# microsoft/FIBER

Measured on AMD Instinct MI355X. Metric: train-step images/sec (384^2, seq40) FIBER-Base, higher is better.
Workload: dtype bf16; 1 GPU; FIBER-Base (Swin-B 384^2 + RoBERTa-base S=40) MLM+ITM pretrain step, fused backbone fwd+bwd x2 + heads + AdamW; per_gpu_batch=256, global_batch=256, parallelism=dp1, rccl_ranks=1, dropout=reference defaults (text 0.1, DropPath linspace 0..0.1), residual_dtype=bf16, mlm_head_rows=all, launch=eager (one launch per kernel)

## Files before the change

### fiber_amd/csrc/elementwise.hip

```cpp
#include "common.h"

namespace {

__global__ __launch_bounds__(256) void gelu_bwd_kernel(const bf16* __restrict__ dg, const bf16* __restrict__ h,
                                                       bf16* __restrict__ dh, size_t nvec) {
  for (size_t i = blockIdx.x * (size_t)256 + threadIdx.x; i < nvec; i += (size_t)gridDim.x * 256) {
    const bf16x8 a = reinterpret_cast<const bf16x8*>(dg)[i], b = reinterpret_cast<const bf16x8*>(h)[i];
    reinterpret_cast<bf16x8*>(dh)[i] = gelu_grad_mul8(a, b);
  }
}

__global__ __launch_bounds__(256) void scale_add_kernel(const bf16* __restrict__ a, const bf16* __restrict__ b,
                                                        const float* __restrict__ alpha, float mult,
                                                        bf16* __restrict__ out, size_t nvec) {
  const float s = (alpha ? alpha[0] : 1.f) * mult;
  for (size_t i = blockIdx.x * (size_t)256 + threadIdx.x; i < nvec; i += (size_t)gridDim.x * 256) {
    const bf16x8 y = reinterpret_cast<const bf16x8*>(b)[i];
    bf16x8 o;
    if (a) {
      const bf16x8 x = reinterpret_cast<const bf16x8*>(a)[i];
#pragma unroll
      for (int e = 0; e < 8; ++e) o[e] = f2bf(bf2f(x[e]) + s * bf2f(y[e]));
    } else {
#pragma unroll
// ... 10 lines not shown
  for (size_t i = blockIdx.x * (size_t)256 + threadIdx.x; i < nvec; i += (size_t)gridDim.x * 256) {
    const bf16x8 x = reinterpret_cast<const bf16x8*>(a)[i], y = reinterpret_cast<const bf16x8*>(b)[i];
#pragma unroll
    for (int e = 0; e < 8; ++e) s += bf2f(x[e]) * bf2f(y[e]);
  }
  s = wave_sum(s);
  if ((threadIdx.x & 63) == 0) red[threadIdx.x >> 6] = s;
  __syncthreads();
  if (threadIdx.x == 0) out[blockIdx.x] = (red[0] + red[1]) + (red[2] + red[3]);
}

__global__ __launch_bounds__(256) void colsum_kernel(const bf16* __restrict__ x, float* __restrict__ out, int M, int N,
                                                     int ld, int rows_per_block) {
  __shared__ float red[8][32 * 8 + 1];
  const int cv = threadIdx.x & 31, rl = threadIdx.x >> 5;
  const int col = (blockIdx.x * 32 + cv) * 8;
  const int r0 = blockIdx.y * rows_per_block, r1 = min(M, r0 + rows_per_block);
  float s[8] = {0, 0, 0, 0, 0, 0, 0, 0};
  if (col < N) {
    int r = r0 + rl;
    for (; r + 24 < r1; r += 32) {
      const bf16x8 v0 = *reinterpret_cast<const bf16x8*>(x + (size_t)r * ld + col);
      const bf16x8 v1 = *reinterpret_cast<const bf16x8*>(x + (size_t)(r + 8) * ld + col);
      const bf16x8 v2 = *reinterpret_cast<const bf16x8*>(x + (size_t)(r + 16) * ld + col);
      const bf16x8 v3 = *reinterpret_cast<const bf16x8*>(x + (size_t)(r + 24) * ld + col);
#pragma unroll
      for (int e = 0; e < 8; ++e) s[e] += (bf2f(v0[e]) + bf2f(v1[e])) + (bf2f(v2[e]) + bf2f(v3[e]));
    }
    for (; r < r1; r += 8) {
      const bf16x8 v = *reinterpret_cast<const bf16x8*>(x + (size_t)r * ld + col);
#pragma unroll
      for (int e = 0; e < 8; ++e) s[e] += bf2f(v[e]);
    }
  }
#pragma unroll
  for (int e = 0; e < 8; ++e) red[rl][cv * 8 + e] = s[e];
  __syncthreads();
  const int c = threadIdx.x;
  float t = 0.f;
#pragma unroll
  for (int r = 0; r < 8; ++r) t += red[r][c];
  const int gc = blockIdx.x * 256 + c;
  if (gc < N) out[(size_t)blockIdx.y * N + gc] = t;
}

__global__ __launch_bounds__(256) void gelu_bwd_colsum_kernel(const bf16* __restrict__ dg, const bf16* __restrict__ h,
                                                              bf16* __restrict__ dh, float* __restrict__ out, int M, int N,
                                                              int rows_per_block) {
  __shared__ float red[8][32 * 8 + 1];
  const int cv = threadIdx.x & 31, rl = threadIdx.x >> 5;
  const int col = (blockIdx.x * 32 + cv) * 8;
  const int r0 = blockIdx.y * rows_per_block, r1 = min(M, r0 + rows_per_block);
  float s[8] = {0, 0, 0, 0, 0, 0, 0, 0};
  if (col < N) {
    auto one = [&](int r, const bf16x8& a, const bf16x8& b) {
      const bf16x8 o = gelu_grad_mul8(a, b);
#pragma unroll
      for (int e = 0; e < 8; ++e) s[e] += bf2f(o[e]);
      *reinterpret_cast<bf16x8*>(dh + (size_t)r * N + col) = o;
    };
    int r = r0 + rl;
    for (; r + 8 < r1; r += 16) {
      const size_t o0 = (size_t)r * N + col, o1 = (size_t)(r + 8) * N + col;
      const bf16x8 a0 = *reinterpret_cast<const bf16x8*>(dg + o0), b0 = *reinterpret_cast<const bf16x8*>(h + o0);
      const bf16x8 a1 = *reinterpret_cast<const bf16x8*>(dg + o1), b1 = *reinterpret_cast<const bf16x8*>(h + o1);
      one(r, a0, b0); one(r + 8, a1, b1);
    }
    for (; r < r1; r += 8) {
      const size_t off = (size_t)r * N + col;
      one(r, *reinterpret_cast<const bf16x8*>(dg + off), *reinterpret_cast<const bf16x8*>(h + off));
    }
  }
#pragma unroll
  for (int e = 0; e < 8; ++e) red[rl][cv * 8 + e] = s[e];
  __syncthreads();
  const int c = threadIdx.x;
  float t = 0.f;
#pragma unroll
  for (int r = 0; r < 8; ++r) t += red[r][c];
  const int gc = blockIdx.x * 256 + c;
  if (gc < N) out[(size_t)blockIdx.y * N + gc] = t;
}

__global__ __launch_bounds__(256) void rowscale_colsum_kernel(const bf16* __restrict__ x, const float* __restrict__ scale,
                                                              bf16* __restrict__ y, float* __restrict__ out, int M, int N,
                                                              int rows_per_block, int rows_per_sample) {
  __shared__ float red[8][32 * 8 + 1];
  const int cv = threadIdx.x & 31, rl = threadIdx.x >> 5;
  const int col = (blockIdx.x * 32 + cv) * 8;
  const int r0 = blockIdx.y * rows_per_block, r1 = min(M, r0 + rows_per_block);
  float s[8] = {0, 0, 0, 0, 0, 0, 0, 0};
  if (col < N) {
    auto one = [&](int r, const bf16x8& a) {
      const float sc = scale[r / rows_per_sample];
      bf16x8 o;
#pragma unroll
      for (int e = 0; e < 8; ++e) { o[e] = f2bf(sc * bf2f(a[e])); s[e] += bf2f(o[e]); }
      *reinterpret_cast<bf16x8*>(y + (size_t)r * N + col) = o;
    };
    int r = r0 + rl;
    for (; r + 24 < r1; r += 32) {
      const bf16x8 a0 = *reinterpret_cast<const bf16x8*>(x + (size_t)r * N + col);
      const bf16x8 a1 = *reinterpret_cast<const bf16x8*>(x + (size_t)(r + 8) * N + col);
      const bf16x8 a2 = *reinterpret_cast<const bf16x8*>(x + (size_t)(r + 16) * N + col);
      const bf16x8 a3 = *reinterpret_cast<const bf16x8*>(x + (size_t)(r + 24) * N + col);
      one(r, a0); one(r + 8, a1); one(r + 16, a2); one(r + 24, a3);
    }
    for (; r < r1; r += 8) one(r, *reinterpret_cast<const bf16x8*>(x + (size_t)r * N + col));
  }
#pragma unroll
  for (int e = 0; e < 8; ++e) red[rl][cv * 8 + e] = s[e];
  __syncthreads();
  const int c = threadIdx.x;
  float t = 0.f;
#pragma unroll
  for (int r = 0; r < 8; ++r) t += red[r][c];
  const int gc = blockIdx.x * 256 + c;
  if (gc < N) out[(size_t)blockIdx.y * N + gc] = t;
}

__global__ __launch_bounds__(256) void colsum_fold_kernel(const float* __restrict__ part, float* __restrict__ out, int slabs, int N) {
  __shared__ float red[16][17];
  const int cl = threadIdx.x & 15, rl = threadIdx.x >> 4;
  const int c = blockIdx.x * 16 + cl;
  float s0 = 0.f, s1 = 0.f, s2 = 0.f, s3 = 0.f;
  if (c < N) {
    int y = rl;
    for (; y + 48 < slabs; y += 64) {
      s0 += part[(size_t)y * N + c];
      s1 += part[(size_t)(y + 16) * N + c];
      s2 += part[(size_t)(y + 32) * N + c];
      s3 += part[(size_t)(y + 48) * N + c];
    }
    for (; y < slabs; y += 16) s0 += part[(size_t)y * N + c];
  }
  red[rl][cl] = (s0 + s1) + (s2 + s3);
  __syncthreads();
  if (rl == 0 && c < N) {
    float t = 0.f;
#pragma unroll
    for (int r = 0; r < 16; ++r) t += red[r][cl];
    out[c] = t;
  }
}

__global__ __launch_bounds__(256) void dropout_kernel(const bf16* __restrict__ x, bf16* __restrict__ y, size_t nvec,
                                                      uint64_t seed, const uint64_t* __restrict__ seed_base, uint32_t thresh,
                                                      float inv_keep) {
  if (seed_base) seed += *seed_base;
  for (size_t i = blockIdx.x * (size_t)256 + threadIdx.x; i < nvec; i += (size_t)gridDim.x * 256) {
    const bf16x8 v = reinterpret_cast<const bf16x8*>(x)[i];
    bf16x8 o;
    const uint32_t h0 = drop_base(seed, i * 8);
#pragma unroll
    for (int e = 0; e < 8; ++e) o[e] = drop_keep_e(h0, e, thresh) ? f2bf(bf2f(v[e]) * inv_keep) : f2bf(0.f);
    reinterpret_cast<bf16x8*>(y)[i] = o;
  }
}

__global__ __launch_bounds__(256) void droppath_scale_kernel(float* __restrict__ out, int n, float keep, uint64_t seed,
                                                             const uint64_t* __restrict__ seed_base) {
  if (seed_base) seed += *seed_base;
  const int i = blockIdx.x * 256 + threadIdx.x;
  if (i < n) {
    const float u = (float)(hash_u32(seed, (uint64_t)i) >> 9) * (1.0f / 8388608.0f);
    out[i] = floorf(keep + u) / keep;
  }
}

__global__ __launch_bounds__(256) void rowscale_add_kernel(const bf16* __restrict__ r, const bf16* __restrict__ x,
                                                           const float* __restrict__ scale, bf16* __restrict__ out,
                                                           size_t nvec, size_t vec_per_sample) {
  for (size_t i = blockIdx.x * (size_t)256 + threadIdx.x; i < nvec; i += (size_t)gridDim.x * 256) {
    const float s = scale[i / vec_per_sample];
    const bf16x8 b = reinterpret_cast<const bf16x8*>(x)[i];
    bf16x8 o;
    if (r) {
      const bf16x8 a = reinterpret_cast<const bf16x8*>(r)[i];
#pragma unroll
      for (int e = 0; e < 8; ++e) o[e] = f2bf(bf2f(a[e]) + s * bf2f(b[e]));
    } else {
#pragma unroll
      for (int e = 0; e < 8; ++e) o[e] = f2bf(s * bf2f(b[e]));
    }
    reinterpret_cast<bf16x8*>(out)[i] = o;
  }
}


struct StreamAddArgs {
  const void* res; const bf16* a; const bf16* b; const float* alpha; const float* rowscale;
  float* out32; bf16* out16;
  size_t nvec, vec_per_sample;
  uint64_t seed_a, seed_b; const uint64_t* seed_base;
  uint32_t thresh_a, thresh_b; float inv_keep_a, inv_keep_b;
};

template <int RES>
__global__ __launch_bounds__(256) void stream_add_kernel(StreamAddArgs p) {
  const float al = p.alpha ? p.alpha[0] : 1.f;
  uint64_t sa = p.seed_a, sb = p.seed_b;
  if (p.seed_base) { sa += *p.seed_base; sb += *p.seed_base; }
  for (size_t i = blockIdx.x * (size_t)256 + threadIdx.x; i < p.nvec; i += (size_t)gridDim.x * 256) {
    const float rs = p.rowscale ? p.rowscale[i / p.vec_per_sample] : 1.f;
    const bf16x8 av = reinterpret_cast<const bf16x8*>(p.a)[i];
    float v[8];
#pragma unroll
    for (int e = 0; e < 8; ++e) v[e] = bf2f(av[e]);
    if (p.thresh_a) {
      const uint32_t ha = drop_base(sa, i * 8);
#pragma unroll
      for (int e = 0; e < 8; ++e) v[e] = drop_keep_e(ha, e, p.thresh_a) ? v[e] * p.inv_keep_a : 0.f;
    }
    if (p.b) {
      const bf16x8 bv = reinterpret_cast<const bf16x8*>(p.b)[i];
      const uint32_t hb = drop_base(sb, i * 8);
#pragma unroll
      for (int e = 0; e < 8; ++e) {
        float t = bf2f(bv[e]);
        if (p.thresh_b) t = drop_keep_e(hb, e, p.thresh_b) ? t * p.inv_keep_b : 0.f;
        v[e] += al * t;
      }
    }
#pragma unroll
    for (int e = 0; e < 8; ++e) v[e] *= rs;
    if constexpr (RES == 2) {
      const float* rp = reinterpret_cast<const float*>(p.res) + i * 8;
      const float4 r0 = *reinterpret_cast<const float4*>(rp), r1 = *reinterpret_cast<const float4*>(rp + 4);
      v[0] += r0.x; v[1] += r0.y; v[2] += r0.z; v[3] += r0.w; v[4] += r1.x; v[5] += r1.y; v[6] += r1.z; v[7] += r1.w;
    } else if constexpr (RES == 1) {
      const bf16x8 rv = reinterpret_cast<const bf16x8*>(p.res)[i];
#pragma unroll
      for (int e = 0; e < 8; ++e) v[e] += bf2f(rv[e]);
    }
    if (p.out32) {
      float* op = p.out32 + i * 8;
      *reinterpret_cast<float4*>(op) = float4{v[0], v[1], v[2], v[3]};
      *reinterpret_cast<float4*>(op + 4) = float4{v[4], v[5], v[6], v[7]};
    }
    if (p.out16) {
      bf16x8 o;
#pragma unroll
      for (int e = 0; e < 8; ++e) o[e] = f2bf(v[e]);
      reinterpret_cast<bf16x8*>(p.out16)[i] = o;
    }
  }
}

struct StreamAddBwdArgs {
  const bf16* dy; const bf16* b; const float* alpha; const float* rowscale;
  bf16* da; bf16* db; float* dpart;
  size_t nvec, vec_per_sample;
// ... 89 lines not shown
  hipLaunchKernelGGL(scale_add_kernel, dim3(ew_grid(n / 8)), dim3(256), 0, stream, (const bf16*)a, (const bf16*)b, alpha, mult, (bf16*)out, (size_t)n / 8);
  FIBER_CHECK_LAUNCH();
  return FIBER_OK;
}

static inline int dot_grid(size_t nvec) {
  const size_t g = (nvec + 255) / 256;
  return (int)(g > FIBER_DOT_PARTS ? FIBER_DOT_PARTS : g);
}

extern "C" int fiber_dot_bf16(const void* a, const void* b, float* out, float* workspace, long n, hipStream_t stream) {
  if (n <= 0) return FIBER_OK;
  if ((n & 7) || !out || fiber_misaligned(16, a, b)) return FIBER_EINVAL;
  const size_t nvec = n / 8;
  const int grid = dot_grid(nvec);
  if (grid > 1 && !workspace) return FIBER_EINVAL;
  hipLaunchKernelGGL(dot_kernel, dim3(grid), dim3(256), 0, stream, (const bf16*)a, (const bf16*)b, grid > 1 ? workspace : out, nvec);
  FIBER_CHECK_LAUNCH();
  if (grid > 1) {
    hipLaunchKernelGGL(colsum_fold_kernel, dim3(1), dim3(256), 0, stream, workspace, out, grid, 1);
    FIBER_CHECK_LAUNCH();
  }
  return FIBER_OK;
}

extern "C" int fiber_colsum_slabs(int M, int N) {
  const int gx = cdiv(N, 256);
  int gy = cdiv(M, 512);
  int cap = cdiv(1024, gx);
  cap = cap > 512 ? 512 : cap;
  gy = gy > cap ? cap : gy;
  return gy < 1 ? 1 : gy;
}

extern "C" int fiber_colsum_bf16(const void* x, float* out, float* workspace, int M, int N, int ld, hipStream_t stream) {
  if (M <= 0 || N <= 0) return FIBER_OK;
  if ((N & 7) || (ld & 7) || fiber_misaligned(16, x)) return FIBER_EINVAL;
  const int gx = cdiv(N, 256);
  const int gy0 = fiber_colsum_slabs(M, N);
  const int rpb = cdiv(M, gy0), gy = cdiv(M, rpb);
  if (gy > 1 && !workspace) return FIBER_EINVAL;
  hipLaunchKernelGGL(colsum_kernel, dim3(gx, gy), dim3(256), 0, stream, (const bf16*)x, gy > 1 ? workspace : out, M, N, ld, rpb);
  FIBER_CHECK_LAUNCH();
  if (gy > 1) {
    hipLaunchKernelGGL(colsum_fold_kernel, dim3(cdiv(N, 16)), dim3(256), 0, stream, workspace, out, gy, N);
    FIBER_CHECK_LAUNCH();
  }
  return FIBER_OK;
}

extern "C" int fiber_gelu_bwd_colsum_bf16(const void* dgelu, const void* h_pre, void* dh, float* db, float* workspace, int M,
                                          int N, hipStream_t stream) {
  if (M <= 0 || N <= 0) return FIBER_OK;
  if ((N & 7) || fiber_misaligned(16, dgelu, h_pre, dh)) return FIBER_EINVAL;
  const int gx = cdiv(N, 256);
  const int gy0 = fiber_colsum_slabs(M, N);
  const int rpb = cdiv(M, gy0), gy = cdiv(M, rpb);
  if (gy > 1 && !workspace) return FIBER_EINVAL;
  hipLaunchKernelGGL(gelu_bwd_colsum_kernel, dim3(gx, gy), dim3(256), 0, stream, (const bf16*)dgelu, (const bf16*)h_pre, (bf16*)dh,
                     gy > 1 ? workspace : db, M, N, rpb);
  FIBER_CHECK_LAUNCH();
  if (gy > 1) {
    hipLaunchKernelGGL(colsum_fold_kernel, dim3(cdiv(N, 16)), dim3(256), 0, stream, workspace, db, gy, N);
    FIBER_CHECK_LAUNCH();
  }
  return FIBER_OK;
}

extern "C" int fiber_rowscale_colsum_bf16(const void* x, const float* scale, void* y, float* db, float* workspace, int M, int N,
                                          int rows_per_sample, hipStream_t stream) {
  if (M <= 0 || N <= 0) return FIBER_OK;
  if ((N & 7) || rows_per_sample <= 0 || fiber_misaligned(16, x, y)) return FIBER_EINVAL;
  const int gx = cdiv(N, 256);
  const int gy0 = fiber_colsum_slabs(M, N);
  const int rpb = cdiv(M, gy0), gy = cdiv(M, rpb);
  if (gy > 1 && !workspace) return FIBER_EINVAL;
  hipLaunchKernelGGL(rowscale_colsum_kernel, dim3(gx, gy), dim3(256), 0, stream, (const bf16*)x, scale, (bf16*)y,
                     gy > 1 ? workspace : db, M, N, rpb, rows_per_sample);
  FIBER_CHECK_LAUNCH();
  if (gy > 1) {
    hipLaunchKernelGGL(colsum_fold_kernel, dim3(cdiv(N, 16)), dim3(256), 0, stream, workspace, db, gy, N);
    FIBER_CHECK_LAUNCH();
  }
  return FIBER_OK;
}

extern "C" int fiber_fold_rows_f32(const float* part, float* out, int rows, int N, hipStream_t stream) {
  if (rows <= 0 || N <= 0) return FIBER_OK;
  hipLaunchKernelGGL(colsum_fold_kernel, dim3(cdiv(N, 16)), dim3(256), 0, stream, part, out, rows, N);
  FIBER_CHECK_LAUNCH();
  return FIBER_OK;
}

extern "C" int fiber_dropout_bf16(const void* x, void* y, long n, float p, uint64_t seed, const uint64_t* seed_base,
                                  hipStream_t stream) {
  if (n <= 0) return FIBER_OK;
  if ((n & 7) || p < 0.f || p >= 1.f || fiber_misaligned(16, x, y)) return FIBER_EINVAL;
  const uint32_t thresh = (uint32_t)((double)p * 4294967296.0);
  hipLaunchKernelGGL(dropout_kernel, dim3(ew_grid(n / 8)), dim3(256), 0, stream, (const bf16*)x, (bf16*)y, (size_t)n / 8, seed, seed_base, thresh, 1.f / (1.f - p));
  FIBER_CHECK_LAUNCH();
  return FIBER_OK;
}

extern "C" int fiber_droppath_scale_f32(float* out, int n, float keep, uint64_t seed, const uint64_t* seed_base,
                                        hipStream_t stream) {
  if (n <= 0) return FIBER_OK;
  if (keep <= 0.f || keep > 1.f) return FIBER_EINVAL;
  hipLaunchKernelGGL(droppath_scale_kernel, dim3(cdiv(n, 256)), dim3(256), 0, stream, out, n, keep, seed, seed_base);
  FIBER_CHECK_LAUNCH();
  return FIBER_OK;
}

extern "C" int fiber_rowscale_add_bf16(const void* r, const void* x, const float* scale, void* out, long n,
                                       long per_sample, hipStream_t stream) {
  if (n <= 0) return FIBER_OK;
  if ((n & 7) || per_sample <= 0 || (per_sample & 7) || fiber_misaligned(16, r, x, out)) return FIBER_EINVAL;
  hipLaunchKernelGGL(rowscale_add_kernel, dim3(ew_grid(n / 8)), dim3(256), 0, stream, (const bf16*)r, (const bf16*)x, scale, (bf16*)out, (size_t)n / 8, (size_t)per_sample / 8);
  FIBER_CHECK_LAUNCH();
  return FIBER_OK;
}

extern "C" int fiber_stream_add(const void* res, int res_kind, const void* a, const void* b, const float* alpha,
                                const float* rowscale, long per_sample, float p_a, uint64_t seed_a, float p_b, uint64_t seed_b,
                                const uint64_t* seed_base, float* out32, void* out16, long n, hipStream_t stream) {
  if (n <= 0) return FIBER_OK;
  if ((n & 7) || !a || (!out32 && !out16) || (res_kind && !res) || res_kind < 0 || res_kind > 2) return FIBER_EINVAL;
  if (fiber_misaligned(16, res, a, b, out32, out16)) return FIBER_EINVAL;
  if (rowscale && (per_sample <= 0 || (per_sample & 7))) return FIBER_EINVAL;
  if (p_a < 0.f || p_a >= 1.f || p_b < 0.f || p_b >= 1.f || (p_b > 0.f && !b)) return FIBER_EINVAL;
  StreamAddArgs p{res, (const bf16*)a, (const bf16*)b, alpha, rowscale, out32, (bf16*)out16, (size_t)n / 8,
                  rowscale ? (size_t)per_sample / 8 : (size_t)1, seed_a, seed_b, seed_base,
                  (uint32_t)((double)p_a * 4294967296.0), (uint32_t)((double)p_b * 4294967296.0), 1.f / (1.f - p_a), 1.f / (1.f - p_b)};
  const int grid = ew_grid(p.nvec);
  if (res_kind == 2) hipLaunchKernelGGL(stream_add_kernel<2>, dim3(grid), dim3(256), 0, stream, p);
  else if (res_kind == 1) hipLaunchKernelGGL(stream_add_kernel<1>, dim3(grid), dim3(256), 0, stream, p);
  else hipLaunchKernelGGL(stream_add_kernel<0>, dim3(grid), dim3(256), 0, stream, p);
  FIBER_CHECK_LAUNCH();
  return FIBER_OK;
}

extern "C" int fiber_stream_add_bwd(const void* dy, const void* b, const float* alpha, const float* rowscale, long per_sample,
                                    float p_a, uint64_t seed_a, float p_b, uint64_t seed_b, const uint64_t* seed_base, void* da,
                                    void* db, float* dalpha, float* workspace, long n, hipStream_t stream) {
  if (n <= 0) return FIBER_OK;
  if ((n & 7) || !dy || (dalpha && (!b || !db))) return FIBER_EINVAL;
  if (fiber_misaligned(16, dy, b, da, db)) return FIBER_EINVAL;
  if (rowscale && (per_sample <= 0 || (per_sample & 7))) return FIBER_EINVAL;
  if (p_a < 0.f || p_a >= 1.f || p_b < 0.f || p_b >= 1.f) return FIBER_EINVAL;
  StreamAddBwdArgs p{(const bf16*)dy, (const bf16*)b, alpha, rowscale, (bf16*)da, (bf16*)db, nullptr, (size_t)n / 8,
                     rowscale ? (size_t)per_sample / 8 : (size_t)1, seed_a, seed_b, seed_base,
                     (uint32_t)((double)p_a * 4294967296.0), (uint32_t)((double)p_b * 4294967296.0), 1.f / (1.f - p_a), 1.f / (1.f - p_b)};
  int grid = ew_grid(p.nvec);
  if (dalpha) {
    grid = dot_grid(p.nvec);
    if (grid > 1 && !workspace) return FIBER_EINVAL;
    p.dpart = grid > 1 ? workspace : dalpha;
  }
  hipLaunchKernelGGL(stream_add_bwd_kernel, dim3(grid), dim3(256), 0, stream, p);
  FIBER_CHECK_LAUNCH();
  if (dalpha && grid > 1) {
    hipLaunchKernelGGL(colsum_fold_kernel, dim3(1), dim3(256), 0, stream, workspace, dalpha, grid, 1);
    FIBER_CHECK_LAUNCH();
  }
  return FIBER_OK;
}

// ... 8 lines not shown
```

### fiber_amd/csrc/gemm.hip

```cpp
#include <stdlib.h>

#include "gemm_epilogue.h"

namespace {

template <int BM, int BN>
__global__ __launch_bounds__(256) void gemm_nt_kernel(GemmArgs a) {
  constexpr int WTM = BM / 2, WTN = BN / 2;
  constexpr int TM = WTM / 32, TN = WTN / 32;
  constexpr int PA = BM / 32, PB = BN / 32;
  __shared__ __attribute__((aligned(16))) bf16 As[2][BM * BK];
  __shared__ __attribute__((aligned(16))) bf16 Bs[2][BN * BK];

  const int tid = threadIdx.x, lane = tid & 63, wave = tid >> 6;
  const int wm = wave >> 1, wn = wave & 1;
  const int tilesN = (a.N + BN - 1) / BN, tilesM = (a.M + BM - 1) / BM;
  const int nblk = tilesM * tilesN;
  int bid = blockIdx.x;
  {
    const int q = nblk >> 3, r = nblk & 7, xcd = bid & 7, idx = bid >> 3;
    bid = (xcd < r ? xcd * (q + 1) : r * (q + 1) + (xcd - r) * q) + idx;
  }
  const int tm0 = (bid / tilesN) * BM, tn0 = (bid % tilesN) * BN;

// ... 45 lines not shown
  const int frow = lane & 31, fk = lane >> 5;
  for (int kt = 0; kt < nk; ++kt) {
    const int cur = kt & 1;
    if (kt + 1 < nk) gload(kt + 1);
#pragma unroll
    for (int ks = 0; ks < BK / 16; ++ks) {
      bf16x8 fa[TM], fb[TN];
#pragma unroll
      for (int i = 0; i < TM; ++i)
        fa[i] = *reinterpret_cast<const bf16x8*>(&As[cur][swz(wm * WTM + i * 32 + frow, ks * 2 + fk)]);
#pragma unroll
      for (int j = 0; j < TN; ++j)
        fb[j] = *reinterpret_cast<const bf16x8*>(&Bs[cur][swz(wn * WTN + j * 32 + frow, ks * 2 + fk)]);
#pragma unroll
      for (int i = 0; i < TM; ++i)
#pragma unroll
        for (int j = 0; j < TN; ++j)
          acc[i][j] = __builtin_amdgcn_mfma_f32_32x32x16_bf16(fb[j], fa[i], acc[i][j], 0, 0, 0);
    }
    if (kt + 1 < nk) lstore(cur ^ 1);
    __syncthreads();
  }

#pragma unroll
  for (int i = 0; i < TM; ++i) {
    const int m = tm0 + wm * WTM + i * 32 + (lane & 31);
    if (m >= a.M) continue;
    const float rsc = a.rowscale ? a.rowscale[m / a.rows_per_sample] : 1.f;
#pragma unroll
    for (int j = 0; j < TN; ++j) {
#pragma unroll
      for (int q = 0; q < 4; ++q) {
        const int n = tn0 + wn * WTN + j * 32 + q * 8 + (lane >> 5) * 4;
        if (n >= a.N) continue;
        float v[4];
#pragma unroll
        for (int e = 0; e < 4; ++e) v[e] = acc[i][j][q * 4 + e];
        if (a.bias) {
          const float4 b = *reinterpret_cast<const float4*>(a.bias + n);
          v[0] += b.x; v[1] += b.y; v[2] += b.z; v[3] += b.w;
        }
        if ((a.act & 0xff) == 1) {
          if (a.Ypre) {
            bf16x4 o;
#pragma unroll
            for (int e = 0; e < 4; ++e) o[e] = f2bf(v[e]);
            *reinterpret_cast<bf16x4*>(a.Ypre + (size_t)m * a.ldy + n) = o;
          }
#pragma unroll
          for (int e = 0; e < 4; ++e) v[e] = gelu_erf(v[e]);
        }
        if (a.rowscale) {
#pragma unroll
          for (int e = 0; e < 4; ++e) v[e] *= rsc;
        }
        if (a.act & 0x800) {
          const float4 r = *reinterpret_cast<const float4*>(reinterpret_cast<const float*>(a.R) + (size_t)m * a.ldr + n);
          const float4 o = {bf2f(f2bf(v[0])) + r.x, bf2f(f2bf(v[1])) + r.y, bf2f(f2bf(v[2])) + r.z, bf2f(f2bf(v[3])) + r.w};
          *reinterpret_cast<float4*>(reinterpret_cast<float*>(a.Ypre) + (size_t)m * a.ldy + n) = o;
          if (a.Y) {
            bf16x4 ob = {f2bf(o.x), f2bf(o.y), f2bf(o.z), f2bf(o.w)};
            *reinterpret_cast<bf16x4*>(a.Y + (size_t)m * a.ldy + n) = ob;
          }
          continue;
        }
        if (a.R) {
          const bf16x4 r = *reinterpret_cast<const bf16x4*>(a.R + (size_t)m * a.ldr + n);
#pragma unroll
          for (int e = 0; e < 4; ++e) v[e] += bf2f(r[e]);
        }
        if (a.act & 0x100) {
          *reinterpret_cast<float4*>(reinterpret_cast<float*>(a.Y) + (size_t)m * a.ldy + n) = float4{v[0], v[1], v[2], v[3]};
          continue;
        }
        bf16x4 o;
#pragma unroll
        for (int e = 0; e < 4; ++e) o[e] = f2bf(v[e]);
        *reinterpret_cast<bf16x4*>(a.Y + (size_t)m * a.ldy + n) = o;
      }
    }
  }
}

template <int BM, int BN, int WM, int WN, int NS, int EPI, bool HAS_R, bool HAS_RS>
__global__ __launch_bounds__(64 * WM * WN) void gemm_nt_glds_kernel(GemmArgs a) {
  constexpr int NT = 64 * WM * WN;
  constexpr int WTM = BM / WM, WTN = BN / WN;
  constexpr int TM = WTM / 32, TN = WTN / 32;
  constexpr int RPD = NT / 8;
  constexpr int PA = BM / RPD, PB = BN / RPD;
  constexpr int CLD = BN + 8;
  static_assert(BM * CLD <= NS * (BM + BN) * BK, "epilogue tile must fit in the operand buffers");
  __shared__ __attribute__((aligned(16))) bf16 smem[NS * (BM + BN) * BK + 512];
  bf16* As = smem;
  bf16* Bs = smem + NS * BM * BK;
  float* bias_s = reinterpret_cast<float*>(smem + NS * (BM + BN) * BK);

  const int tid = threadIdx.x, lane = tid & 63, wave = tid >> 6;
  const int wm = wave / WN, wn = wave % WN;
  const int tilesN = (a.N + BN - 1) / BN, tilesM = (a.M + BM - 1) / BM;
  const int nblk = tilesM * tilesN;
  int bid = blockIdx.x;
  {
    const int q = nblk >> 3, r = nblk & 7, xcd = bid & 7, idx = bid >> 3;
    bid = (xcd < r ? xcd * (q + 1) : r * (q + 1) + (xcd - r) * q) + idx;
  }
  const int tm0 = (bid / tilesN) * BM, tn0 = (bid % tilesN) * BN;

  const int srow = wave * 8 + (lane >> 3), spc = lane & 7;
  const bf16* xsrc[PA];
  const bf16* wsrc[PB];
#pragma unroll
  for (int p = 0; p < PA; ++p) {
    const int row = srow + p * RPD;
    int r = tm0 + row;
    r = r < a.M ? r : a.M - 1;
    xsrc[p] = a.X + (size_t)r * a.ldx + ((spc ^ ((row >> 1) & 7)) << 3);
  }
#pragma unroll
  for (int p = 0; p < PB; ++p) {
    const int row = srow + p * RPD;
    int r = tn0 + row;
    r = r < a.N ? r : a.N - 1;
    wsrc[p] = a.W + (size_t)r * a.ldw + ((spc ^ ((row >> 1) & 7)) << 3);
  }
  auto dma1 = [&](int d, int kt, int buf) {
    if (d < PA)
      __builtin_amdgcn_global_load_lds((const __attribute__((address_space(1))) void*)(xsrc[d < PA ? d : 0] + kt * BK),
                                       (__attribute__((address_space(3))) void*)(As + buf * BM * BK + (d * RPD + wave * 8) * BK), 16, 0, 0);
    else
      __builtin_amdgcn_global_load_lds((const __attribute__((address_space(1))) void*)(wsrc[d >= PA ? d - PA : 0] + kt * BK),
                                       (__attribute__((address_space(3))) void*)(Bs + buf * BN * BK + ((d - PA) * RPD + wave * 8) * BK), 16, 0, 0);
  };
  auto dma = [&](int kt, int buf) {
#pragma unroll
    for (int d = 0; d < PA + PB; ++d) dma1(d, kt, buf);
  };

  f32x16 acc[TM][TN];
#pragma unroll
  for (int i = 0; i < TM; ++i)
#pragma unroll
    for (int j = 0; j < TN; ++j)
#pragma unroll
      for (int r = 0; r < 16; ++r) acc[i][j][r] = 0.f;

  stage_bias<BN>(a, bias_s, tn0);
  const int nk = a.K / BK;
  const int frow = lane & 31, fk = lane >> 5;
  const bool dbg_nodma = a.act & 0x100;
  constexpr int KS = BK / 16;
  constexpr int DPK = (PA + PB + KS - 2) / (KS - 1);
  auto compute = [&](int buf, bool prefetch, int kt_next, int nbuf) {
    const bf16* Ac = As + buf * BM * BK;
    const bf16* Bc = Bs + buf * BN * BK;
    bf16x8 fa[2][TM], fb[2][TN];
#pragma unroll
    for (int i = 0; i < TM; ++i) fa[0][i] = *reinterpret_cast<const bf16x8*>(Ac + swz(wm * WTM + i * 32 + frow, fk));
#pragma unroll
    for (int j = 0; j < TN; ++j) fb[0][j] = *reinterpret_cast<const bf16x8*>(Bc + swz(wn * WTN + j * 32 + frow, fk));
#pragma unroll
    for (int ks = 0; ks < KS; ++ks) {
      const int c = ks & 1, n = c ^ 1;
      if (ks + 1 < KS) {
#pragma unroll
        for (int i = 0; i < TM; ++i) fa[n][i] = *reinterpret_cast<const bf16x8*>(Ac + swz(wm * WTM + i * 32 + frow, (ks + 1) * 2 + fk));
#pragma unroll
        for (int j = 0; j < TN; ++j) fb[n][j] = *reinterpret_cast<const bf16x8*>(Bc + swz(wn * WTN + j * 32 + frow, (ks + 1) * 2 + fk));
        if (prefetch) {
#pragma unroll
          for (int d = ks * DPK; d < (ks + 1) * DPK && d < PA + PB; ++d) dma1(d, kt_next, nbuf);
        }
      }
      __builtin_amdgcn_sched_barrier(0);
#pragma unroll
      for (int i = 0; i < TM; ++i)
#pragma unroll
        for (int j = 0; j < TN; ++j)
          acc[i][j] = __builtin_amdgcn_mfma_f32_32x32x16_bf16(fb[c][j], fa[c][i], acc[i][j], 0, 0, 0);
      __builtin_amdgcn_sched_barrier(0);
    }
  };
  if constexpr (NS == 2) {
    dma(0, 0);
    asm volatile("s_waitcnt vmcnt(0)" ::: "memory");
    __syncthreads();
    for (int kt = 0; kt < nk; ++kt) {
      const int cur = kt & 1;
      compute(cur, kt + 1 < nk && !dbg_nodma, kt + 1, cur ^ 1);
      asm volatile("s_waitcnt vmcnt(0)" ::: "memory");
      __syncthreads();
    }
  } else {
    static_assert(NS == 3 && PA + PB == 6, "counted vmcnt below is written for 3 stages x 6 DMA instructions");
    dma(0, 0);
    if (nk > 1) dma(1, 1);
    int buf = 0;
    for (int kt = 0; kt < nk; ++kt) {
      if (kt + 1 < nk) asm volatile("s_waitcnt vmcnt(6)" ::: "memory");
      else asm volatile("s_waitcnt vmcnt(0)" ::: "memory");
      __builtin_amdgcn_s_barrier();
      asm volatile("" ::: "memory");
      const int nb = buf == 0 ? 2 : buf - 1;
      compute(buf, kt + 2 < nk && !dbg_nodma, kt + 2, nb);
      buf = buf == 2 ? 0 : buf + 1;
    }
    asm volatile("s_waitcnt lgkmcnt(0)" ::: "memory");
    __syncthreads();
  }

  if (tm0 + BM <= a.M && tn0 + BN <= a.N)
    tile_epilogue<BM, BN, WM, WN, 1, EPI, HAS_R, HAS_RS, true>(a, acc, smem, bias_s, tm0, tn0);
  else
    tile_epilogue<BM, BN, WM, WN, 1, EPI, HAS_R, HAS_RS, false>(a, acc, smem, bias_s, tm0, tn0);
}

template <int WM, int WN, int EPI, bool HAS_R, bool HAS_RS>
__global__ __launch_bounds__(64 * WM * WN) void gemm_nt_wide_persist_kernel(GemmArgs a) {
  constexpr int BM = 256, BN = 256, NS = 2;
  constexpr int NT = 64 * WM * WN;
  static_assert(NT == 512 && WM == 2, "two wave groups of four; DMA pass geometry for 8 waves");
  constexpr int WTM = BM / WM, WTN = BN / WN;
  constexpr int TM = WTM / 32, TN = WTN / 32;
  constexpr int RPD = NT / 8;
  constexpr int PA = BM / RPD, PB = BN / RPD;
  constexpr int STAGE = (BM + BN) * BK;
  constexpr int CLD = BN + 8;
  constexpr int ROUNDS = 4;
  static_assert((size_t)(BM / ROUNDS) * CLD * 2 <= (size_t)STAGE * 2, "an epilogue round must fit one ring stage");
  __shared__ __attribute__((aligned(16))) bf16 smem[NS * STAGE + 1024];
  float* bias_s = reinterpret_cast<float*>(smem + NS * STAGE);

  const int tid = threadIdx.x, lane = tid & 63, wave = tid >> 6;
  const int wm = wave / WN, wn = wave % WN;
  const int tilesN = (a.N + BN - 1) / BN, tilesM = (a.M + BM - 1) / BM;
  const int nblk = tilesM * tilesN;
  const int P = gridDim.x >> 3, xcd = blockIdx.x & 7, widx = blockIdx.x >> 3;
  const int q8 = nblk >> 3, r8 = nblk & 7;
  const int first = (xcd < r8 ? xcd * (q8 + 1) : r8 * (q8 + 1) + (xcd - r8) * q8) + widx;
  const int count = q8 + (xcd < r8 ? 1 : 0);
  const int T = widx < count ? (count - widx + P - 1) / P : 0;
  if (T == 0) return;

  const int srow = wave * 8 + (lane >> 3), spc = lane & 7;
  const bf16* xbase; const bf16* wbase;
  unsigned xo[PA], wo[PB];
  auto aim = [&](int seq) {
    const int id = first + seq * P;
    const int m0 = (id / tilesN) * BM, n0 = (id % tilesN) * BN;
    xbase = a.X + (size_t)m0 * a.ldx;
    wbase = a.W + (size_t)n0 * a.ldw;
#pragma unroll
    for (int p = 0; p < PA; ++p) {
      const int row = srow + p * RPD;
      xo[p] = (unsigned)(min(row, a.M - 1 - m0) * a.ldx + ((spc ^ ((row >> 1) & 7)) << 3)) * 2u;
    }
#pragma unroll
    for (int p = 0; p < PB; ++p) {
      const int row = srow + p * RPD;
      wo[p] = (unsigned)(min(row, a.N - 1 - n0) * a.ldw + ((spc ^ ((row >> 1) & 7)) << 3)) * 2u;
    }
    if (a.bias)
      lds_dma16(a.bias, (unsigned)min(n0 + lane * 4, a.N - 4) * 4u, bias_s + (seq & 1) * 256);
  };
  auto dma = [&](int g, int kt) {
    bf16* st = smem + (g & 1) * STAGE;
#pragma unroll
    for (int p = 0; p < PA; ++p)
      lds_dma16(xbase + kt * BK, xo[p], st + (p * RPD + wave * 8) * BK);
#pragma unroll
    for (int p = 0; p < PB; ++p)
      lds_dma16(wbase + kt * BK, wo[p], st + BM * BK + (p * RPD + wave * 8) * BK);
  };

  f32x16 acc[TM][TN];
  auto zero_acc = [&]() {
#pragma unroll
    for (int i = 0; i < TM; ++i)
#pragma unroll
      for (int j = 0; j < TN; ++j)
#pragma unroll
        for (int r = 0; r < 16; ++r) acc[i][j][r] = 0.f;
  };
  zero_acc();

  const int nk = a.K / BK;
  const int frow = lane & 31, fk = lane >> 5;
  bf16x8 fa[2][TM], fb[2][TN];
  auto load_phase = [&](int g, int sub) {
    const bf16* Ac = smem + (g & 1) * STAGE;
    const bf16* Bc = Ac + BM * BK;
#pragma unroll
    for (int ks = 0; ks < 2; ++ks) {
#pragma unroll
      for (int i = 0; i < TM; ++i) fa[ks][i] = *reinterpret_cast<const bf16x8*>(Ac + swz(wm * WTM + i * 32 + frow, sub * 4 + ks * 2 + fk));
#pragma unroll
      for (int j = 0; j < TN; ++j) fb[ks][j] = *reinterpret_cast<const bf16x8*>(Bc + swz(wn * WTN + j * 32 + frow, sub * 4 + ks * 2 + fk));
    }
  };
  auto math_phase = [&]() {
    __builtin_amdgcn_s_setprio(1);
#pragma unroll
    for (int ks = 0; ks < 2; ++ks)
#pragma unroll
      for (int i = 0; i < TM; ++i)
#pragma unroll
        for (int j = 0; j < TN; ++j)
          acc[i][j] = __builtin_amdgcn_mfma_f32_32x32x16_bf16(fb[ks][j], fa[ks][i], acc[i][j], 0, 0, 0);
    __builtin_amdgcn_s_setprio(0);
  };
  auto phase_barrier = [&](bool landed) {
    if (landed) asm volatile("s_waitcnt vmcnt(0) lgkmcnt(0)" ::: "memory");
    else asm volatile("s_waitcnt lgkmcnt(0)" ::: "memory");
    __builtin_amdgcn_sched_barrier(0);
    __builtin_amdgcn_s_barrier();
    asm volatile("" ::: "memory");
    __builtin_amdgcn_sched_barrier(0);
  };

  aim(0);
  dma(0, 0);
  phase_barrier(true);
  int g = 0;
  for (int seq = 0; seq < T; ++seq) {
    const int id = first + seq * P;
    const int tm0 = (id / tilesN) * BM, tn0 = (id % tilesN) * BN;
    if (wm == 1) phase_barrier(false);
    for (int kt = 0; kt < nk; ++kt, ++g) {
      load_phase(g, 0);
      if (kt + 1 < nk) dma(g + 1, kt + 1);
      else if (seq + 1 < T) { aim(seq + 1); dma(g + 1, 0); }
      phase_barrier(false);
      math_phase();
      phase_barrier(false);
      load_phase(g, 1);
      phase_barrier(wm == 1);
      math_phase();
      phase_barrier(wm == 0);
    }
    if (wm == 0) phase_barrier(false);
    bf16* Cs = smem + ((g - 1) & 1) * STAGE;
    const float* bias_c = bias_s + (seq & 1) * 256;
    if (tm0 + BM <= a.M && tn0 + BN <= a.N)
      tile_epilogue<BM, BN, WM, WN, ROUNDS, EPI, HAS_R, HAS_RS, true, true>(a, acc, Cs, bias_c, tm0, tn0);
    else
      tile_epilogue<BM, BN, WM, WN, ROUNDS, EPI, HAS_R, HAS_RS, false, true>(a, acc, Cs, bias_c, tm0, tn0);
    zero_acc();
  }
}

template <int EPI, bool HAS_R, bool HAS_RS, bool TRACE = false>
__global__ __launch_bounds__(512) void gemm_nt_q8_kernel(GemmArgs a) {
  constexpr int BM = 256, BN = 256, WN = 4;
  constexpr int WTM = 128, WTN = 64, TM = 4, TN = 2;
  constexpr int STAGE = (BM + BN) * BK;
  constexpr int SLAB = 32 * 64;
  __shared__ __attribute__((aligned(16))) bf16 smem[2 * STAGE + 8 * SLAB];

  const int tid = threadIdx.x, lane = tid & 63;
  const int wave = __builtin_amdgcn_readfirstlane(tid >> 6);
  const int wm = wave / WN, wn = wave % WN;
  bf16* cw = smem + 2 * STAGE + wave * SLAB;
  const int tilesN = (a.N + BN - 1) / BN, tilesM = (a.M + BM - 1) / BM;
  const int nblk = tilesM * tilesN;
  const int P = gridDim.x >> 3, xcd = blockIdx.x & 7, widx = blockIdx.x >> 3;
  const int q8 = nblk >> 3, r8 = nblk & 7;
  const int first = (xcd < r8 ? xcd * (q8 + 1) : r8 * (q8 + 1) + (xcd - r8) * q8) + widx;
  const int count = q8 + (xcd < r8 ? 1 : 0);
  const int T = widx < count ? (count - widx + P - 1) / P : 0;
  if (T == 0) return;
  const int nk = a.K / BK;

  const int lr = lane >> 3;
  const unsigned csw = (unsigned)(((lane & 7) ^ (((wave & 1) << 2) + (lr >> 1))) << 4);
  const int ra0 = wave * 8, rb0 = (wave >> 2) * 64 + (wave & 3) * 8;
  const bf16* xbase; const bf16* wbase;
  unsigned xo[2][2], wo[2][2];
  int c_seq = 0, c_kt = 0, c_g = 0;
  auto aim = [&]() {
    const int id = first + c_seq * P;
    const int m0 = (id / tilesN) * BM, n0 = (id % tilesN) * BN;
    xbase = a.X + (size_t)m0 * a.ldx;
    wbase = a.W + (size_t)n0 * a.ldw;
    const int xlim = a.M - 1 - m0, wlim = a.N - 1 - n0;
#pragma unroll
    for (int h = 0; h < 2; ++h)
#pragma unroll
      for (int u = 0; u < 2; ++u) {
        xo[h][u] = (unsigned)(min(u * 128 + h * 64 + ra0 + lr, xlim) * a.ldx) * 2u + csw;
        wo[h][u] = (unsigned)(min(u * 128 + h * 32 + rb0 + lr, wlim) * a.ldw) * 2u + csw;
      }
  };
  auto advance = [&]() {
    ++c_g;
    if (++c_kt == nk) {
      if (c_seq + 1 < T) { c_kt = 0; ++c_seq; aim(); }
      else c_kt = nk - 1;
    }
  };
  auto stageA = [&](int h) {
    bf16* st = smem + (c_g & 1) * STAGE;
    lds_dma16(xbase + c_kt * BK, xo[h][0], st + (h * 64 + ra0) * BK);
    lds_dma16(xbase + c_kt * BK, xo[h][1], st + (128 + h * 64 + ra0) * BK);
  };
  auto stageW = [&](int j) {
    bf16* st = smem + (c_g & 1) * STAGE + BM * BK;
    lds_dma16(wbase + c_kt * BK, wo[j][0], st + (j * 32 + rb0) * BK);
    lds_dma16(wbase + c_kt * BK, wo[j][1], st + (128 + j * 32 + rb0) * BK);
  };

  f32x16 acc[TM][TN];
  const int frow = lane & 31, fk = lane >> 5;
  bf16x8 fa[4][2], fb[2][4];
  auto readA = [&](const bf16* sb, int h) {
#pragma unroll
    for (int ks = 0; ks < 4; ++ks)
#pragma unroll
      for (int ii = 0; ii < 2; ++ii)
        fa[ks][ii] = *reinterpret_cast<const bf16x8*>(sb + swz(wm * WTM + (2 * h + ii) * 32 + frow, ks * 2 + fk));
  };
  auto readW = [&](const bf16* sb, int j) {
#pragma unroll
    for (int ks = 0; ks < 4; ++ks)
      fb[j][ks] = *reinterpret_cast<const bf16x8*>(sb + BM * BK + swz(wn * WTN + j * 32 + frow, ks * 2 + fk));
  };
  struct SeedRaw { float v[32]; bool on; };
  auto seed_raw = [&](int n0w, int j) {
    SeedRaw r;
    r.on = EPI != 2 && a.bias && n0w < a.N;
    if (r.on) {
      typedef __attribute__((address_space(4))) const float cfloat;
      cfloat* bp = (cfloat*)(uintptr_t)(a.bias + n0w + j * 32);
#pragma unroll
      for (int i = 0; i < 32; ++i) r.v[i] = bp[i];
    } else {
// ... 63 lines not shown
      const unsigned long long t = __builtin_amdgcn_s_memtime();
      tr[i] += t - t0;
      t0 = t;
    }
  };
  for (int seq = 0; seq < T; ++seq) {
    const int id = first + seq * P;
    const int tm0 = (id / tilesN) * BM, tn0 = (id % tilesN) * BN;
    const int n0w = tn0 + wn * WTN;
    if (!keep_stagger && wm == 1) { __builtin_amdgcn_s_barrier(); asm volatile("" ::: "memory"); }
    for (int kt = 0; kt < nk; ++kt, ++g) {
      const bf16* sb = smem + (g & 1) * STAGE;
      readW(sb, 0);
      __builtin_amdgcn_sched_barrier(0);
      readA(sb, 0);
      stageW(1);
      mark(0);
      if (kt == 0) {
        const SeedRaw raw = seed_raw(n0w, 0);
        bar_load(false);
        mark(1);
        mma_seeded(0, 0, seed_sel(raw));
      } else {
        bar_load(false);
        mark(1);
        mma(0, 0);
      }
      mark(2);
      bar_math();
      mark(3);
      readW(sb, 1);
      stageA(1);
      advance();
      mark(4);
      if (kt == 0) {
        const SeedRaw raw = seed_raw(n0w, 1);
        bar_load(true);
        mark(5);
        mma_seeded(0, 1, seed_sel(raw));
      } else {
        bar_load(true);
        mark(5);
        mma(0, 1);
      }
      mark(6);
      bar_math();
      mark(7);
      readA(sb, 1);
      stageA(0);
      mark(8);
      if (kt == 0) {
        const SeedRaw raw = seed_raw(n0w, 1);
        bar_load(false);
        mark(9);
        mma_seeded(1, 1, seed_sel(raw));
      } else {
        bar_load(false);
        mark(9);
        mma(1, 1);
      }
      mark(10);
      bar_math();
      mark(11);
      stageW(0);
      mark(12);
      if (kt == 0) {
        const SeedRaw raw = seed_raw(n0w, 0);
        bar_load(true);
        mark(13);
        mma_seeded(1, 0, seed_sel(raw));
      } else {
        bar_load(true);
        mark(13);
        mma(1, 0);
      }
      mark(14);
      bar_math();
      mark(15);
    }
    if (!keep_stagger && wm == 0) { __builtin_amdgcn_s_barrier(); asm volatile("" ::: "memory"); }
    if constexpr (TRACE) t0 = __builtin_amdgcn_s_memtime();
    if (n0w >= a.N) {
    } else if (tm0 + BM <= a.M)
      wave_epilogue<TM, EPI, HAS_R, HAS_RS, true>(a, acc, cw, tm0 + wm * WTM, tn0 + wn * WTN);
    else
      wave_epilogue<TM, EPI, HAS_R, HAS_RS, false>(a, acc, cw, tm0 + wm * WTM, tn0 + wn * WTN);
    mark(16);
  }
  if (keep_stagger && wm == 0) { __builtin_amdgcn_s_barrier(); asm volatile("" ::: "memory"); }
  asm volatile("s_waitcnt vmcnt(0)" ::: "memory");
  if constexpr (TRACE) {
    if (lane == 0 && blockIdx.x < 8) {
      float* o = a.colpart + (blockIdx.x * 8 + wave) * 24;
      for (int i = 0; i < 17; ++i) o[i] = (float)tr[i];
      o[17] = (float)(__builtin_amdgcn_s_memtime() - tstart);
      o[18] = (float)nk;
      o[19] = (float)T;
    }
  }
}

constexpr bool q8_ok(int epi, bool r, bool rs) { return (epi == 0 && (!r || rs)) || (epi == 1 && !r) || epi == 2 || (epi == 3 && rs); }
__device__ float g_gemm_one = 1.0f;
constexpr bool wide_persist_ok(int epi, bool r, bool rs) { return epi != 0 && !q8_ok(epi, r, rs); }

}

#ifdef FIBER_P2_PROBE
#ifndef FIBER_P2_PROBE_EPI
#define FIBER_P2_PROBE_EPI 0
#endif
extern "C" void fiber_p2_probe(GemmArgs a, hipStream_t st) {
  hipLaunchKernelGGL((gemm_nt_q8_kernel<FIBER_P2_PROBE_EPI, false, false>), dim3(256), dim3(512), 0, st, a);
}
#else
enum GemmFamily { kRejected, kQ8, kWidePersist, kRing256x128, kRing128, kRing64, kReg128, kReg64 };
struct GemmPlan { GemmFamily family; int rows; unsigned grid; };

constexpr long kWideMinTiles = 200;

static GemmPlan gemm_plan(int M, int N, int K, int ldy, int ldr, bool has_r, bool has_rs, bool colpart, int act) {
  static const int force = getenv("FIBER_GEMM_TILE") ? atoi(getenv("FIBER_GEMM_TILE")) : 0;
  static const int nowide = getenv("FIBER_GEMM_NOWIDE") ? atoi(getenv("FIBER_GEMM_NOWIDE")) : 0;
  static const int tile[8][2] = {{0, 0}, {256, 256}, {256, 256}, {256, 128}, {128, 128}, {64, 64}, {128, 128}, {64, 64}};
  const long big = (long)cdiv(M, 128) * cdiv(N, 128);
  const long huge = (long)cdiv(M, 256) * cdiv(N, 128);
  const long wide = (long)cdiv(M, 256) * cdiv(N, 256);
  const int mode = act & 0xff;
  const int epi = (act & 0x800) ? 3 : (mode == 1 || mode == 2) ? mode : 0;
  const bool trace = (act & 0x1000) != 0;
  const bool v2 = (K % 64 == 0) && (N % 8 == 0) && (ldy % 8 == 0) && (!has_r || ldr % 8 == 0) && !getenv("FIBER_GEMM_V1");
  const bool wide_ok = v2 && !nowide && force == 0 && wide >= kWideMinTiles && K >= 128;
  const bool q8 = q8_ok(epi, has_r, has_rs) && !(epi == 2 && colpart) && !trace;
  GemmFamily f;
  if (act & 0x100) {
    if (mode != 0 || has_r || colpart) return GemmPlan{kRejected, 0, 0};
    f = big >= 192 ? kReg128 : kReg64;
  } else if (wide_ok && q8 && (N % 256 == 0 || (N % 64 == 0 && N > 256))) f = kQ8;
  else if (wide_ok && epi != 2 && N % 256 == 0) f = (epi == 0 || trace) ? kQ8 : kWidePersist;
  else if (v2 && ((huge >= 400 && K >= 256 && force == 0) || force == 256)) f = kRing256x128;
  else if (big >= 192 || force == 128) f = v2 ? kRing128 : kReg128;
  else f = v2 ? kRing64 : kReg64;
  const bool persistent = f == kQ8 || f == kWidePersist;
  return GemmPlan{f, tile[f][0], persistent ? 256u : (unsigned)(cdiv(M, tile[f][0]) * cdiv(N, tile[f][1]))};
}

extern "C" int fiber_gemm_row_tile(int M, int N, int K) {
  return gemm_plan(M, N, K, N, 0, false, false, true, 2).rows;
}

template <int EPI, bool R, bool RS>
static int launch_nt(const GemmPlan& p, const GemmArgs& a, hipStream_t stream) {
  const dim3 grid(p.grid);
  if (p.family == kQ8) {
    if constexpr (q8_ok(EPI, R, RS)) hipLaunchKernelGGL((gemm_nt_q8_kernel<EPI, R, RS>), grid, dim3(512), 0, stream, a);
    else return FIBER_EINVAL;
  } else if (p.family == kWidePersist) {
    if constexpr (wide_persist_ok(EPI, R, RS)) hipLaunchKernelGGL((gemm_nt_wide_persist_kernel<2, 4, EPI, R, RS>), grid, dim3(512), 0, stream, a);
    else return FIBER_EINVAL;
  } else if (p.family == kRing256x128) hipLaunchKernelGGL((gemm_nt_glds_kernel<256, 128, 4, 2, 3, EPI, R, RS>), grid, dim3(512), 0, stream, a);
  else if (p.family == kRing128) hipLaunchKernelGGL((gemm_nt_glds_kernel<128, 128, 2, 2, 2, EPI, R, RS>), grid, dim3(256), 0, stream, a);
  else hipLaunchKernelGGL((gemm_nt_glds_kernel<64, 64, 2, 2, 2, EPI, R, RS>), grid, dim3(256), 0, stream, a);
  return FIBER_OK;
}

extern "C" int fiber_gemm_nt_bf16(const void* X, const void* W, const float* bias, const void* residual, void* Y,
                                  void* Ypre, const float* rowscale, int rows_per_sample, const void* aux, int ldaux,
                                  float* colpart, int M, int N, int K, int ldx, int ldw, int ldy, int ldr, int act,
                                  hipStream_t stream) {
  if (M <= 0 || N <= 0 || K <= 0) return FIBER_OK;
  if ((K & 7) || (N & 3) || (ldx & 7) || (ldw & 7) || (ldy & 3) || (residual && (ldr & 3))) return FIBER_EINVAL;
  if (rowscale && rows_per_sample <= 0) return FIBER_EINVAL;
  if ((act & 0xff) == 2 && (!aux || (ldaux & 7))) return FIBER_EINVAL;
  GemmArgs a{(const bf16*)X, (const bf16*)W, bias, (const bf16*)residual, (bf16*)Y, (bf16*)Ypre, rowscale,
             (const bf16*)aux, colpart, M, N, K, ldx, ldw, ldy, ldr, act, rows_per_sample, ldaux};
  static const int stagger_env = getenv("FIBER_GEMM_STAGGER") ? atoi(getenv("FIBER_GEMM_STAGGER")) : 0;
  if (stagger_env) a.act |= 0x4000;
  if ((size_t)M * N * 2 > ((size_t)256 << 20)) a.act |= 0x2000;
  const int mode = act & 0xff;
  if ((mode == 2 || colpart) && !((K % 64 == 0) && (N % 8 == 0) && (ldy % 8 == 0))) return FIBER_EINVAL;
  if (mode == 2 && residual) return FIBER_EINVAL;
  if ((act & 0x800) && (mode != 0 || !residual || !Ypre || colpart || (act & 0x100))) return FIBER_EINVAL;
  if (colpart && mode != 2 && !(act & 0x1000)) return FIBER_EINVAL;
  const GemmPlan plan = gemm_plan(M, N, K, ldy, ldr, residual != nullptr, rowscale != nullptr, colpart != nullptr, act);
  if (plan.family == kRejected) return FIBER_EINVAL;
  const dim3 grid(plan.grid);
  int rc = FIBER_OK;
  if (plan.family == kQ8 && (act & 0x1000)) {
    a.act &= 0x40ff;
    if (mode == 1) hipLaunchKernelGGL((gemm_nt_q8_kernel<1, false, false, true>), grid, dim3(512), 0, stream, a);
    else hipLaunchKernelGGL((gemm_nt_q8_kernel<0, false, false, true>), grid, dim3(512), 0, stream, a);
  }
  else if (plan.family == kReg128) hipLaunchKernelGGL((gemm_nt_kernel<128, 128>), grid, dim3(256), 0, stream, a);
  else if (plan.family == kReg64) hipLaunchKernelGGL((gemm_nt_kernel<64, 64>), grid, dim3(256), 0, stream, a);
  else if (act & 0x800) rc = rowscale ? launch_nt<3, true, true>(plan, a, stream) : launch_nt<3, true, false>(plan, a, stream);
  else if (mode == 2) rc = rowscale ? launch_nt<2, false, true>(plan, a, stream) : launch_nt<2, false, false>(plan, a, stream);
  else if (mode == 1 && residual) rc = rowscale ? launch_nt<1, true, true>(plan, a, stream) : launch_nt<1, true, false>(plan, a, stream);
  else if (mode == 1) rc = rowscale ? launch_nt<1, false, true>(plan, a, stream) : launch_nt<1, false, false>(plan, a, stream);
  else if (residual && rowscale) rc = launch_nt<0, true, true>(plan, a, stream);
  else if (residual && plan.family == kQ8) {
    static const float* one_of[16] = {};
    int dev = 0;
    if (hipGetDevice(&dev) != hipSuccess || dev < 0 || dev >= 16) return FIBER_ELAUNCH;
    if (one_of[dev] == nullptr) { float* p = nullptr; if (hipGetSymbolAddress((void**)&p, HIP_SYMBOL(g_gemm_one)) != hipSuccess) return FIBER_ELAUNCH; one_of[dev] = p; }
    const float* one = one_of[dev];
    if (one == nullptr) return FIBER_ELAUNCH;
    a.rowscale = one; a.rows_per_sample = a.M;
    rc = launch_nt<0, true, true>(plan, a, stream);
  }
  else if (residual) rc = launch_nt<0, true, false>(plan, a, stream);
  else if (rowscale) rc = launch_nt<0, false, true>(plan, a, stream);
  else rc = launch_nt<0, false, false>(plan, a, stream);
  if (rc != FIBER_OK) return rc;
  FIBER_CHECK_LAUNCH();
  return FIBER_OK;
}
#endif
```

### fiber_amd/csrc/gemm_epilogue.h

```cpp
#pragma once
#include "common.h"

namespace {

constexpr int BK = 64;

struct GemmArgs {
  const bf16* X; const bf16* W; const float* bias; const bf16* R; bf16* Y; bf16* Ypre;
  const float* rowscale;
  const bf16* aux;
  float* colpart;
  int M, N, K, ldx, ldw, ldy, ldr, act, rows_per_sample, ldaux;
};

__device__ __forceinline__ int swz(int row, int chunk) { return (row * 8 + (chunk ^ ((row >> 1) & 7))) * 8; }

__device__ __forceinline__ void st_out(bf16x8* p, bf16x8 v, bool stream) {
  if (stream) __builtin_nontemporal_store(v, p); else *p = v;
}
__device__ __forceinline__ void st_stream(bf16x8* p, bf16x8 v) { __builtin_nontemporal_store(v, p); }

template <bool RAWBAR>
__device__ __forceinline__ void epi_barrier() {
  if constexpr (RAWBAR) {
    asm volatile("s_waitcnt lgkmcnt(0)" ::: "memory");
    __builtin_amdgcn_s_barrier();
    asm volatile("" ::: "memory");
  } else {
    __syncthreads();
  }
}

template <int BM, int BN, int WM, int WN, int ROUNDS, int EPI, bool HAS_R, bool HAS_RS, bool FULL, bool RAWBAR = false>
__device__ __forceinline__ void tile_epilogue(const GemmArgs& a, f32x16 (&acc)[BM / WM / 32][BN / WN / 32], bf16* Cs,
                                              const float* bias_s, int tm0, int tn0) {
  constexpr int NT = 64 * WM * WN;
  constexpr int WTM = BM / WM, WTN = BN / WN;
  constexpr int TM = WTM / 32, TN = WTN / 32;
  constexpr int CLD = BN + 8;
  constexpr int HM = BM / ROUNDS;
  constexpr int CPR = BN / 8;
  constexpr int RPP = NT / CPR;
  constexpr int NPH = HM / RPP;
  static_assert(HM % 32 == 0 && HM % RPP == 0, "epilogue geometry");
  const int tid = threadIdx.x, lane = tid & 63, wave = tid >> 6;
  const int wm = wave / WN, wn = wave % WN;
  const int erow = tid / CPR, echunk = tid % CPR;
  const int n_out = tn0 + echunk * 8;
  const bool col_ok = FULL || n_out < a.N;
  constexpr bool E0 = EPI == 0 || EPI == 3;
  constexpr bool SIDE = (HAS_R && EPI != 3) || EPI == 2;
  const bf16* sidep = EPI == 2 ? a.aux : a.R;
  const size_t sideld = EPI == 2 ? a.ldaux : a.ldr;
  const bool has_bias = a.bias != nullptr;
  float csum[8] = {0.f, 0.f, 0.f, 0.f, 0.f, 0.f, 0.f, 0.f};

#pragma unroll
  for (int h = 0; h < ROUNDS; ++h) {
    const int mbase = tm0 + h * HM + erow;
    bf16x8 side[SIDE ? NPH : 1];
    float prs[((EPI == 1 || EPI == 2) && HAS_RS) ? NPH : 1];
    if constexpr (SIDE) {
      const bf16* sp = sidep + (size_t)mbase * sideld + n_out;
#pragma unroll
      for (int pp = 0; pp < NPH; ++pp)
        if (FULL || (mbase + pp * RPP < a.M && col_ok)) side[pp] = *reinterpret_cast<const bf16x8*>(sp + (size_t)pp * RPP * sideld);
    }
    if constexpr ((EPI == 1 || EPI == 2) && HAS_RS) {
#pragma unroll
      for (int pp = 0; pp < NPH; ++pp) prs[pp] = a.rowscale[min(mbase + pp * RPP, a.M - 1) / a.rows_per_sample];
    }
#pragma unroll
    for (int i = 0; i < TM; ++i) {
      if (ROUNDS == 1 || (wm * WTM + i * 32) / HM == h) {
        const int ml = wm * WTM + i * 32 + (lane & 31);
        float rsc = 1.f;
        if constexpr (E0 && HAS_RS) rsc = a.rowscale[min(tm0 + ml, a.M - 1) / a.rows_per_sample];
        bf16* crow = Cs + (ml - h * HM) * CLD + wn * WTN + (lane >> 5) * 4;
#pragma unroll
        for (int j = 0; j < TN; ++j)
#pragma unroll
          for (int q = 0; q < 4; ++q) {
            const int nl = wn * WTN + j * 32 + q * 8 + (lane >> 5) * 4;
            float v[4];
#pragma unroll
            for (int e = 0; e < 4; ++e) v[e] = acc[i][j][q * 4 + e];
            if (EPI != 2 && has_bias) {
              const float4 bb = *reinterpret_cast<const float4*>(bias_s + nl);
              v[0] += bb.x; v[1] += bb.y; v[2] += bb.z; v[3] += bb.w;
            }
            if constexpr (E0 && HAS_RS) {
#pragma unroll
              for (int e = 0; e < 4; ++e) v[e] *= rsc;
            }
            bf16x4 o;
#pragma unroll
            for (int e = 0; e < 4; ++e) o[e] = f2bf(v[e]);
            *reinterpret_cast<bf16x4*>(crow + j * 32 + q * 8) = o;
          }
      }
    }
    epi_barrier<RAWBAR>();
    {
      bf16* yp = a.Y + (size_t)mbase * a.ldy + n_out;
      bf16* prep = (EPI == 1 && a.Ypre) ? a.Ypre + (size_t)mbase * a.ldy + n_out : nullptr;
      const size_t ystep = (size_t)RPP * a.ldy;
      const bf16* cp = Cs + erow * CLD + echunk * 8;
#pragma unroll
      for (int pp = 0; pp < NPH; ++pp) {
        if (FULL || (mbase + pp * RPP < a.M && col_ok)) {
          bf16x8 v = *reinterpret_cast<const bf16x8*>(cp + pp * RPP * CLD);
          if constexpr (EPI == 1) {
            if (prep) st_stream(reinterpret_cast<bf16x8*>(prep + pp * ystep), v);
            v = gelu8(v, HAS_RS ? prs[pp] : 1.f);
          } else if constexpr (EPI == 2) {
            v = gelu_grad_mul8(v, side[pp], HAS_RS ? prs[pp] : 1.f);
          }
          if constexpr (EPI == 3) {
            const size_t row = (size_t)(mbase + pp * RPP);
            const float* rp = reinterpret_cast<const float*>(a.R) + row * a.ldr + n_out;
            float* op = reinterpret_cast<float*>(a.Ypre) + row * a.ldy + n_out;
            const float4 r0 = *reinterpret_cast<const float4*>(rp), r1 = *reinterpret_cast<const float4*>(rp + 4);
            const float4 o0 = {bf2f(v[0]) + r0.x, bf2f(v[1]) + r0.y, bf2f(v[2]) + r0.z, bf2f(v[3]) + r0.w};
            const float4 o1 = {bf2f(v[4]) + r1.x, bf2f(v[5]) + r1.y, bf2f(v[6]) + r1.z, bf2f(v[7]) + r1.w};
            *reinterpret_cast<float4*>(op) = o0;
            *reinterpret_cast<float4*>(op + 4) = o1;
            if (a.Y) {
              v[0] = f2bf(o0.x); v[1] = f2bf(o0.y); v[2] = f2bf(o0.z); v[3] = f2bf(o0.w);
              v[4] = f2bf(o1.x); v[5] = f2bf(o1.y); v[6] = f2bf(o1.z); v[7] = f2bf(o1.w);
              st_out(reinterpret_cast<bf16x8*>(yp + pp * ystep), v, (a.act & 0x2000) != 0);
            }
            continue;
          }
          if constexpr (HAS_R) {
#pragma unroll
            for (int e = 0; e < 8; ++e) v[e] = f2bf(bf2f(v[e]) + bf2f(side[pp][e]));
          }
          st_out(reinterpret_cast<bf16x8*>(yp + pp * ystep), v, (a.act & 0x2000) != 0);
          if constexpr (EPI == 2) {
#pragma unroll
            for (int e = 0; e < 8; ++e) csum[e] += bf2f(v[e]);
          }
        }
      }
    }
    if (h + 1 < ROUNDS || EPI == 2 || RAWBAR) epi_barrier<RAWBAR>();
  }
  if constexpr (EPI == 2) {
    if (a.colpart) {
      float* red = reinterpret_cast<float*>(Cs);
      constexpr int LPC = 64 / (CPR < 64 ? CPR : 64);
#pragma unroll
      for (int e = 0; e < 8; ++e) {
        float t = csum[e];
        if constexpr (LPC >= 2 && CPR <= 32) t += __shfl_xor(t, 32);
        if constexpr (LPC >= 4 && CPR <= 16) t += __shfl_xor(t, 16);
        if constexpr (LPC >= 8 && CPR <= 8) t += __shfl_xor(t, 8);
        csum[e] = t;
      }
      static_assert(CPR == 8 || CPR == 16 || CPR == 32, "column-sum shuffle tree");
      if (lane < CPR) {
#pragma unroll
        for (int e = 0; e < 8; ++e) red[wave * BN + lane * 8 + e] = csum[e];
      }
      epi_barrier<RAWBAR>();
      for (int c = tid; c < BN; c += NT) {
        float t = 0.f;
#pragma unroll
        for (int w = 0; w < WM * WN; ++w) t += red[w * BN + c];
        if (tn0 + c < a.N) a.colpart[(size_t)(tm0 / BM) * a.N + tn0 + c] = t;
      }
      if constexpr (RAWBAR) epi_barrier<RAWBAR>();
    }
  }
}

template <int TM, int EPI, bool HAS_R, bool HAS_RS, bool FULL>
__device__ __forceinline__ void wave_epilogue(const GemmArgs& a, f32x16 (&acc)[TM][2], bf16* cw, int m0w, int n0w) {
  int lane = __builtin_amdgcn_mbcnt_hi(~0u, __builtin_amdgcn_mbcnt_lo(~0u, 0u));
  asm volatile("" : "+v"(lane));
  const int wr = lane & 31, wh = lane >> 5;
  const int rr = lane >> 3, rc = lane & 7;
  constexpr bool E0 = EPI == 0 || EPI == 3;
  constexpr bool SIDE = (HAS_R && EPI != 3) || EPI == 2;
  const bf16* sidep = EPI == 2 ? a.aux : a.R;
  const size_t sideld = EPI == 2 ? a.ldaux : a.ldr;
  const int n_out = n0w + rc * 8;
  bf16* wbase = cw + wr * 64 + wh * 4;
  const int wsw = (wr >> 1) & 7;
  const bf16* rbase = cw + rr * 64;
  auto stage = [&](int i) {
    float rsc = 1.f;
    if constexpr (E0 && HAS_RS) rsc = a.rowscale[min(m0w + i * 32 + wr, a.M - 1) / a.rows_per_sample];
#pragma unroll
    for (int j = 0; j < 2; ++j)
#pragma unroll
      for (int q = 0; q < 4; ++q) {
        bf16x4 o;
#pragma unroll
        for (int e = 0; e < 4; ++e) o[e] = f2bf((E0 && HAS_RS) ? acc[i][j][q * 4 + e] * rsc : acc[i][j][q * 4 + e]);
        *reinterpret_cast<bf16x4*>(wbase + (((j * 4 + q) ^ wsw) << 3)) = o;
      }
  };
  auto read_pass = [&](int pp) {
    const int row = pp * 8 + rr;
    return *reinterpret_cast<const bf16x8*>(rbase + pp * 8 * 64 + ((rc ^ ((row >> 1) & 7)) << 3));
  };
  auto load_side = [&](int i, bf16x8 (&sd)[4], float (&prs)[4]) {
    const int mrow = m0w + i * 32 + rr;
    if constexpr (SIDE) {
      const bf16* sp = sidep + (size_t)mrow * sideld + n_out;
#pragma unroll
      for (int pp = 0; pp < 4; ++pp)
        if (FULL || mrow + pp * 8 < a.M) sd[pp] = *reinterpret_cast<const bf16x8*>(sp + (size_t)pp * 8 * sideld);
    }
    if constexpr ((EPI == 1 || EPI == 2) && HAS_RS) {
#pragma unroll
      for (int pp = 0; pp < 4; ++pp) prs[pp] = a.rowscale[min(mrow + pp * 8, a.M - 1) / a.rows_per_sample];
    }
  };
  auto load_side_pass = [&](int i, int pp, bf16x8& sdp, float& prp) {
    const int mrow = m0w + i * 32 + rr + pp * 8;
    if (FULL || mrow < a.M) sdp = *reinterpret_cast<const bf16x8*>(sidep + (size_t)mrow * sideld + n_out);
    if constexpr (HAS_RS) prp = a.rowscale[min(mrow, a.M - 1) / a.rows_per_sample];
  };
  const float* r32 = reinterpret_cast<const float*>(a.R);
  float* y32 = reinterpret_cast<float*>(a.Ypre);
  float4 rf[EPI == 3 ? 4 : 1][2];
  auto load_r32 = [&](int i, int pp) {
    const int mrow = m0w + i * 32 + rr + pp * 8;
    if (FULL || mrow < a.M) {
      const float* rp = r32 + (size_t)mrow * a.ldr + n_out;
      rf[pp][0] = *reinterpret_cast<const float4*>(rp);
      rf[pp][1] = *reinterpret_cast<const float4*>(rp + 4);
    }
  };
  constexpr bool PREF = EPI != 2 && EPI != 3;
  bf16x8 cur[4], sd[4], sdn[PREF ? 4 : 1];
  float prs[4] = {1.f, 1.f, 1.f, 1.f}, prsn[4] = {1.f, 1.f, 1.f, 1.f};
  load_side(0, sd, prs);
  if constexpr (EPI == 3) {
#pragma unroll
    for (int pp = 0; pp < 4; ++pp) load_r32(0, pp);
  }
  stage(0);
  asm volatile("" ::: "memory");
#pragma unroll
  for (int pp = 0; pp < 4; ++pp) cur[pp] = read_pass(pp);
#pragma unroll
  for (int i = 0; i < TM; ++i) {
    if (i + 1 < TM) {
      if constexpr (PREF) load_side(i + 1, sdn, prsn);
      asm volatile("" ::: "memory");
      stage(i + 1);
      asm volatile("" ::: "memory");
    }
    const int mrow = m0w + i * 32 + rr;
    bf16* yp = a.Y + (size_t)mrow * a.ldy + n_out;
    bf16* prep = (EPI == 1 && a.Ypre) ? a.Ypre + (size_t)mrow * a.ldy + n_out : nullptr;
#pragma unroll
    for (int pp = 0; pp < 4; ++pp) {
      if (FULL || mrow + pp * 8 < a.M) {
        bf16x8 v = cur[pp];
        if constexpr (EPI == 1) {
          if (prep) st_stream(reinterpret_cast<bf16x8*>(prep + (size_t)pp * 8 * a.ldy), v);
          v = gelu8(v, HAS_RS ? prs[pp] : 1.f);
        } else if constexpr (EPI == 2) {
          v = gelu_grad_mul8(v, sd[pp], HAS_RS ? prs[pp] : 1.f);
        }
        if constexpr (EPI == 3) {
          const float4 o0 = {bf2f(v[0]) + rf[pp][0].x, bf2f(v[1]) + rf[pp][0].y, bf2f(v[2]) + rf[pp][0].z, bf2f(v[3]) + rf[pp][0].w};
          const float4 o1 = {bf2f(v[4]) + rf[pp][1].x, bf2f(v[5]) + rf[pp][1].y, bf2f(v[6]) + rf[pp][1].z, bf2f(v[7]) + rf[pp][1].w};
          float* op = y32 + (size_t)(mrow + pp * 8) * a.ldy + n_out;
          *reinterpret_cast<float4*>(op) = o0;
          *reinterpret_cast<float4*>(op + 4) = o1;
          if (a.Y) {
            v[0] = f2bf(o0.x); v[1] = f2bf(o0.y); v[2] = f2bf(o0.z); v[3] = f2bf(o0.w);
            v[4] = f2bf(o1.x); v[5] = f2bf(o1.y); v[6] = f2bf(o1.z); v[7] = f2bf(o1.w);
            st_out(reinterpret_cast<bf16x8*>(yp + (size_t)pp * 8 * a.ldy), v, (a.act & 0x2000) != 0);
          }
        } else {
          if constexpr (HAS_R) {
#pragma unroll
            for (int e = 0; e < 8; ++e) v[e] = f2bf(bf2f(v[e]) + bf2f(sd[pp][e]));
          }
          st_out(reinterpret_cast<bf16x8*>(yp + (size_t)pp * 8 * a.ldy), v, (a.act & 0x2000) != 0);
        }
      }
      if constexpr (HAS_R || EPI == 2) __builtin_amdgcn_sched_barrier(0);
      if (i + 1 < TM) {
        asm volatile("" ::: "memory");
        cur[pp] = read_pass(pp);
        if constexpr (EPI == 3) load_r32(i + 1, pp);
        else if constexpr (PREF) { sd[pp] = sdn[pp]; prs[pp] = prsn[pp]; }
        else load_side_pass(i + 1, pp, sd[pp], prs[pp]);
      }
    }
  }
}

template <int BN>
__device__ __forceinline__ void stage_bias(const GemmArgs& a, float* bias_s, int tn0) {
  if (a.bias && threadIdx.x < BN / 4) {
    const int n = min(tn0 + (int)threadIdx.x * 4, a.N - 4);
    *reinterpret_cast<float4*>(bias_s + threadIdx.x * 4) = *reinterpret_cast<const float4*>(a.bias + n);
  }
  asm volatile("s_waitcnt vmcnt(0)" ::: "memory");
}

}
```

### fiber_amd/csrc/norm.hip

```cpp
#include "common.h"

namespace {

struct MergeMap {
  int H, W, C;
  __device__ __forceinline__ size_t src(int row, int col) const {
    const int Wh = W >> 1, per = (H >> 1) * Wh;
    const int b = row / per, ij = row - b * per, i = ij / Wh, j = ij - i * Wh;
    const int s = col / C, c = col - s * C;
    return ((size_t)(b * H + 2 * i + (s & 1)) * W + 2 * j + (s >> 1)) * C + c;
  }
};

template <int LPR>
__device__ __forceinline__ float group_sum(float v) {
#pragma unroll
  for (int o = LPR / 2; o > 0; o >>= 1) v += __shfl_xor(v, o);
  return v;
}

template <int LPR, int NV, bool MERGE, bool X32, int U>
__global__ __launch_bounds__(256) void ln_fwd_kernel(const void* __restrict__ xv, const float* __restrict__ gamma,
                                                     const float* __restrict__ beta, bf16* __restrict__ y,
                                                     float* __restrict__ y32, float* __restrict__ mean,
                                                     float* __restrict__ rstd, int rows, int C, float eps, MergeMap mm) {
  const bf16* x = reinterpret_cast<const bf16*>(xv);
  const float* xf = reinterpret_cast<const float*>(xv);
  constexpr int RPW = 64 / LPR;
  const int lane = threadIdx.x & 63, wave = threadIdx.x >> 6;
  const int sub = lane / LPR, gl = lane % LPR;
  const int nvec = C >> 3;
  float g[NV][8], b[NV][8];
#pragma unroll
  for (int i = 0; i < NV; ++i) {
    const int vi = gl + i * LPR;
#pragma unroll
    for (int e = 0; e < 8; ++e) { g[i][e] = vi < nvec ? gamma[vi * 8 + e] : 0.f; b[i][e] = vi < nvec ? beta[vi * 8 + e] : 0.f; }
  }
  for (int base = (blockIdx.x * 4 + wave) * (U * RPW); base < rows; base += gridDim.x * 4 * (U * RPW)) {
    float v[U][NV][8];
    bf16x8 raw[U][NV];
#pragma unroll
    for (int u = 0; u < U; ++u) {
      const int row = base + u * RPW + sub;
#pragma unroll
      for (int i = 0; i < NV; ++i) {
        const int vi = gl + i * LPR;
        if (row < rows && vi < nvec) {
          const size_t off = MERGE ? mm.src(row, vi * 8) : (size_t)row * C + vi * 8;
          if constexpr (X32) {
            const float4 t0 = *reinterpret_cast<const float4*>(xf + off), t1 = *reinterpret_cast<const float4*>(xf + off + 4);
            v[u][i][0] = t0.x; v[u][i][1] = t0.y; v[u][i][2] = t0.z; v[u][i][3] = t0.w;
            v[u][i][4] = t1.x; v[u][i][5] = t1.y; v[u][i][6] = t1.z; v[u][i][7] = t1.w;
          } else {
            raw[u][i] = *reinterpret_cast<const bf16x8*>(x + off);
          }
        } else {
          if constexpr (X32) {
#pragma unroll
            for (int e = 0; e < 8; ++e) v[u][i][e] = 0.f;
          } else {
#pragma unroll
            for (int e = 0; e < 8; ++e) raw[u][i][e] = (bf16)0.f;
          }
        }
      }
    }
    float mu[U], rs[U];
#pragma unroll
    for (int u = 0; u < U; ++u) {
      float s = 0.f;
#pragma unroll
      for (int i = 0; i < NV; ++i)
#pragma unroll
        for (int e = 0; e < 8; ++e) {
          if constexpr (!X32) v[u][i][e] = bf2f(raw[u][i][e]);
          s += v[u][i][e];
        }
      mu[u] = s;
    }
#pragma unroll
    for (int u = 0; u < U; ++u) mu[u] = group_sum<LPR>(mu[u]) / C;
#pragma unroll
    for (int u = 0; u < U; ++u) {
      float q = 0.f;
#pragma unroll
      for (int i = 0; i < NV; ++i)
        if (gl + i * LPR < nvec)
#pragma unroll
          for (int e = 0; e < 8; ++e) { const float d = v[u][i][e] - mu[u]; q += d * d; }
      rs[u] = q;
    }
#pragma unroll
    for (int u = 0; u < U; ++u) rs[u] = rsqrtf(group_sum<LPR>(rs[u]) / C + eps);
#pragma unroll
    for (int u = 0; u < U; ++u) {
      const int row = base + u * RPW + sub;
      const bool rok = row < rows;
      if (rok && gl == 0) { mean[row] = mu[u]; rstd[row] = rs[u]; }
#pragma unroll
      for (int i = 0; i < NV; ++i) {
        const int vi = gl + i * LPR;
        if (rok && vi < nvec) {
          bf16x8 o;
          float of[8];
#pragma unroll
          for (int e = 0; e < 8; ++e) { of[e] = (v[u][i][e] - mu[u]) * rs[u] * g[i][e] + b[i][e]; o[e] = f2bf(of[e]); }
          *reinterpret_cast<bf16x8*>(y + (size_t)row * C + vi * 8) = o;
          if (y32) {
            float* yp = y32 + (size_t)row * C + vi * 8;
            *reinterpret_cast<float4*>(yp) = float4{of[0], of[1], of[2], of[3]};
            *reinterpret_cast<float4*>(yp + 4) = float4{of[4], of[5], of[6], of[7]};
          }
        }
      }
    }
  }
}

template <int LPR, int NV, bool MERGE, bool X32, int U>
__global__ __launch_bounds__(256) void ln_bwd_kernel(const bf16* __restrict__ dy, const void* __restrict__ xv,
                                                     const float* __restrict__ gamma, const float* __restrict__ mean,
                                                     const float* __restrict__ rstd, const bf16* __restrict__ dres,
                                                     bf16* __restrict__ dx,
                                                     float* __restrict__ part , int rows, int C,
                                                     MergeMap mm) {
  constexpr int RPW = 64 / LPR;
  const bf16* x = reinterpret_cast<const bf16*>(xv);
  const float* xf = reinterpret_cast<const float*>(xv);
  const int lane = threadIdx.x & 63, wave = threadIdx.x >> 6;
  const int sub = lane / LPR, gl = lane % LPR;
  const int nvec = C >> 3;
  float ag[NV][8], ab[NV][8], g[NV][8];
#pragma unroll
  for (int i = 0; i < NV; ++i) {
    const int vi = gl + i * LPR;
#pragma unroll
    for (int e = 0; e < 8; ++e) { ag[i][e] = 0.f; ab[i][e] = 0.f; g[i][e] = vi < nvec ? gamma[vi * 8 + e] : 0.f; }
  }
  for (int base = (blockIdx.x * 4 + wave) * (U * RPW); base < rows; base += gridDim.x * 4 * (U * RPW)) {
    float xh[U][NV][8], dg[U][NV][8];
    bf16x8 rx[U][NV], rd[U][NV], rr[U][NV];
    float mu[U], rs[U];
#pragma unroll
    for (int u = 0; u < U; ++u) {
      const int row = base + u * RPW + sub;
      const bool rok = row < rows;
      mu[u] = rok ? mean[row] : 0.f;
      rs[u] = rok ? rstd[row] : 0.f;
#pragma unroll
      for (int i = 0; i < NV; ++i) {
        const int vi = gl + i * LPR;
        if (rok && vi < nvec) {
          const size_t off = MERGE ? mm.src(row, vi * 8) : (size_t)row * C + vi * 8;
          if constexpr (X32) {
            const float4 t0 = *reinterpret_cast<const float4*>(xf + off), t1 = *reinterpret_cast<const float4*>(xf + off + 4);
            xh[u][i][0] = t0.x; xh[u][i][1] = t0.y; xh[u][i][2] = t0.z; xh[u][i][3] = t0.w;
            xh[u][i][4] = t1.x; xh[u][i][5] = t1.y; xh[u][i][6] = t1.z; xh[u][i][7] = t1.w;
          } else {
            rx[u][i] = *reinterpret_cast<const bf16x8*>(x + off);
          }
          rd[u][i] = *reinterpret_cast<const bf16x8*>(dy + (size_t)row * C + vi * 8);
          if (dres) rr[u][i] = *reinterpret_cast<const bf16x8*>(dres + off);
        } else {
#pragma unroll
          for (int e = 0; e < 8; ++e) {
            rd[u][i][e] = (bf16)0.f;
            if constexpr (X32) xh[u][i][e] = mu[u]; else rx[u][i][e] = (bf16)0.f;
          }
        }
      }
    }
    float s1[U], s2[U];
#pragma unroll
    for (int u = 0; u < U; ++u) {
      s1[u] = 0.f; s2[u] = 0.f;
#pragma unroll
      for (int i = 0; i < NV; ++i)
#pragma unroll
        for (int e = 0; e < 8; ++e) {
          const float d = bf2f(rd[u][i][e]);
          const float xv1 = X32 ? xh[u][i][e] : bf2f(rx[u][i][e]);
          xh[u][i][e] = (xv1 - mu[u]) * rs[u];
          dg[u][i][e] = d * g[i][e];
          s1[u] += dg[u][i][e];
          s2[u] += dg[u][i][e] * xh[u][i][e];
          ag[i][e] += d * xh[u][i][e];
          ab[i][e] += d;
        }
    }
#pragma unroll
    for (int u = 0; u < U; ++u) { s1[u] = group_sum<LPR>(s1[u]) / C; s2[u] = group_sum<LPR>(s2[u]) / C; }
#pragma unroll
    for (int u = 0; u < U; ++u) {
      const int row = base + u * RPW + sub;
#pragma unroll
      for (int i = 0; i < NV; ++i) {
        const int vi = gl + i * LPR;
        if (row < rows && vi < nvec) {
          const size_t off = MERGE ? mm.src(row, vi * 8) : (size_t)row * C + vi * 8;
          bf16x8 o;
          if (dres) {
#pragma unroll
            for (int e = 0; e < 8; ++e) o[e] = f2bf(rs[u] * (dg[u][i][e] - s1[u] - xh[u][i][e] * s2[u]) + bf2f(rr[u][i][e]));
          } else {
#pragma unroll
            for (int e = 0; e < 8; ++e) o[e] = f2bf(rs[u] * (dg[u][i][e] - s1[u] - xh[u][i][e] * s2[u]));
          }
          *reinterpret_cast<bf16x8*>(dx + off) = o;
        }
      }
    }
  }
#pragma unroll
  for (int i = 0; i < NV; ++i)
#pragma unroll
    for (int e = 0; e < 8; ++e)
#pragma unroll
      for (int o = 32; o >= LPR; o >>= 1) { ag[i][e] += __shfl_xor(ag[i][e], o); ab[i][e] += __shfl_xor(ab[i][e], o); }
  __shared__ float red[2 * LPR * NV * 8];
  constexpr int CP = LPR * NV * 8;
#pragma unroll 1
  for (int w = 0; w < 4; ++w) {
    if (wave == w && sub == 0) {
#pragma unroll
      for (int i = 0; i < NV; ++i) {
        const int vi = gl + i * LPR;
#pragma unroll
        for (int e = 0; e < 8; ++e) {
          if (w == 0) { red[vi * 8 + e] = ag[i][e]; red[CP + vi * 8 + e] = ab[i][e]; }
          else { red[vi * 8 + e] += ag[i][e]; red[CP + vi * 8 + e] += ab[i][e]; }
        }
      }
    }
    __syncthreads();
  }
  float* my = part + (size_t)blockIdx.x * 2 * C;
  for (int c = threadIdx.x; c < C; c += 256) { my[c] = red[c]; my[C + c] = red[CP + c]; }
}

__global__ __launch_bounds__(1024) void ln_bwd_reduce_kernel(const float* __restrict__ part, float* __restrict__ dgamma,
                                                             float* __restrict__ dbeta, int nrows, int C) {
  __shared__ float red[64][17];
  const int cl = threadIdx.x & 15, rl = threadIdx.x >> 4;
  const int col = blockIdx.x * 16 + cl;
  float s = 0.f;
  if (col < 2 * C)
    for (int r = rl; r < nrows; r += 64) s += part[(size_t)r * 2 * C + col];
  red[rl][cl] = s;
  __syncthreads();
#pragma unroll
  for (int o = 32; o > 0; o >>= 1) {
    if (rl < o) red[rl][cl] += red[rl + o][cl];
    __syncthreads();
  }
  if (rl == 0 && col < 2 * C) (col < C ? dgamma[col] : dbeta[col - C]) = red[0][cl];
}

#ifndef LN_UF
#define LN_UF 4
#endif
#ifndef LN_UB
#define LN_UB 4
#endif
#define LN_DISPATCH(KERNEL, LN_U, LN_U2, ...)                                                             \
  do {                                                                                      \
    const int nvec = C >> 3;                                                                \
    if (nvec <= 8) KERNEL(8, 1, LN_U, __VA_ARGS__);                                         \
    else if (nvec <= 16) KERNEL(16, 1, LN_U, __VA_ARGS__);                                  \
    else if (nvec <= 32) KERNEL(32, 1, LN_U, __VA_ARGS__);                                  \
    else if (nvec <= 64) KERNEL(64, 1, LN_U, __VA_ARGS__);                                  \
    else if (nvec <= 128) KERNEL(64, 2, LN_U2, __VA_ARGS__);                                \
    else if (nvec <= 256) KERNEL(64, 4, 1, __VA_ARGS__);                                    \
    else if (nvec <= 384) KERNEL(64, 6, 1, __VA_ARGS__);    \
    else if (nvec <= 512) {                                                                 \
       \
      if constexpr (MERGE) return FIBER_EINVAL; else KERNEL(64, 8, 1, __VA_ARGS__);         \
    } else return FIBER_EINVAL;                                                             \
  } while (0)

inline int rows_per_wave(int C) {
  const int nvec = C >> 3;
  const int u = nvec <= 64 ? LN_UF : nvec <= 128 ? (LN_UF > 1 ? 2 : 1) : 1;
  return u * (nvec <= 8 ? 8 : nvec <= 16 ? 4 : nvec <= 32 ? 2 : 1);
}

template <bool MERGE, bool X32>
int launch_fwd(const void* x, const float* g, const float* b, bf16* y, float* y32, float* mean, float* rstd, int rows, int C,
               float eps, MergeMap mm, hipStream_t st) {
  const int need = cdiv(rows, 4 * rows_per_wave(C));
  static const int div = getenv("FIBER_LN_FWD_DIV") ? atoi(getenv("FIBER_LN_FWD_DIV")) : 4;
  const int want = cdiv(need, div < 1 ? 1 : div);
  const int grid = want < 4096 ? want : 4096;
#define FWD(LPR, NV, UU, ...) hipLaunchKernelGGL((ln_fwd_kernel<LPR, NV, MERGE, X32, UU>), dim3(grid), dim3(256), 0, st, __VA_ARGS__)
  LN_DISPATCH(FWD, LN_UF, (LN_UF > 1 ? 2 : 1), x, g, b, y, y32, mean, rstd, rows, C, eps, mm);
#undef FWD
  FIBER_CHECK_LAUNCH();
  return FIBER_OK;
}

template <bool MERGE, bool X32>
int launch_bwd(const bf16* dy, const void* x, const float* g, const float* mean, const float* rstd, const bf16* dres,
               bf16* dx, float* dgamma, float* dbeta, float* ws, int grid, int rows, int C, MergeMap mm, hipStream_t st) {
#define BWD(LPR, NV, UU, ...) hipLaunchKernelGGL((ln_bwd_kernel<LPR, NV, MERGE, X32, UU>), dim3(grid), dim3(256), 0, st, __VA_ARGS__)
  LN_DISPATCH(BWD, LN_UB, 1, dy, x, g, mean, rstd, dres, dx, ws, rows, C, mm);
#undef BWD
  FIBER_CHECK_LAUNCH();
  hipLaunchKernelGGL(ln_bwd_reduce_kernel, dim3(cdiv(2 * C, 16)), dim3(1024), 0, st, ws, dgamma, dbeta, grid, C);
  FIBER_CHECK_LAUNCH();
  return FIBER_OK;
}

}

extern "C" int fiber_layernorm_bwd_grid(int rows) {
  int g = cdiv(rows, 4 * 16);
  return g < 1 ? 1 : (g > 1024 ? 1024 : g);
}

extern "C" int fiber_layernorm_fwd_bf16(const void* x, const float* gamma, const float* beta, void* y, float* mean,
                                        float* rstd, int rows, int C, float eps, hipStream_t stream) {
  if (rows <= 0) return FIBER_OK;
  if (C & 7) return FIBER_EINVAL;
  return launch_fwd<false, false>(x, gamma, beta, (bf16*)y, nullptr, mean, rstd, rows, C, eps, MergeMap{0, 0, 0}, stream);
}

extern "C" int fiber_layernorm_fwd_stream(const void* x, const float* gamma, const float* beta, void* y, float* y32, float* mean,
                                          float* rstd, int rows, int C, float eps, int flags, hipStream_t stream) {
  if (rows <= 0) return FIBER_OK;
  if (C & 7) return FIBER_EINVAL;
  if (flags & 1) return launch_fwd<false, true>(x, gamma, beta, (bf16*)y, y32, mean, rstd, rows, C, eps, MergeMap{0, 0, 0}, stream);
  return launch_fwd<false, false>(x, gamma, beta, (bf16*)y, y32, mean, rstd, rows, C, eps, MergeMap{0, 0, 0}, stream);
}

extern "C" int fiber_layernorm_bwd_bf16(const void* dy, const void* x, const float* gamma, const float* mean,
                                        const float* rstd, const void* dres, void* dx, float* dgamma, float* dbeta,
                                        float* workspace, int rows, int C, hipStream_t stream) {
  if (rows <= 0) return FIBER_OK;
  if (C & 7) return FIBER_EINVAL;
  return launch_bwd<false, false>((const bf16*)dy, x, gamma, mean, rstd, (const bf16*)dres, (bf16*)dx, dgamma, dbeta, workspace,
                                  fiber_layernorm_bwd_grid(rows), rows, C, MergeMap{0, 0, 0}, stream);
}

extern "C" int fiber_layernorm_bwd_stream(const void* dy, const void* x, const float* gamma, const float* mean,
                                          const float* rstd, const void* dres, void* dx, float* dgamma, float* dbeta,
                                          float* workspace, int rows, int C, int flags, hipStream_t stream) {
  if (rows <= 0) return FIBER_OK;
  if (C & 7) return FIBER_EINVAL;
  if (flags & 1)
    return launch_bwd<false, true>((const bf16*)dy, x, gamma, mean, rstd, (const bf16*)dres, (bf16*)dx, dgamma, dbeta, workspace,
                                   fiber_layernorm_bwd_grid(rows), rows, C, MergeMap{0, 0, 0}, stream);
  return launch_bwd<false, false>((const bf16*)dy, x, gamma, mean, rstd, (const bf16*)dres, (bf16*)dx, dgamma, dbeta, workspace,
                                  fiber_layernorm_bwd_grid(rows), rows, C, MergeMap{0, 0, 0}, stream);
}

extern "C" int fiber_patch_merge_ln_fwd_bf16(const void* x, const float* gamma, const float* beta, void* y, float* mean,
                                             float* rstd, int B, int H, int W, int C, float eps, hipStream_t stream) {
  if ((C & 7) || (H & 1) || (W & 1)) return FIBER_EINVAL;
  if (B <= 0) return FIBER_OK;
  return launch_fwd<true, false>(x, gamma, beta, (bf16*)y, nullptr, mean, rstd, B * (H / 2) * (W / 2), 4 * C, eps,
                                 MergeMap{H, W, C}, stream);
}

extern "C" int fiber_patch_merge_ln_fwd_stream(const void* x, const float* gamma, const float* beta, void* y, float* mean,
                                               float* rstd, int B, int H, int W, int C, float eps, int flags, hipStream_t stream) {
  if ((C & 7) || (H & 1) || (W & 1)) return FIBER_EINVAL;
  if (B <= 0) return FIBER_OK;
  const int rows = B * (H / 2) * (W / 2);
  if (flags & 1) return launch_fwd<true, true>(x, gamma, beta, (bf16*)y, nullptr, mean, rstd, rows, 4 * C, eps, MergeMap{H, W, C}, stream);
  return launch_fwd<true, false>(x, gamma, beta, (bf16*)y, nullptr, mean, rstd, rows, 4 * C, eps, MergeMap{H, W, C}, stream);
}

extern "C" int fiber_patch_merge_ln_bwd_bf16(const void* dy, const void* x, const float* gamma, const float* mean,
                                             const float* rstd, void* dx, float* dgamma, float* dbeta, float* workspace,
                                             int B, int H, int W, int C, hipStream_t stream) {
  if ((C & 7) || (H & 1) || (W & 1)) return FIBER_EINVAL;
  if (B <= 0) return FIBER_OK;
  const int rows = B * (H / 2) * (W / 2);
  return launch_bwd<true, false>((const bf16*)dy, x, gamma, mean, rstd, nullptr, (bf16*)dx, dgamma, dbeta, workspace,
                                 fiber_layernorm_bwd_grid(rows), rows, 4 * C, MergeMap{H, W, C}, stream);
}

extern "C" int fiber_patch_merge_ln_bwd_stream(const void* dy, const void* x, const float* gamma, const float* mean,
                                               const float* rstd, void* dx, float* dgamma, float* dbeta, float* workspace,
                                               int B, int H, int W, int C, int flags, hipStream_t stream) {
  if ((C & 7) || (H & 1) || (W & 1)) return FIBER_EINVAL;
  if (B <= 0) return FIBER_OK;
  const int rows = B * (H / 2) * (W / 2);
  if (flags & 1)
    return launch_bwd<true, true>((const bf16*)dy, x, gamma, mean, rstd, nullptr, (bf16*)dx, dgamma, dbeta, workspace,
                                  fiber_layernorm_bwd_grid(rows), rows, 4 * C, MergeMap{H, W, C}, stream);
  return launch_bwd<true, false>((const bf16*)dy, x, gamma, mean, rstd, nullptr, (bf16*)dx, dgamma, dbeta, workspace,
                                 fiber_layernorm_bwd_grid(rows), rows, 4 * C, MergeMap{H, W, C}, stream);
}
```

### fiber_amd/lib.py

```python
import ctypes as C
import os

import torch

_HERE = os.path.dirname(os.path.abspath(__file__))
LIB_PATH = os.environ.get("FIBER_HIP_LIB") or os.path.join(_HERE, "libfiber_hip.so")

P, I, F, L, U64 = C.c_void_p, C.c_int, C.c_float, C.c_long, C.c_uint64

SIGNATURES = {
    "fiber_gemm_nt_bf16": [P, P, P, P, P, P, P, I, P, I, P, I, I, I, I, I, I, I, I],
    "fiber_gemm_tn_bf16": [P, P, P, P, P, I, I, I, I, I, P, I, F],
    "fiber_gemm_tn_slabs_bf16": [P, P, P, P, P, I, I, I, I, I, P, I, F],
    "fiber_gemm_tn_rowmap_bf16": [P, P, P, P, P, I, I, I, I, I, P, I, F, P],
    "fiber_tn_fold_multi": [P, I, I],
    "fiber_ln_mlp_fwd_bf16": [P, P, P, P, P, P, P, P, I, I, I, F],
    "fiber_ln_mlp_bwd_bf16": [P, P, P, P, P, P, P, P, P, P, I, I, I, F],
    "fiber_layernorm_fwd_bf16": [P, P, P, P, P, P, I, I, F],
    "fiber_layernorm_bwd_bf16": [P, P, P, P, P, P, P, P, P, P, I, I],
    "fiber_layernorm_fwd_stream": [P, P, P, P, P, P, P, I, I, F, I],
    "fiber_layernorm_bwd_stream": [P, P, P, P, P, P, P, P, P, P, I, I, I],
    "fiber_patch_merge_ln_fwd_stream": [P, P, P, P, P, P, I, I, I, I, F, I],
    "fiber_patch_merge_ln_bwd_stream": [P, P, P, P, P, P, P, P, P, I, I, I, I, I],
    "fiber_stream_add": [P, I, P, P, P, P, L, F, U64, F, U64, P, P, P, L],
    "fiber_stream_add_bwd": [P, P, P, P, L, F, U64, F, U64, P, P, P, P, P, L],
    "fiber_cast_f32_bf16": [P, P, L],
    "fiber_patch_merge_ln_fwd_bf16": [P, P, P, P, P, P, I, I, I, I, F],
    "fiber_patch_merge_ln_bwd_bf16": [P, P, P, P, P, P, P, P, P, I, I, I, I],
    "fiber_window_attn_fwd_bf16": [P, P, P, P, I, I, I, I, I, I, I, I],
    "fiber_window_attn_bwd_bf16": [P, P, P, P, P, P, P, P, P, P, P, I, I, I, I, I, I, I, I],
    "fiber_mha_fwd_bf16": [P, P, P, P, P, P, I, I, I, I, I, I, I, I, I, F, F, U64, P],
    "fiber_mha_causal_fwd_bf16": [P, P, P, P, P, P, I, I, I, I, I, I, I, I, I, F, F, U64, P],
    "fiber_mha_bwd_bf16": [P, P, P, P, P, P, P, P, P, P, P, I, I, I, I, I, I, I, I, I, I, I, I, I, F, F, U64, P],
    "fiber_mha_causal_bwd_bf16": [P, P, P, P, P, P, P, P, P, P, P, I, I, I, I, I, I, I, I, I, I, I, I, I, F, F, U64, P],
    "fiber_roberta_embed_fwd": [P, P, P, P, P, P, P, P, P, P, I, I, I, I, F, F, U64, P],
    "fiber_roberta_embed_bwd": [P, P, P, P, P, P, P, P, P, P, P, P, P, P, P, I, I, I, I, F, U64, P],
    "fiber_im2col_patch4": [P, P, I, I, I],
    "fiber_im2col_patch4_pair": [P, P, P, P, I, I, I],
    "fiber_gelu_bwd_bf16": [P, P, P, L],
    "fiber_gelu_bwd_colsum_bf16": [P, P, P, P, P, I, I],
    "fiber_scale_add_bf16": [P, P, P, F, P, L],
    "fiber_dot_bf16": [P, P, P, P, L],
    "fiber_colsum_bf16": [P, P, P, I, I, I],
    "fiber_fold_rows_f32": [P, P, I, I],
    "fiber_dropout_bf16": [P, P, L, F, U64, P],
    "fiber_droppath_scale_f32": [P, I, F, U64, P],
    "fiber_rowscale_add_bf16": [P, P, P, P, L, L],
    "fiber_rowscale_colsum_bf16": [P, P, P, P, P, I, I, I],
    "fiber_ce_fwd_bf16": [P, P, P, P, P, I, I, L],
    "fiber_colsum_labelled_bf16": [P, P, P, P, I, I, L],
    "fiber_ce_bwd_bf16": [P, P, P, P, P, I, I, L],
    "fiber_adamw_multi_f32": [P, P, P, I, F, F, F, F, F, I, P],
    "fiber_resize_bicubic_norm_u8": [P, I, P, P, P, I, I, P, P],
    "fiber_mlm_mask_i64": [P, P, P, L, U64, C.c_uint, I, I, I, I],
    "fiber_transpose_multi_bf16": [P, I, I],
    "fiber_rowperm_cast_multi_bf16": [P, I, I],
    "fiber_dcn_gather_bf16": [P, P, P, P, I, I, I, I, I, I, I, I, I, I],
    "fiber_dcn_scatter_bf16": [P, P, P, P, P, P, P, I, I, I, I, I, I, I, I, I, I],
    "fiber_dcn_dx_bf16": [P, P, P, P, P, I, I, I, I, I, I, I, I, I, I],
    "fiber_ground_fwd_bf16": [P, P, P, P, P, P, P, P, P, I, I, I, I, F, F],
    "fiber_ground_bwd_bf16": [P, P, P, P, P, P, P, P, P, P, P, I, I, I, I, F, F],
    "fiber_det_scores_f32": [P, P, P, P, P, I, I, I, I, F, I],
    "fiber_det_decode_f32": [P, P, P, P, P, P, P, P, P, I, I, I, I, I, I, I, F],
    "fiber_det_nms_mask": [P, P, P, P, I, I, F],
    "fiber_det_nms_select": [P, P, P, P, P, P, P, P, P, P, I, I, I],
    "fiber_atss_candidates_f32": [P, P, I, P, P, P, P, I, I, I, I],
    "fiber_atss_resolve_f32": [P, P, P, P, P, P, I, I, I, I],
    "fiber_atss_finalize_f32": [P, P, P, P, P, P, P, P, P, P, I, I, I, I],
    "fiber_atss_loss_fwd_f32": [P, P, P, P, P, P, P, I, I, I, I, I],
    "fiber_atss_loss_bwd_f32": [P, P, P, P, P, P, P, P, I, I, I, I],
    "fiber_dropblock_mask_u8": [P, I, U64, P, F, I, P, P, I, I, I],
    "fiber_fpn_merge_fwd_bf16": [P, P, P, P, P, P, I, I, I, I, I, I],
    "fiber_fpn_merge_bwd_bf16": [P, P, P, P, P, P, I, I, I, I, I, I],
}
PLAIN = {"fiber_layernorm_bwd_grid": [I], "fiber_window_attn_bwd_slices": [I, I], "fiber_window_attn_colsum_rows": [I, I, I], "fiber_colsum_slabs": [I, I], "fiber_tn_fold_blocks": [I, I, I, I], "fiber_colsum_labelled_slabs": [I], "fiber_gemm_row_tile": [I, I, I], "fiber_gemm_tn_splits": [I, I, I],
         "fiber_adamw_chunk": [], "fiber_resample_ksize": [I, I], "fiber_dcn_dx_workspace": [I, I, I, I, I, I, I],
         "fiber_roberta_embed_bwd_workspace": [I, I, I], "fiber_ground_workspace": [I, I, I], "fiber_det_max_candidates": [],
         "fiber_atss_num_candidates": [P, I, I], "fiber_atss_loss_rows": [I, I]}

PLAIN_LONG = {"fiber_dcn_dx_workspace", "fiber_roberta_embed_bwd_workspace", "fiber_ground_workspace"}
_lib = None


class FiberHipError(RuntimeError):
    pass


def load():
    global _lib
    if _lib is not None:
        return _lib
    if not os.path.isfile(LIB_PATH):
        raise FiberHipError(f"{LIB_PATH} not built: run `python -c 'import __graft_entry__ as g; g.build()'` "
                            "or `make -C fiber_amd/csrc` (there is no fallback path)")
    lib = C.CDLL(LIB_PATH)
    for name, args in SIGNATURES.items():
        fn = getattr(lib, name)
        fn.argtypes = args + [P]
        fn.restype = I
    for name, args in PLAIN.items():
        fn = getattr(lib, name)
        fn.argtypes = args
        fn.restype = L if name in PLAIN_LONG else I
    _lib = lib
    return lib


def exported_symbols():
    return list(SIGNATURES) + list(PLAIN)


def ptr(t):
    if t is None:
        return None
    if not t.is_cuda:
        raise FiberHipError("fiber_amd ops need HIP device tensors (no CPU fallback)")
    return t.data_ptr()


_TRACE = [] if os.environ.get("FIBER_TRACE_LAUNCHES") else None


def call(name, *args):
    lib = load()
    cur = torch.cuda.current_stream()
    stream = cur.cuda_stream
    rc = getattr(lib, name)(*args, stream)
    if _TRACE is not None:
        ev = torch.cuda.Event()
        ev.record(cur)
        _TRACE.append((stream, name, [a for a in args if isinstance(a, (int, float))], ev))
# ... 8 lines not shown
```

### fiber_amd/modules/swin_transformer.py

```python
import torch
import torch.nn as nn

from .. import ops

DIM_TEXT = 768
NUM_FUSE_BLOCK = 6


def _rel_pos_index(ws):
    r = torch.arange(ws)
    rr, cc = torch.meshgrid(r, r, indexing="ij")
    rr, cc = rr.reshape(-1), cc.reshape(-1)
    return (rr[:, None] - rr[None, :] + ws - 1) * (2 * ws - 1) + (cc[:, None] - cc[None, :] + ws - 1)


def _shift_mask(H, W, ws, shift):
    def region(n):
        lab = torch.zeros(n, dtype=torch.long)
        lab[n - ws:n - shift] = 1
        lab[n - shift:] = 2
        return lab
    lab = region(H)[:, None] * 3 + region(W)[None, :]
    lab = lab.view(H // ws, ws, W // ws, ws).permute(0, 2, 1, 3).reshape(-1, ws * ws)
    diff = lab[:, None, :] - lab[:, :, None]
# ... 12 lines not shown
    def __init__(self, img_size=224, patch_size=4, in_chans=3, embed_dim=96):
        super().__init__()
        assert patch_size == 4 and in_chans == 3, "the HIP im2col kernel covers the 4x4 / RGB patch embed FIBER uses"
        self.img_size = (img_size, img_size)
        self.grid_size = (img_size // patch_size, img_size // patch_size)
        self.num_patches = self.grid_size[0] * self.grid_size[1]
        self.proj = nn.Conv2d(in_chans, embed_dim, kernel_size=patch_size, stride=patch_size)
        self.norm = nn.LayerNorm(embed_dim)

    def forward(self, img):
        x = ops.patch_embed_proj(img, self.proj.weight, self.proj.bias)
        return ops.layernorm(x, self.norm.weight, self.norm.bias, self.norm.eps, want_f32=ops.residual_fp32())


class WindowAttention(nn.Module):
    def __init__(self, dim, window_size, num_heads, dim_text=None):
        super().__init__()
        ws = window_size[0] if isinstance(window_size, (tuple, list)) else window_size
        self.dim, self.window_size, self.num_heads = dim, (ws, ws), num_heads
        assert dim // num_heads == 32, "Swin head_dim is 32 for every FIBER variant (kernel contract)"
        self.scale = (dim // num_heads) ** -0.5
        self.relative_position_bias_table = nn.Parameter(torch.zeros((2 * ws - 1) ** 2, num_heads))
        self.register_buffer("relative_position_index", _rel_pos_index(ws))
        self.qkv = nn.Linear(dim, dim * 3)
        self.proj = nn.Linear(dim, dim)
        nn.init.trunc_normal_(self.relative_position_bias_table, std=0.02)
        if dim_text is not None:
            self.qkv_text_i2t = nn.Linear(dim_text, dim * 2)
            self.qkv_i2t = nn.Linear(dim, dim)
            self.proj_i2t = nn.Linear(dim, dim)
            self.alpha_i2t = nn.Parameter(torch.Tensor([0]))
            self.norm_i2t_i = nn.LayerNorm(dim)

    def forward(self, u, res, shift, shortcut=None, y=None, y_mask=None, rowscale=None, rowscale_value=None):
        B, L, C = u.shape
        H, W = res
        ws = self.window_size[0]
        if ops.head_major_supported(ws):
            qkv = ops.linear_qkv_head_major(u, self.qkv.weight, self.qkv.bias, self.num_heads)
            o = ops.window_attention(qkv, self.relative_position_bias_table, B, H, W, self.num_heads, ws, shift, head_major=True)
        else:
            qkv = ops.linear(u, self.qkv.weight, self.qkv.bias)
            o = ops.window_attention(qkv, self.relative_position_bias_table, B, H, W, self.num_heads, ws, shift)
        if y is None:
            return ops.linear(o, self.proj.weight, self.proj.bias, residual=shortcut, rowscale=rowscale, rowscale_value=rowscale_value)
        a = ops.linear(o, self.proj.weight, self.proj.bias)
        S = y.shape[1]
        assert y.shape[0] == B, "text batch must match image batch"
        kv = ops.linear(y, self.qkv_text_i2t.weight, self.qkv_text_i2t.bias).view(B * S, 2 * C)
        an, a = ops.layernorm_res(a, self.norm_i2t_i.weight, self.norm_i2t_i.bias, self.norm_i2t_i.eps)
        qi = ops.linear(an, self.qkv_i2t.weight, self.qkv_i2t.bias).view(B * L, C)
        km = y_mask.reshape(B, S) if y_mask is not None else None
        yi = ops.mha(qi, kv[:, :C], kv[:, C:], km, B, self.num_heads, self.scale)
        yi = ops.linear(yi.view(B, L, C), self.proj_i2t.weight, self.proj_i2t.bias)
        if shortcut is None:
            return ops.scale_add(a, yi, self.alpha_i2t)
        return ops.stream_add(shortcut, a, b=yi, alpha=self.alpha_i2t, rowscale=rowscale)


class SwinTransformerBlock(nn.Module):
    def __init__(self, dim, input_resolution, num_heads, window_size=7, shift_size=0, mlp_ratio=4.0, drop_path=0.0,
                 dim_text=None):
        super().__init__()
        self.dim, self.input_resolution, self.num_heads = dim, input_resolution, num_heads
        self.window_size, self.shift_size = window_size, shift_size
        if min(input_resolution) <= window_size:
            self.shift_size, self.window_size = 0, min(input_resolution)
        assert 0 <= self.shift_size < self.window_size
        self.norm1 = nn.LayerNorm(dim)
        self.attn = WindowAttention(dim, self.window_size, num_heads, dim_text)
        self.drop_path_rate = float(drop_path)
        self.norm2 = nn.LayerNorm(dim)
        self.mlp = Mlp(dim, int(dim * mlp_ratio))
        H, W = input_resolution
        self.register_buffer("attn_mask", _shift_mask(H, W, self.window_size, self.shift_size) if self.shift_size > 0 else None)

    def forward(self, x, y=None, y_mask=None):
        H, W = self.input_resolution
        B, L, C = x.shape
        assert L == H * W, "input feature has wrong size"
        dp = self.drop_path_rate if self.training else 0.0
        s1 = ops.drop_path_scale(B, dp, x.device) if dp > 0.0 else None
        s2 = ops.drop_path_scale(B, dp, x.device) if dp > 0.0 else None
        u, x = ops.layernorm_res(x, self.norm1.weight, self.norm1.bias, self.norm1.eps)
        rv = 1.0 / (1.0 - dp) if dp > 0.0 else None
        x = self.attn(u, (H, W), self.shift_size, shortcut=x, y=y, y_mask=y_mask, rowscale=s1, rowscale_value=rv)
        return ops.ln_mlp(x, self.norm2.weight, self.norm2.bias, self.norm2.eps, self.mlp.fc1.weight, self.mlp.fc1.bias,
                          self.mlp.fc2.weight, self.mlp.fc2.bias, rowscale=s2, rowscale_value=rv)


class PatchMerging(nn.Module):
    def __init__(self, input_resolution, dim):
        super().__init__()
        self.input_resolution, self.dim = input_resolution, dim
        self.reduction = nn.Linear(4 * dim, 2 * dim, bias=False)
        self.norm = nn.LayerNorm(4 * dim)

    def forward(self, x):
        H, W = self.input_resolution
        B, L, C = x.shape
        assert L == H * W and H % 2 == 0 and W % 2 == 0
        z = ops.patch_merge_ln(x, self.norm.weight, self.norm.bias, H, W, self.norm.eps)
        return ops.start_stream(ops.linear(z, self.reduction.weight))


class BasicLayer(nn.Module):
    def __init__(self, dim, input_resolution, depth, num_heads, window_size, mlp_ratio=4.0, drop_path=0.0,
                 downsample=None, dim_text=None, layer_index=0):
        super().__init__()
        self.dim, self.input_resolution, self.depth = dim, input_resolution, depth
        self.blocks = nn.ModuleList([
            SwinTransformerBlock(
                dim=dim, input_resolution=input_resolution, num_heads=num_heads, window_size=window_size,
                shift_size=0 if (i % 2 == 0) else window_size // 2, mlp_ratio=mlp_ratio,
                drop_path=drop_path[i] if isinstance(drop_path, list) else drop_path,
                dim_text=None if layer_index == 2 and i < 20 - NUM_FUSE_BLOCK else dim_text)
            for i in range(depth)])
        self.downsample = downsample(input_resolution, dim=dim) if downsample is not None else None

    def forward(self, x, y=None, y_mask=None):
        for blk in self.blocks:
            x = blk(x, y, y_mask)
        return self.downsample(x) if self.downsample is not None else x


class SwinTransformer(nn.Module):
    def __init__(self, img_size=224, patch_size=4, in_chans=3, embed_dim=96, depths=(2, 2, 6, 2), num_heads=(3, 6, 12, 24),
                 window_size=7, mlp_ratio=4.0, drop_path_rate=0.1, **kwargs):
        super().__init__()
        window_size = int(img_size / 32)
        self.num_layers = len(depths)
        self.embed_dim = embed_dim
        self.num_features = int(embed_dim * 2 ** (self.num_layers - 1))
        self.patch_embed = PatchEmbed(img_size, patch_size, in_chans, embed_dim)
        self.patch_grid = self.patch_embed.grid_size
        self.absolute_pos_embed = None
        self.pos_drop = nn.Identity()
        dpr = [v.item() for v in torch.linspace(0, drop_path_rate, sum(depths))]
        self.layers = nn.Sequential(*[
            BasicLayer(dim=int(embed_dim * 2 ** i),
                       input_resolution=(self.patch_grid[0] // 2 ** i, self.patch_grid[1] // 2 ** i),
                       depth=depths[i], num_heads=num_heads[i], window_size=window_size, mlp_ratio=mlp_ratio,
                       drop_path=dpr[sum(depths[:i]):sum(depths[:i + 1])],
                       downsample=PatchMerging if i < self.num_layers - 1 else None,
                       dim_text=DIM_TEXT if i >= 2 else None, layer_index=i)
            for i in range(self.num_layers)])
        self.norm = nn.LayerNorm(self.num_features)
        self.avgpool = nn.AdaptiveAvgPool1d(1)
        self.apply(_init_vit_weights)

    def forward_features(self, x, y=None, y_mask=None):
        x = self.patch_embed(x)
        for layer in self.layers:
            x = layer(x, y, y_mask)
        return ops.layernorm(x, self.norm.weight, self.norm.bias, self.norm.eps)

    def forward(self, x, y=None, y_mask=None):
        return self.forward_features(x, y, y_mask)


def _init_vit_weights(m):
    if isinstance(m, nn.Linear):
        nn.init.trunc_normal_(m.weight, std=0.02)
        if m.bias is not None:
            nn.init.zeros_(m.bias)
    elif isinstance(m, nn.LayerNorm):
        nn.init.zeros_(m.bias)
        nn.init.ones_(m.weight)


_ARCH = {
# ... 24 lines not shown
```

### fiber_amd/ops.py

```python
import math
import threading
import weakref

import torch

from . import lib

import os

BF16 = torch.bfloat16
_wcache = {}


def _cache_get(key, w):
    hit = _wcache.get(key)
    if hit is not None and hit[2]() is w:
        return hit
    return None


def _cache_put(key, stamp, value, w):
    _wcache[key] = (stamp, value, weakref.ref(w, lambda _r, k=key: _wcache.pop(k, None)))
_FUSED_MLP_BWD = os.environ.get("FIBER_FUSED_MLP_BWD", "auto")
_WIN_COLSUM = os.environ.get("FIBER_WIN_COLSUM", "0") == "1"
# ... 548 lines not shown
        shp = x.shape
        x2 = _c(x).view(-1, shp[-1])
        wb = bf16_weight(weight)
        need_pre = bool(act) and any(ctx.needs_input_grad[:3])
        rps = (x2.shape[0] // rowscale.numel()) if rowscale is not None else 0
        oshp = (*shp[:-1], weight.shape[0])
        if res32 is not None:
            assert residual is not None and not act
            y, y32 = gemm_nt(x2, wb, bias, None, 0, False, rowscale, rps, res32=_c(res32).view(-1, weight.shape[0]))
            pre, y32 = None, y32.view(oshp)
            ctx.mark_non_differentiable(y32)
        else:
            r2 = _c(residual).view(-1, weight.shape[0]) if residual is not None else None
            y, pre = gemm_nt(x2, wb, bias, r2, act, need_pre, rowscale, rps)
            y32 = None
        ctx.save_for_backward(x2, weight, pre, rowscale)
        ctx.act, ctx.has_bias, ctx.has_res, ctx.shp, ctx.rs_value = act, bias is not None, residual is not None, shp, rs_value
        return y.view(oshp), y32

    @staticmethod
    def backward(ctx, dy, _dy32=None):
        x2, weight, pre, rowscale = ctx.saved_tensors
        dy2 = _c(dy).view(-1, weight.shape[0])
        dres = dy if ctx.has_res else None
        db = None
        hint = _take_colsum(dy2)
        fold = not ctx.act and dy2.shape[1] % 8 == 0 and droppath_foldable(dy2.shape[0], rowscale, ctx.rs_value)
        if rowscale is not None and not fold:
            if ctx.has_bias and ctx.needs_input_grad[2] and not ctx.act and dy2.shape[1] % 8 == 0:
                dy2, db = rowscale_colsum(dy2, rowscale)
            else:
                ds = torch.empty_like(dy2)
                lib.call("fiber_rowscale_add_bf16", None, lib.ptr(dy2), lib.ptr(rowscale), lib.ptr(ds), dy2.numel(),
                         dy2.numel() // rowscale.numel())
                dy2 = ds
        if ctx.act:
            dh, db = gelu_bwd_colsum(dy2, pre)
        else:
            dh = dy2
        need_db = ctx.has_bias and ctx.needs_input_grad[2]
        if fold:
            rps = dh.shape[0] // rowscale.numel()
            dx = gemm_nt(dh, bf16_weight_t(weight), None, None, 0, False, rowscale, rps)[0].view(ctx.shp) if ctx.needs_input_grad[0] else None
            dw = db = None
            if ctx.needs_input_grad[1]:
                dw = wgrad(dh, x2, want_bias=need_db, row_mask=rowscale, scale=ctx.rs_value)
                if need_db:
                    dw, db = dw
            elif need_db:
                db = rowscale_colsum(dh, rowscale)[1]
            return dx, dw, db, dres, None, None, None, None
        dx = _dgrad(dh, weight).view(ctx.shp) if ctx.needs_input_grad[0] else None
        if need_db and db is None and hint is not None and dh is dy2:
            db = hint
        want = need_db and db is None
        dw = None
        if ctx.needs_input_grad[1]:
            dw = wgrad(dh, x2, want_bias=want)
            if want:
                dw, db = dw
        elif want:
            db = colsum(dh)
        if not need_db:
            db = None
        return dx, dw, db, dres, None, None, None, None


def linear(x, weight, bias=None, residual=None, act=None, rowscale=None, rowscale_value=None):
    N, K = weight.shape
    if (N % 8) or (K % 8):
        _note_lib_site()
        y = _LibLinear.apply(x, weight.to(BF16), bias.to(BF16) if bias is not None else None)
        if act:
            y = torch.nn.functional.gelu(y)
        assert rowscale is None
        return y + residual if residual is not None else y
    y, y32 = _Linear.apply(x, weight, bias, residual, 1 if act else 0, rowscale, rowscale_value, f32_of(residual))
    return with_f32(y, y32)


class _MLP(torch.autograd.Function):

    @staticmethod
    def forward(ctx, x, w1, b1, w2, b2, residual, rowscale, rs_value=None, res32=None):
        shp = x.shape
        x2 = _c(x).view(-1, shp[-1])
        need_bwd = any(ctx.needs_input_grad[:5])
        g, h = gemm_nt(x2, bf16_weight(w1), b1, None, 1, need_bwd)
        rps = (x2.shape[0] // rowscale.numel()) if rowscale is not None else 0
        oshp = (*shp[:-1], w2.shape[0])
        if res32 is not None:
            y, y32 = gemm_nt(g, bf16_weight(w2), b2, None, 0, False, rowscale, rps, res32=_c(res32).view(-1, w2.shape[0]))
            y32 = y32.view(oshp)
            ctx.mark_non_differentiable(y32)
        else:
            r2 = _c(residual).view(-1, w2.shape[0]) if residual is not None else None
            y, _ = gemm_nt(g, bf16_weight(w2), b2, r2, 0, False, rowscale, rps)
            y32 = None
        if need_bwd:
            ctx.save_for_backward(x2, w1, w2, h, g, rowscale)
        ctx.has_res, ctx.shp, ctx.rs_value = residual is not None, shp, rs_value
        return y.view(oshp), y32

    @staticmethod
    def backward(ctx, dy, _dy32=None):
        dres = dy if ctx.has_res else None
        if not ctx.saved_tensors:
            return (None,) * 5 + (dres, None, None, None)
        x2, w1, w2, h, g, rowscale = ctx.saved_tensors
        dy2 = _c(dy).view(-1, w2.shape[0])
        db2 = None
        C, C4 = dy2.shape[1], h.shape[1]
        fused = C % 64 == 0 and C4 % 8 == 0 and _FUSED_MLP_BWD != "0"
        fold = fused and dy2.shape[1] % 8 == 0 and droppath_foldable(dy2.shape[0], rowscale, ctx.rs_value)
        rs_arg, rps, mask, scale = None, 0, None, 1.0
        if fold:
            rs_arg, rps, mask, scale = rowscale, dy2.shape[0] // rowscale.numel(), rowscale, ctx.rs_value
        elif rowscale is not None:
            if dy2.shape[1] % 8 == 0:
                dy2, db2 = rowscale_colsum(dy2, rowscale)
            else:
                ds = torch.empty_like(dy2)
                lib.call("fiber_rowscale_add_bf16", None, lib.ptr(dy2), lib.ptr(rowscale), lib.ptr(ds), dy2.numel(),
                         dy2.numel() // rowscale.numel())
                dy2 = ds
        if fused:
            dh, _ = gemm_nt(dy2, bf16_weight_t(w2), None, None, 2, False, rs_arg, rps, aux=h)
            db1 = None
        else:
            dh, db1 = gelu_bwd_colsum(_dgrad(dy2, w2), h)
        if db2 is None:
            dw2, db2 = wgrad(dy2, g, want_bias=True, row_mask=mask, scale=scale)
        else:
            dw2 = wgrad(dy2, g)
        dx = _dgrad(dh, w1).view(ctx.shp)
        if db1 is None:
            dw1, db1 = wgrad(dh, x2, want_bias=True)
        else:
            dw1 = wgrad(dh, x2)
        return dx, dw1, db1, dw2, db2, dres, None, None, None


def mlp(x, w1, b1, w2, b2, residual=None, rowscale=None, rowscale_value=None):
    y, y32 = _MLP.apply(x, w1, b1, w2, b2, residual, rowscale, rowscale_value, f32_of(residual))
    return with_f32(y, y32)


_LN_MLP = os.environ.get("FIBER_LN_MLP", "1") != "0"
_fa_perms = {}


def _fa_perm(K, device):
    key = (K, device)
    if key not in _fa_perms:
        i = torch.arange(K, device=device)
        _fa_perms[key] = (i & ~12) | ((i & 4) << 1) | ((i & 8) >> 1)
    return _fa_perms[key]


def _fa(m16):
    return m16[:, _fa_perm(m16.shape[1], m16.device)].contiguous()


def _ln_mlp_weights(gamma, beta, w1, b1, w2):
    key = ("LNMLP", id(w1))
    stamp = tuple(_stamp(t) for t in (gamma, beta, w1, b1, w2))
    hit = _cache_get(key, w1)
    if hit is not None and hit[0] == stamp:
        return hit[1]
    with torch.no_grad():
        w1f = w1.detach().float()
        w1p16 = (w1f * gamma.detach().float()[None, :]).to(BF16)
        b1p = torch.addmv(b1.detach().float(), w1f, beta.detach().float()).contiguous()
        w2_16 = w2.detach().to(BF16)
        val = (w1p16.contiguous(), b1p, _fa(w2_16), w2_16.t().contiguous(), _fa(w1p16.t()))
    _cache_put(key, stamp, val, w1)
    return val


_LN_MLP_WIDTHS = tuple(int(v) for v in os.environ.get("FIBER_LN_MLP_WIDTHS", "128").split(",") if v)


def ln_mlp_eligible(x, C):
    return _LN_MLP and C in _LN_MLP_WIDTHS and C in (128, 256) and x.is_cuda and x.dtype == BF16 and f32_of(x) is None


class _LnMlp(torch.autograd.Function):

    @staticmethod
    def forward(ctx, x, gamma, beta, eps, w1, b1, w2, b2, rowscale, rs_value):
        shp = x.shape
        C = shp[-1]
        x2 = _c(x).view(-1, C)
        M = x2.shape[0]
        w1p, b1p, w2p, _, _ = _ln_mlp_weights(gamma, beta, w1, b1, w2)
        y = torch.empty_like(x2)
        need_bwd = any(ctx.needs_input_grad[:8])
        g = torch.empty((M, 4 * C), dtype=BF16, device=x2.device) if need_bwd else None
        rps = M // rowscale.numel() if rowscale is not None else 0
        lib.call("fiber_ln_mlp_fwd_bf16", lib.ptr(x2), lib.ptr(w1p), lib.ptr(b1p), lib.ptr(w2p), lib.ptr(b2.detach()), lib.ptr(rowscale),
                 lib.ptr(y), lib.ptr(g), M, C, rps, float(eps))
        if need_bwd:
            ctx.save_for_backward(x2, gamma, beta, w1, b1, w2, rowscale, g)
        ctx.eps, ctx.shp, ctx.rs_value = float(eps), shp, rs_value
        return y.view(shp)

    @staticmethod
    def backward(ctx, dy):
        x2, gamma, beta, w1, b1, w2, rowscale, g = ctx.saved_tensors
        M, C = x2.shape
        H = 4 * C
        dy2 = _c(dy).view(M, C)
        w1p, b1p, _, w2tp, w1tp = _ln_mlp_weights(gamma, beta, w1, b1, w2)
        dx = torch.empty_like(x2)
        dh = torch.empty((M, H), dtype=BF16, device=x2.device)
        xhat = torch.empty_like(x2)
        rps = M // rowscale.numel() if rowscale is not None else 0
        lib.call("fiber_ln_mlp_bwd_bf16", lib.ptr(x2), lib.ptr(dy2), lib.ptr(w1p), lib.ptr(b1p), lib.ptr(w2tp), lib.ptr(w1tp),
                 lib.ptr(rowscale), lib.ptr(dx), lib.ptr(dh), lib.ptr(xhat), M, C, rps, ctx.eps)
        w1f, gf, bf_ = w1.detach().float(), gamma.detach().float(), beta.detach().float()

        def unfold(dw1p, db1):
            return (dw1p * w1f).sum(0), torch.mv(w1f.t(), db1), torch.addcmul(torch.outer(db1, bf_), dw1p, gf[None, :]), db1
        dgamma, dbeta, dw1, db1 = wgrad(dh, xhat, want_bias=True, post=unfold)
        del dh, xhat
        if rowscale is None:
            dw2, db2 = wgrad(dy2, g, want_bias=True)
        elif droppath_foldable(M, rowscale, ctx.rs_value):
            dw2, db2 = wgrad(dy2, g, want_bias=True, row_mask=rowscale, scale=ctx.rs_value)
        else:
            dys, db2 = rowscale_colsum(dy2, rowscale)
            dw2 = wgrad(dys, g)
        return dx.view(ctx.shp), dgamma, dbeta, None, dw1, db1, dw2, db2, None, None


def ln_mlp(x, gamma, beta, eps, w1, b1, w2, b2, rowscale=None, rowscale_value=None):
    if ln_mlp_eligible(x, x.shape[-1]) and w1.shape[0] == 4 * x.shape[-1]:
        return _LnMlp.apply(x, gamma, beta, eps, w1, b1, w2, b2, rowscale, rowscale_value)
    v, r = layernorm_res(x, gamma, beta, eps)
    return mlp(v, w1, b1, w2, b2, residual=r, rowscale=rowscale, rowscale_value=rowscale_value)


def _ln_fwd(x2, x32, gamma, beta, eps, want_f32):
    rows, C = x2.shape
    y = torch.empty((rows, C), dtype=BF16, device=x2.device)
    y32 = torch.empty((rows, C), dtype=torch.float32, device=x2.device) if want_f32 else None
    mean = torch.empty(rows, dtype=torch.float32, device=x2.device)
    rstd = torch.empty_like(mean)
    if x32 is None and not want_f32:
        lib.call("fiber_layernorm_fwd_bf16", lib.ptr(x2), lib.ptr(gamma), lib.ptr(beta), lib.ptr(y), lib.ptr(mean), lib.ptr(rstd), rows, C, eps)
    else:
        src = x32 if x32 is not None else x2
        lib.call("fiber_layernorm_fwd_stream", lib.ptr(src), lib.ptr(gamma), lib.ptr(beta), lib.ptr(y), lib.ptr(y32), lib.ptr(mean),
                 lib.ptr(rstd), rows, C, eps, 1 if x32 is not None else 0)
    return y, y32, mean, rstd


def _ln_bwd(dy2, xs, is32, gamma, mean, rstd, dr2):
    rows, C = dy2.shape
    dx = torch.empty((rows, C), dtype=BF16, device=dy2.device)
    dg = torch.empty(C, dtype=torch.float32, device=dy2.device)
    db = torch.empty_like(dg)
    ws = torch.empty(lib.plain("fiber_layernorm_bwd_grid", rows) * 8 * C, dtype=torch.float32, device=dy2.device)
    if is32:
        lib.call("fiber_layernorm_bwd_stream", lib.ptr(dy2), lib.ptr(xs), lib.ptr(gamma), lib.ptr(mean), lib.ptr(rstd), lib.ptr(dr2),
                 lib.ptr(dx), lib.ptr(dg), lib.ptr(db), lib.ptr(ws), rows, C, 1)
    else:
        lib.call("fiber_layernorm_bwd_bf16", lib.ptr(dy2), lib.ptr(xs), lib.ptr(gamma), lib.ptr(mean), lib.ptr(rstd), lib.ptr(dr2),
                 lib.ptr(dx), lib.ptr(dg), lib.ptr(db), lib.ptr(ws), rows, C)
    return dx, dg, db


class _LayerNorm(torch.autograd.Function):

    @staticmethod
    def forward(ctx, x, gamma, beta, eps, x32=None, want_f32=False):
        C = x.shape[-1]
        x2 = _c(x).view(-1, C)
        xs = _c(x32).view(-1, C) if x32 is not None else None
        y, y32, mean, rstd = _ln_fwd(x2, xs, gamma, beta, eps, want_f32)
        ctx.save_for_backward(xs if xs is not None else x2, gamma, mean, rstd)
        ctx.is32 = xs is not None
        if y32 is not None:
            y32 = y32.view(x.shape)
            ctx.mark_non_differentiable(y32)
        return y.view(x.shape), y32

    @staticmethod
    def backward(ctx, dy, _dy32=None):
        xs, gamma, mean, rstd = ctx.saved_tensors
        dx, dg, db = _ln_bwd(_c(dy).view(xs.shape), xs, ctx.is32, gamma, mean, rstd, None)
        return dx.view(dy.shape), dg, db, None, None, None


def layernorm(x, gamma, beta, eps=1e-5, want_f32=False):
    x32 = f32_of(x)
    y, y32 = _LayerNorm.apply(x, gamma, beta, eps, x32, bool(want_f32))
    return with_f32(y, y32)


class _LayerNormRes(torch.autograd.Function):

    @staticmethod
    def forward(ctx, x, gamma, beta, eps, x32=None):
        C = x.shape[-1]
        x2 = _c(x).view(-1, C)
        xs = _c(x32).view(-1, C) if x32 is not None else None
        y, _, mean, rstd = _ln_fwd(x2, xs, gamma, beta, eps, False)
        ctx.save_for_backward(xs if xs is not None else x2, gamma, mean, rstd)
        ctx.is32 = xs is not None
        return y.view(x.shape), x2.view(x.shape)

    @staticmethod
    def backward(ctx, dy, dres):
        xs, gamma, mean, rstd = ctx.saved_tensors
        rows, C = xs.shape
        if dy is None:
            return dres, None, None, None, None
        dr2 = _c(dres).view(rows, C) if dres is not None else None
        dx, dg, db = _ln_bwd(_c(dy).view(rows, C), xs, ctx.is32, gamma, mean, rstd, dr2)
        return dx.view(dy.shape), dg, db, None, None


def layernorm_res(x, gamma, beta, eps=1e-5):
    x32 = f32_of(x)
    y, r = _LayerNormRes.apply(x, gamma, beta, eps, x32)
    return y, with_f32(r, x32)


class _PatchMergeLN(torch.autograd.Function):
    @staticmethod
    def forward(ctx, x, gamma, beta, H, W, eps, x32=None):
        B, L, C = x.shape
        xs = _c(x32) if x32 is not None else _c(x)
        rows = B * (H // 2) * (W // 2)
        y = torch.empty((B, rows // B, 4 * C), dtype=BF16, device=x.device)
        mean = torch.empty(rows, dtype=torch.float32, device=x.device)
        rstd = torch.empty_like(mean)
        if x32 is not None:
            lib.call("fiber_patch_merge_ln_fwd_stream", lib.ptr(xs), lib.ptr(gamma), lib.ptr(beta), lib.ptr(y), lib.ptr(mean), lib.ptr(rstd),
                     B, H, W, C, eps, 1)
        else:
            lib.call("fiber_patch_merge_ln_fwd_bf16", lib.ptr(xs), lib.ptr(gamma), lib.ptr(beta), lib.ptr(y), lib.ptr(mean), lib.ptr(rstd), B, H, W, C, eps)
        ctx.save_for_backward(xs, gamma, mean, rstd)
        ctx.dims, ctx.is32 = (B, H, W, C), x32 is not None
        return y

    @staticmethod
    def backward(ctx, dy):
        xs, gamma, mean, rstd = ctx.saved_tensors
        B, H, W, C = ctx.dims
        rows = B * (H // 2) * (W // 2)
        dy = _c(dy)
        dx = torch.empty(xs.shape, dtype=BF16, device=dy.device)
        dg = torch.empty(4 * C, dtype=torch.float32, device=dy.device)
        db = torch.empty_like(dg)
        ws = torch.empty(lib.plain("fiber_layernorm_bwd_grid", rows) * 8 * 4 * C, dtype=torch.float32, device=dy.device)
        if ctx.is32:
            lib.call("fiber_patch_merge_ln_bwd_stream", lib.ptr(dy), lib.ptr(xs), lib.ptr(gamma), lib.ptr(mean), lib.ptr(rstd), lib.ptr(dx),
                     lib.ptr(dg), lib.ptr(db), lib.ptr(ws), B, H, W, C, 1)
        else:
            lib.call("fiber_patch_merge_ln_bwd_bf16", lib.ptr(dy), lib.ptr(xs), lib.ptr(gamma), lib.ptr(mean), lib.ptr(rstd), lib.ptr(dx),
                     lib.ptr(dg), lib.ptr(db), lib.ptr(ws), B, H, W, C)
        return dx, dg, db, None, None, None, None


def patch_merge_ln(x, gamma, beta, H, W, eps=1e-5):
    return _PatchMergeLN.apply(x, gamma, beta, H, W, eps, f32_of(x))


class _WindowAttn(torch.autograd.Function):
    @staticmethod
    def forward(ctx, qkv, bias_table, B, H, W, heads, ws, shift, head_major):
        C = qkv.shape[-1] // 3
        qkv = _c(qkv)
        rows = B * H * W
        o = torch.empty((rows, C), dtype=BF16, device=qkv.device)
        lse = torch.empty((rows, heads), dtype=torch.float32, device=qkv.device)
        lib.call("fiber_window_attn_fwd_bf16", lib.ptr(qkv), lib.ptr(bias_table), lib.ptr(o), lib.ptr(lse), B, H, W, C, heads, ws, shift, head_major)
        ctx.save_for_backward(qkv, bias_table, o, lse)
        ctx.dims = (B, H, W, C, heads, ws, shift, head_major)
        return o.view(B, H * W, C)

    @staticmethod
    def backward(ctx, do):
        qkv, bias_table, o, lse = ctx.saved_tensors
        B, H, W, C, heads, ws, shift, head_major = ctx.dims
        do = _c(do)
        rows, N = B * H * W, ws * ws
        dqkv = torch.empty_like(qkv)
        dtab = torch.empty_like(bias_table)
        delta = torch.empty((rows, heads), dtype=torch.float32, device=do.device)
        nz = lib.plain("fiber_window_attn_bwd_slices", rows // N, heads)
        part = torch.empty(nz * heads * N * N, dtype=torch.float32, device=do.device)
        cs_rows = lib.plain("fiber_window_attn_colsum_rows", rows // N, heads, ws) if _WIN_COLSUM else 0
        csum = torch.empty(3 * C, dtype=torch.float32, device=do.device) if cs_rows else None
        cs_ws = torch.empty(cs_rows * 3 * C, dtype=torch.float32, device=do.device) if cs_rows else None
        lib.call("fiber_window_attn_bwd_bf16", lib.ptr(qkv), lib.ptr(bias_table), lib.ptr(o), lib.ptr(do), lib.ptr(lse), lib.ptr(dqkv),
                 lib.ptr(dtab), lib.ptr(delta), lib.ptr(part), lib.ptr(csum), lib.ptr(cs_ws), B, H, W, C, heads, ws, shift, head_major)
        if csum is not None:
            _offer_colsum(dqkv.view(-1, 3 * C), csum)
        return dqkv, dtab, None, None, None, None, None, None, None


def window_attention(qkv, bias_table, B, H, W, heads, ws, shift, head_major=False):
    return _WindowAttn.apply(qkv, bias_table, B, H, W, heads, ws, shift, int(head_major))


def head_major_supported(ws):
# ... 426 lines not shown
        t.fill_(v - (1 << 64) if v >= (1 << 63) else v)


def manual_seed(seed):
    _seed_state["seed"], _seed_state["ctr"], _seed_state["step"] = int(seed) & 0xFFFFFFFF, 0, None
    _seed_state["collate_ctr"] = 0
    _write_base_dev()


def set_rng_step(step):
    if _seed_state["step"] != step:
        _seed_state["step"] = step
        _seed_state["ctr"] = 0
        if _seed_state["base_dev"] is not None and not torch.cuda.is_current_stream_capturing():
            _write_base_dev()


def enable_graph_rng(device):
    if _seed_state["base_dev"] is None or _seed_state["base_dev"].device != torch.device(device):
        _seed_state["base_dev"] = torch.zeros((), dtype=torch.int64, device=device)
    _write_base_dev()
    return _seed_state["base_dev"]


def disable_graph_rng():
    _seed_state["base_dev"] = None


def seed_base_ptr():
    t = _seed_state["base_dev"]
    return None if t is None else t.data_ptr()


def next_seed():
    _seed_state["ctr"] += 1
    if _seed_state["base_dev"] is not None:
        return _seed_state["ctr"]
    return (_base_value() + _seed_state["ctr"]) & _M64


def collate_seed():
    _seed_state["collate_ctr"] = _seed_state.get("collate_ctr", 0) + 1
    hi = (_seed_state["seed"] ^ 0xC011A7E5) & 0xFFFFFFFF
    return ((hi << 32) | (_seed_state["collate_ctr"] & 0xFFFFFFFF)) & _M64


def collate_counter():
    return int(_seed_state.get("collate_ctr", 0))


def set_collate_counter(n):
    _seed_state["collate_ctr"] = int(n)


def dropout(x, p, training):
    if not training or p <= 0.0:
        return x
    return _Dropout.apply(x, float(p), next_seed())


class _RowScaleAdd(torch.autograd.Function):

    @staticmethod
    def forward(ctx, resid, x, scale):
        resid, x = _c(resid), _c(x)
        out = torch.empty_like(x)
        per = x.numel() // x.shape[0]
        lib.call("fiber_rowscale_add_bf16", lib.ptr(resid), lib.ptr(x), lib.ptr(scale), lib.ptr(out), x.numel(), per)
        ctx.save_for_backward(scale)
        return out

    @staticmethod
    def backward(ctx, dout):
        (scale,) = ctx.saved_tensors
        dout = _c(dout)
        dx = torch.empty_like(dout)
        per = dout.numel() // dout.shape[0]
        lib.call("fiber_rowscale_add_bf16", None, lib.ptr(dout), lib.ptr(scale), lib.ptr(dx), dout.numel(), per)
        return dout, dx, None


def drop_path_scale(batch, p, device):
    out = torch.empty(batch, dtype=torch.float32, device=device)
    lib.call("fiber_droppath_scale_f32", lib.ptr(out), batch, 1.0 - p, next_seed(), seed_base_ptr())
    return out


def rowscale_add(resid, x, scale):
    return _RowScaleAdd.apply(resid, x, scale)


def drop_path_add(resid, x, p, training):
    if not training or p <= 0.0:
        return add(resid, x)
    return _RowScaleAdd.apply(resid, x, drop_path_scale(x.shape[0], p, x.device))


class _RobertaEmbed(torch.autograd.Function):
    @staticmethod
    def forward(ctx, ids, word, pos_tab, type_tab, gamma, beta, pad, eps, p_drop, seed):
        B, S = ids.shape
        C = word.shape[1]
        ids = _c(ids)
        word, pos_tab, type_tab, gamma, beta = (_c(t) for t in (word, pos_tab, type_tab, gamma, beta))
        y = torch.empty((B, S, C), dtype=BF16, device=ids.device)
        pos = torch.empty((B, S), dtype=torch.int32, device=ids.device)
        mean = torch.empty(B * S, dtype=torch.float32, device=ids.device)
        rstd = torch.empty_like(mean)
        lib.call("fiber_roberta_embed_fwd", lib.ptr(ids), lib.ptr(word), lib.ptr(pos_tab), lib.ptr(type_tab), lib.ptr(gamma), lib.ptr(beta),
                 lib.ptr(y), lib.ptr(pos), lib.ptr(mean), lib.ptr(rstd), B, S, C, pad, eps, p_drop, seed, seed_base_ptr())
        ctx.save_for_backward(ids, pos, word, pos_tab, type_tab, gamma, mean, rstd)
        ctx.cfg = (B, S, C, pad, p_drop, seed, seed_base_ptr())
        return y

    @staticmethod
    def backward(ctx, dy):
        ids, pos, word, pos_tab, type_tab, gamma, mean, rstd = ctx.saved_tensors
        B, S, C, pad, p_drop, seed, base = ctx.cfg
        dy = _c(dy)
        dword, dpos, dtype = torch.zeros_like(word), torch.zeros_like(pos_tab), torch.zeros_like(type_tab)
        dg = torch.empty(C, dtype=torch.float32, device=dy.device)
        db = torch.empty_like(dg)
        ws = torch.empty(lib.plain("fiber_roberta_embed_bwd_workspace", B, S, C), dtype=torch.float32, device=dy.device)
        lib.call("fiber_roberta_embed_bwd", lib.ptr(dy), lib.ptr(ids), lib.ptr(pos), lib.ptr(word), lib.ptr(pos_tab), lib.ptr(type_tab),
                 lib.ptr(gamma), lib.ptr(mean), lib.ptr(rstd), lib.ptr(dword), lib.ptr(dpos), lib.ptr(dtype), lib.ptr(dg), lib.ptr(db),
                 lib.ptr(ws), B, S, C, pad, p_drop, seed, base)
        return None, dword, dpos, dtype, dg, db, None, None, None, None


def roberta_embed(ids, word, pos_tab, type_tab, gamma, beta, pad=1, eps=1e-5, p_drop=0.0, training=False):
    p = float(p_drop) if training else 0.0
    return _RobertaEmbed.apply(ids, word, pos_tab, type_tab, gamma, beta, pad, eps, p, next_seed() if p > 0 else 0)


class ImagePair:

    def __init__(self, img, alt, sel):
        assert img.shape == alt.shape and sel.numel() == img.shape[0]
        self.img, self.alt, self.sel = img, alt, sel.reshape(-1).to(torch.bool)
        self.shape = torch.Size((2 * img.shape[0],) + tuple(img.shape[1:]))
        self.device, self.dtype, self.is_cuda = img.device, img.dtype, img.is_cuda

    def size(self, d=None):
        return self.shape if d is None else self.shape[d]

    def tensor(self):
        return torch.cat([self.img, torch.where(self.sel.view(-1, 1, 1, 1), self.img, self.alt)], 0)


class _PatchEmbedProj(torch.autograd.Function):

    @staticmethod
    def forward(ctx, img, weight, bias, pair=None):
        Cout = weight.shape[0]
        if pair is not None:
            B, _, H, W = pair.shape
            rows = B * (H // 4) * (W // 4)
            a, b, sel = _c(pair.img.float()), _c(pair.alt.float()), pair.sel.to(torch.uint8)
            cols = torch.empty((rows, 64), dtype=BF16, device=a.device)
            lib.call("fiber_im2col_patch4_pair", lib.ptr(a), lib.ptr(b), lib.ptr(sel), lib.ptr(cols), B // 2, H, W)
            img = a
        else:
            B, _, H, W = img.shape
            img = _c(img.float())
            rows = B * (H // 4) * (W // 4)
            cols = torch.empty((rows, 64), dtype=BF16, device=img.device)
            lib.call("fiber_im2col_patch4", lib.ptr(img), lib.ptr(cols), B, H, W)
        key = ("pe", id(weight))
# ... 489 lines not shown
```

### include/fiber_hip.h

```cpp
#ifndef FIBER_HIP_H
#define FIBER_HIP_H
#include <stdint.h>
#ifdef __cplusplus
extern "C" {
#endif
typedef struct ihipStream_t* fiber_stream_t;

int fiber_gemm_nt_bf16(const void* X, const void* W, const float* bias, const void* residual, void* Y, void* Ypre,
                       const float* rowscale, int rows_per_sample, const void* aux, int ldaux, float* colpart, int M, int N,
                       int K, int ldx, int ldw, int ldy, int ldr, int act, fiber_stream_t stream);
int fiber_gemm_row_tile(int M, int N, int K);

int fiber_gemm_tn_splits(int M, int N, int K);
int fiber_gemm_tn_bf16(const void* dY, const void* X, float* dW, float* dbias, float* workspace, int M, int N, int K, int lddy,
                       int ldx, const float* row_mask, int rows_per_sample, float scale, fiber_stream_t stream);
int fiber_gemm_tn_slabs_bf16(const void* dY, const void* X, float* dW, float* dbias, float* workspace, int M, int N, int K, int lddy,
                       int ldx, const float* row_mask, int rows_per_sample, float scale, fiber_stream_t stream);
int fiber_gemm_tn_rowmap_bf16(const void* dY, const void* X, float* dW, float* dbias, float* workspace, int M, int N, int K, int lddy,
                              int ldx, const float* row_mask, int rows_per_sample, float scale, const int* row_map,
                              fiber_stream_t stream);
int fiber_tn_fold_blocks(int S, int N, int K, int has_dbias);
int fiber_tn_fold_multi(const void* table, int ndesc, int nblocks, fiber_stream_t stream);

int fiber_layernorm_fwd_bf16(const void* x, const float* gamma, const float* beta, void* y, float* mean, float* rstd, int rows,
// ... 5 lines not shown

int fiber_layernorm_fwd_stream(const void* x, const float* gamma, const float* beta, void* y, float* y32, float* mean, float* rstd,
                               int rows, int C, float eps, int flags, fiber_stream_t stream);
int fiber_layernorm_bwd_stream(const void* dy, const void* x, const float* gamma, const float* mean, const float* rstd,
                               const void* dres, void* dx, float* dgamma, float* dbeta, float* workspace, int rows, int C, int flags,
                               fiber_stream_t stream);

int fiber_patch_merge_ln_fwd_bf16(const void* x, const float* gamma, const float* beta, void* y, float* mean, float* rstd, int B,
                                  int H, int W, int C, float eps, fiber_stream_t stream);
int fiber_patch_merge_ln_bwd_bf16(const void* dy, const void* x, const float* gamma, const float* mean, const float* rstd,
                                  void* dx, float* dgamma, float* dbeta, float* workspace, int B, int H, int W, int C,
                                  fiber_stream_t stream);
int fiber_patch_merge_ln_fwd_stream(const void* x, const float* gamma, const float* beta, void* y, float* mean, float* rstd, int B,
                                    int H, int W, int C, float eps, int flags, fiber_stream_t stream);
int fiber_patch_merge_ln_bwd_stream(const void* dy, const void* x, const float* gamma, const float* mean, const float* rstd,
                                    void* dx, float* dgamma, float* dbeta, float* workspace, int B, int H, int W, int C, int flags,
                                    fiber_stream_t stream);

int fiber_ln_mlp_fwd_bf16(const void* x, const void* w1p, const float* b1p, const void* w2p, const float* b2, const float* rowscale,
                          void* y, void* g, int M, int C, int rows_per_sample, float eps, fiber_stream_t stream);
int fiber_ln_mlp_bwd_bf16(const void* x, const void* dy, const void* w1p, const float* b1p, const void* w2tp, const void* w1tp,
                          const float* rowscale, void* dx, void* dh, void* xhat, int M, int C, int rows_per_sample, float eps,
                          fiber_stream_t stream);

int fiber_window_attn_fwd_bf16(const void* qkv, const float* bias_table, void* o, float* lse, int B, int Hres, int Wres, int C,
                               int heads, int ws, int shift, int head_major, fiber_stream_t stream);
int fiber_window_attn_bwd_slices(int n_windows, int heads);
int fiber_window_attn_colsum_rows(int n_windows, int heads, int ws);
int fiber_window_attn_bwd_bf16(const void* qkv, const float* bias_table, const void* o, const void* dout, const float* lse,
                               void* dqkv, float* dbias_table, float* delta_ws, float* dbias_ws, float* dqkv_colsum,
                               float* colsum_ws, int B, int Hres, int Wres, int C, int heads, int ws, int shift, int head_major,
                               fiber_stream_t stream);

int fiber_mha_fwd_bf16(const void* q, const void* k, const void* v, const float* kmask, void* o, float* lse, int B, int heads,
                       int Lq, int Lk, int D, int ldq, int ldk, int ldv, int ldo, float scale, float p_drop, uint64_t seed,
                       const uint64_t* seed_base, fiber_stream_t stream);
int fiber_mha_bwd_bf16(const void* q, const void* k, const void* v, const float* kmask, const void* o, const void* dout,
                       const float* lse, void* dq, void* dk, void* dv, float* delta_ws, int B, int heads, int Lq, int Lk, int D,
                       int ldq, int ldk, int ldv, int ldo, int lddo, int lddq, int lddk, int lddv, float scale, float p_drop,
                       uint64_t seed, const uint64_t* seed_base, fiber_stream_t stream);
int fiber_mha_causal_fwd_bf16(const void* q, const void* k, const void* v, const float* kmask, void* o, float* lse, int B,
                              int heads, int Lq, int Lk, int D, int ldq, int ldk, int ldv, int ldo, float scale, float p_drop,
                              uint64_t seed, const uint64_t* seed_base, fiber_stream_t stream);
int fiber_mha_causal_bwd_bf16(const void* q, const void* k, const void* v, const float* kmask, const void* o, const void* dout,
                              const float* lse, void* dq, void* dk, void* dv, float* delta_ws, int B, int heads, int Lq, int Lk,
                              int D, int ldq, int ldk, int ldv, int ldo, int lddo, int lddq, int lddk, int lddv, float scale,
                              float p_drop, uint64_t seed, const uint64_t* seed_base, fiber_stream_t stream);

int fiber_roberta_embed_fwd(const int64_t* ids, const float* word, const float* pos_tab, const float* type_tab,
                            const float* gamma, const float* beta, void* y, int* pos_out, float* mean, float* rstd, int B, int S,
                            int C, int pad, float eps, float p_drop, uint64_t seed, const uint64_t* seed_base, fiber_stream_t stream);
int fiber_roberta_embed_bwd(const void* dy, const int64_t* ids, const int* pos, const float* word, const float* pos_tab,
                            const float* type_tab, const float* gamma, const float* mean, const float* rstd, float* dword,
                            float* dpos, float* dtype, float* dgamma, float* dbeta, float* workspace, int B, int S, int C, int pad,
                            float p_drop, uint64_t seed, const uint64_t* seed_base, fiber_stream_t stream);
long fiber_roberta_embed_bwd_workspace(int B, int S, int C);

int fiber_im2col_patch4(const float* img, void* cols, int B, int H, int W, fiber_stream_t stream);
int fiber_im2col_patch4_pair(const float* img, const float* alt, const unsigned char* sel, void* cols, int B, int H, int W,
                             fiber_stream_t stream);

int fiber_gelu_bwd_bf16(const void* dgelu, const void* h_pre, void* dh, long n, fiber_stream_t stream);
int fiber_gelu_bwd_colsum_bf16(const void* dgelu, const void* h_pre, void* dh, float* db, float* workspace, int M, int N,
                               fiber_stream_t stream);
int fiber_scale_add_bf16(const void* a, const void* b, const float* alpha, float mult, void* out, long n, fiber_stream_t stream);
int fiber_dot_bf16(const void* a, const void* b, float* out, float* workspace, long n, fiber_stream_t stream);
int fiber_colsum_slabs(int M, int N);
int fiber_colsum_bf16(const void* x, float* out, float* workspace, int M, int N, int ld, fiber_stream_t stream);
int fiber_fold_rows_f32(const float* part, float* out, int rows, int N, fiber_stream_t stream);
int fiber_dropout_bf16(const void* x, void* y, long n, float p, uint64_t seed, const uint64_t* seed_base, fiber_stream_t stream);
int fiber_droppath_scale_f32(float* out, int n, float keep, uint64_t seed, const uint64_t* seed_base, fiber_stream_t stream);
int fiber_rowscale_add_bf16(const void* r, const void* x, const float* scale, void* out, long n, long per_sample,
                            fiber_stream_t stream);
int fiber_stream_add(const void* res, int res_kind, const void* a, const void* b, const float* alpha, const float* rowscale,
                     long per_sample, float p_a, uint64_t seed_a, float p_b, uint64_t seed_b, const uint64_t* seed_base,
                     float* out32, void* out16, long n, fiber_stream_t stream);
int fiber_stream_add_bwd(const void* dy, const void* b, const float* alpha, const float* rowscale, long per_sample, float p_a,
                         uint64_t seed_a, float p_b, uint64_t seed_b, const uint64_t* seed_base, void* da, void* db, float* dalpha,
                         float* workspace, long n, fiber_stream_t stream);
int fiber_cast_f32_bf16(const float* x, void* y, long n, fiber_stream_t stream);
int fiber_rowscale_colsum_bf16(const void* x, const float* scale, void* y, float* db, float* workspace, int M, int N,
                               int rows_per_sample, fiber_stream_t stream);

int fiber_ce_fwd_bf16(const void* logits, const long long* labels, float* loss, float* lse, int* pred, int rows, int V,
                      long long ignore_index, fiber_stream_t stream);
int fiber_ce_bwd_bf16(const void* logits, const long long* labels, const float* lse, const float* scale, void* dlogits, int rows,
                      int V, long long ignore_index, fiber_stream_t stream);
int fiber_colsum_labelled_slabs(int rows);
int fiber_colsum_labelled_bf16(const void* x, const long long* labels, float* out, float* workspace, int rows, int V,
                               long long ignore_index, fiber_stream_t stream);

int fiber_adamw_chunk(void);
int fiber_adamw_multi_f32(const long long* table, const long long* numel, const int* chunks, int nchunks, float lr,
                          float weight_decay, float beta1, float beta2, float eps, int step, const float* hyper,
                          fiber_stream_t stream);
int fiber_transpose_multi_bf16(const void* table, int ndesc, int ntiles, fiber_stream_t stream);
int fiber_rowperm_cast_multi_bf16(const void* table, int ndesc, int ntiles, fiber_stream_t stream);
int fiber_resample_ksize(int in_size, int out_size);
int fiber_resize_bicubic_norm_u8(const void* descs, int n, int* coef, void* tmp, float* out, int S, int max_h, const float* mean,
                                 const float* std, fiber_stream_t stream);
int fiber_mlm_mask_i64(const long long* ids, long long* ids_mlm, long long* labels, long n, unsigned long long seed,
                       unsigned p_select, int mask_id, int vocab, int special_lo, int special_hi, fiber_stream_t stream);

int fiber_dcn_gather_bf16(const void* x, const float* offset, const float* mask, void* cols, int B, int H, int W, int C, int Ho,
                          int Wo, int kh, int kw, int stride, int pad, fiber_stream_t stream);
int fiber_dcn_scatter_bf16(const void* dcols, const void* x, const float* offset, const float* mask, float* dx, float* doffset,
                           float* dmask, int B, int H, int W, int C, int Ho, int Wo, int kh, int kw, int stride, int pad,
                           fiber_stream_t stream);
long fiber_dcn_dx_workspace(int B, int H, int W, int C, int Ho, int Wo, int stride);
int fiber_dcn_dx_bf16(const void* dcols, const float* offset, const float* mask, void* dx, float* workspace, int B, int H, int W,
                      int C, int Ho, int Wo, int kh, int kw, int stride, int pad, fiber_stream_t stream);

long fiber_ground_workspace(int B, int A, int T);
int fiber_ground_fwd_bf16(const void* X, const void* P, const float* tbias, const float* log_scale, const unsigned char* target,
                          const unsigned char* text_mask, float* logits, float* loss, float* workspace, int B, int A, int T, int C,
                          float alpha, float gamma, fiber_stream_t stream);
int fiber_ground_bwd_bf16(const void* X, const void* P, const float* tbias, const float* log_scale, const unsigned char* target,
                          const unsigned char* text_mask, const float* g, void* ds, float* dtbias, float* dlog_scale, float* workspace,
                          int B, int A, int T, int C, float alpha, float gamma, fiber_stream_t stream);

int fiber_det_max_candidates(void);
int fiber_det_scores_f32(const float* logits, const float* centerness, const int* class_ptr, const int* tok_idx, float* out, int B, int A,
                         int T, int C, float pre_nms_thresh, int agg_max, fiber_stream_t stream);
int fiber_det_decode_f32(const float* topk_val, const long long* topk_idx, const float* bbox_reg, const float* anchors,
                         const float* image_sizes, float* boxes, float* scores, int* labels, int* source, int B, int k, int A, int C, int N,
                         int offset, int level, float min_size, fiber_stream_t stream);
int fiber_det_nms_mask(const float* boxes, const float* scores, const int* labels, unsigned long long* mask, int B, int N, float nms_thresh,
                       fiber_stream_t stream);
int fiber_det_nms_select(const float* boxes, const float* scores, const int* labels, const int* source, const unsigned long long* mask,
                         float* out_boxes, float* out_scores, int* out_labels, int* out_source, int* out_count, int B, int N, int D,
                         fiber_stream_t stream);

int fiber_atss_num_candidates(const int* level_off, int L, int topk);
int fiber_atss_candidates_f32(const float* anchors, const int* level_off, int L, const float* gt_boxes, const int* num_gt, int* cand_idx,
                              float* cand_iou, int B, int Gmax, int A, int topk, fiber_stream_t stream);
int fiber_atss_resolve_f32(const float* anchors, const float* gt_boxes, const int* num_gt, const int* cand_idx, const float* cand_iou,
                           unsigned long long* key, int B, int Gmax, int A, int K, fiber_stream_t stream);
int fiber_atss_finalize_f32(const float* anchors, const float* gt_boxes, const int* gt_labels, const unsigned char* positive_map,
                            const unsigned long long* key, int* matched, int* labels, float* reg_targets, unsigned char* token_targets,
                            int* num_pos, int B, int Gmax, int A, int T, fiber_stream_t stream);
int fiber_atss_loss_rows(int B, int A_level);
int fiber_atss_loss_fwd_f32(const float* bbox_reg, const float* centerness, const float* anchors, const int* labels,
                            const float* reg_targets, float* part, float* ctr_targets, int B, int A, int A_level, int offset, int row0,
                            fiber_stream_t stream);
int fiber_atss_loss_bwd_f32(const float* bbox_reg, const float* centerness, const float* anchors, const int* labels,
                            const float* reg_targets, const float* g, float* d_bbox_reg, float* d_centerness, int B, int A, int A_level,
                            int offset, fiber_stream_t stream);

int fiber_dropblock_mask_u8(unsigned char* seeds, int draw, uint64_t seed, const uint64_t* seed_base, float gamma, int block,
                            unsigned char* keep, int* kept, int B, int H, int W, fiber_stream_t stream);
int fiber_fpn_merge_fwd_bf16(const void* lateral, const void* coarse, const unsigned char* keep, const int* kept, void* inner_out,
                             void* dropped_out, int B, int H, int W, int C, int Hc, int Wc, fiber_stream_t stream);
int fiber_fpn_merge_bwd_bf16(const void* d_inner, const void* d_dropped, const unsigned char* keep, const int* kept, void* d_lateral_out,
                             void* d_coarse_out, int B, int H, int W, int C, int Hc, int Wc, fiber_stream_t stream);

#ifdef __cplusplus
}
#endif
#endif
```

Baseline: 1001 images/s.

## Compact DropPath-dropped samples out of residual branch compute

Adds a DropPath compaction path. Samples whose drop-path scale is zero are removed before the branch: layernorm gathers only kept rows, the branch runs on the compacted batch, and the output GEMM scatters results back with residual and rowscale in its epilogue. Dropped samples get their residual copied straight through. The backward uses matching gather and scatter kernels. Which samples to keep is worked out on the host by replaying the hash, which costs some host work per block, adds extra small kernels, and makes branch batch sizes vary from step to step.

```diff
diff --git a/fiber_amd/csrc/elementwise.hip b/fiber_amd/csrc/elementwise.hip
--- a/fiber_amd/csrc/elementwise.hip
+++ b/fiber_amd/csrc/elementwise.hip
@@ -116,9 +116,10 @@
   if (gc < N) out[(size_t)blockIdx.y * N + gc] = t;
 }
 
-__global__ __launch_bounds__(256) void rowscale_colsum_kernel(const bf16* __restrict__ x, const float* __restrict__ scale,
-                                                              bf16* __restrict__ y, float* __restrict__ out, int M, int N,
-                                                              int rows_per_block, int rows_per_sample) {
+template <bool GATHER>
+__device__ __forceinline__ void rowscale_colsum_body(const bf16* __restrict__ x, const float* __restrict__ scale,
+                                                     bf16* __restrict__ y, float* __restrict__ out, int M, int N,
+                                                     int rows_per_block, int rows_per_sample, const int* __restrict__ kept) {
   __shared__ float red[8][32 * 8 + 1];
   const int cv = threadIdx.x & 31, rl = threadIdx.x >> 5;
   const int col = (blockIdx.x * 32 + cv) * 8;
@@ -132,15 +133,19 @@
       for (int e = 0; e < 8; ++e) { o[e] = f2bf(sc * bf2f(a[e])); s[e] += bf2f(o[e]); }
       *reinterpret_cast<bf16x8*>(y + (size_t)r * N + col) = o;
     };
+    auto src = [&](int r) {
+      if constexpr (GATHER) { const int j = r / rows_per_sample; return (size_t)(kept[j] * rows_per_sample + (r - j * rows_per_sample)); }
+      else return (size_t)r;
+    };
     int r = r0 + rl;
     for (; r + 24 < r1; r += 32) {
-      const bf16x8 a0 = *reinterpret_cast<const bf16x8*>(x + (size_t)r * N + col);
-      const bf16x8 a1 = *reinterpret_cast<const bf16x8*>(x + (size_t)(r + 8) * N + col);
-      const bf16x8 a2 = *reinterpret_cast<const bf16x8*>(x + (size_t)(r + 16) * N + col);
-      const bf16x8 a3 = *reinterpret_cast<const bf16x8*>(x + (size_t)(r + 24) * N + col);
+      const bf16x8 a0 = *reinterpret_cast<const bf16x8*>(x + src(r) * N + col);
+      const bf16x8 a1 = *reinterpret_cast<const bf16x8*>(x + src(r + 8) * N + col);
+      const bf16x8 a2 = *reinterpret_cast<const bf16x8*>(x + src(r + 16) * N + col);
+      const bf16x8 a3 = *reinterpret_cast<const bf16x8*>(x + src(r + 24) * N + col);
       one(r, a0); one(r + 8, a1); one(r + 16, a2); one(r + 24, a3);
     }
-    for (; r < r1; r += 8) one(r, *reinterpret_cast<const bf16x8*>(x + (size_t)r * N + col));
+    for (; r < r1; r += 8) one(r, *reinterpret_cast<const bf16x8*>(x + src(r) * N + col));
   }
 #pragma unroll
   for (int e = 0; e < 8; ++e) red[rl][cv * 8 + e] = s[e];
@@ -151,6 +156,18 @@
   for (int r = 0; r < 8; ++r) t += red[r][c];
   const int gc = blockIdx.x * 256 + c;
   if (gc < N) out[(size_t)blockIdx.y * N + gc] = t;
+}
+
+__global__ __launch_bounds__(256) void rowscale_colsum_kernel(const bf16* __restrict__ x, const float* __restrict__ scale,
+                                                              bf16* __restrict__ y, float* __restrict__ out, int M, int N,
+                                                              int rows_per_block, int rows_per_sample) {
+  rowscale_colsum_body<false>(x, scale, y, out, M, N, rows_per_block, rows_per_sample, nullptr);
+}
+__global__ __launch_bounds__(256) void rowscale_colsum_gather_kernel(const bf16* __restrict__ x, const float* __restrict__ scale,
+                                                                     bf16* __restrict__ y, float* __restrict__ out, int M, int N,
+                                                                     int rows_per_block, int rows_per_sample,
+                                                                     const int* __restrict__ kept) {
+  rowscale_colsum_body<true>(x, scale, y, out, M, N, rows_per_block, rows_per_sample, kept);
 }
 
 __global__ __launch_bounds__(256) void colsum_fold_kernel(const float* __restrict__ part, float* __restrict__ out, int slabs, int N) {
@@ -202,6 +219,40 @@
   }
 }
 
+__global__ __launch_bounds__(256) void droppath_map_kernel(const float* __restrict__ scale, int* __restrict__ kept,
+                                                           int* __restrict__ rank, float* __restrict__ cscale, int n) {
+  __shared__ int cnt[256];
+  const int per = (n + 255) / 256, b0 = min((int)threadIdx.x * per, n), b1 = min(b0 + per, n);
+  int c = 0;
+  for (int b = b0; b < b1; ++b) c += scale[b] != 0.f;
+  cnt[threadIdx.x] = c;
+  __syncthreads();
+  if (threadIdx.x == 0) {
+    int run = 0;
+    for (int t = 0; t < 256; ++t) { const int v = cnt[t]; cnt[t] = run; run += v; }
+  }
+  __syncthreads();
+  int j = cnt[threadIdx.x];
+  for (int b = b0; b < b1; ++b) {
+    const float sc = scale[b];
+    if (sc != 0.f) { kept[j] = b; cscale[j] = sc; rank[b] = j; ++j; }
+    else rank[b] = -1;
+  }
+  __syncthreads();
+  if (threadIdx.x == 255) cnt[0] = j;
+  __syncthreads();
+  for (int q = cnt[0] + threadIdx.x; q < n; q += 256) { kept[q] = 0; cscale[q] = 0.f; }
+}
+
+__global__ __launch_bounds__(256) void copy_dropped_kernel(const bf16* __restrict__ x, bf16* __restrict__ y,
+                                                           const int* __restrict__ rank, size_t vec_per_sample) {
+  const int b = blockIdx.y;
+  if (rank[b] >= 0) return;
+  const bf16x8* xp = reinterpret_cast<const bf16x8*>(x) + (size_t)b * vec_per_sample;
+  bf16x8* yp = reinterpret_cast<bf16x8*>(y) + (size_t)b * vec_per_sample;
+  for (size_t i = blockIdx.x * (size_t)256 + threadIdx.x; i < vec_per_sample; i += (size_t)gridDim.x * 256) yp[i] = xp[i];
+}
+
 __global__ __launch_bounds__(256) void rowscale_add_kernel(const bf16* __restrict__ r, const bf16* __restrict__ x,
                                                            const float* __restrict__ scale, bf16* __restrict__ out,
                                                            size_t nvec, size_t vec_per_sample) {
@@ -457,6 +508,41 @@
     hipLaunchKernelGGL(colsum_fold_kernel, dim3(cdiv(N, 16)), dim3(256), 0, stream, workspace, db, gy, N);
     FIBER_CHECK_LAUNCH();
   }
+  return FIBER_OK;
+}
+
+extern "C" int fiber_rowscale_colsum_gather_bf16(const void* x, const float* scale, const int* kept, void* y, float* db, float* workspace,
+                                                 int M, int N, int rows_per_sample, hipStream_t stream) {
+  if (M <= 0 || N <= 0) return FIBER_OK;
+  if ((N & 7) || rows_per_sample <= 0 || M % rows_per_sample || !kept || fiber_misaligned(16, x, y)) return FIBER_EINVAL;
+  const int gx = cdiv(N, 256);
+  const int gy0 = fiber_colsum_slabs(M, N);
+  const int rpb = cdiv(M, gy0), gy = cdiv(M, rpb);
+  if (gy > 1 && !workspace) return FIBER_EINVAL;
+  hipLaunchKernelGGL(rowscale_colsum_gather_kernel, dim3(gx, gy), dim3(256), 0, stream, (const bf16*)x, scale, (bf16*)y,
+                     gy > 1 ? workspace : db, M, N, rpb, rows_per_sample, kept);
+  FIBER_CHECK_LAUNCH();
+  if (gy > 1) {
+    hipLaunchKernelGGL(colsum_fold_kernel, dim3(cdiv(N, 16)), dim3(256), 0, stream, workspace, db, gy, N);
+    FIBER_CHECK_LAUNCH();
+  }
+  return FIBER_OK;
+}
+
+extern "C" int fiber_droppath_map_i32(const float* scale, int* kept, int* rank, float* cscale, int n, hipStream_t stream) {
+  if (n <= 0) return FIBER_OK;
+  hipLaunchKernelGGL(droppath_map_kernel, dim3(1), dim3(256), 0, stream, scale, kept, rank, cscale, n);
+  FIBER_CHECK_LAUNCH();
+  return FIBER_OK;
+}
+
+extern "C" int fiber_copy_dropped_bf16(const void* x, void* y, const int* rank, int samples, long per_sample, hipStream_t stream) {
+  if (samples <= 0 || per_sample <= 0) return FIBER_OK;
+  if ((per_sample & 7) || !rank || fiber_misaligned(16, x, y)) return FIBER_EINVAL;
+  const size_t vps = (size_t)per_sample / 8;
+  const unsigned gx = (unsigned)(vps / 1024 < 1 ? 1 : vps / 1024 > 64 ? 64 : vps / 1024);
+  hipLaunchKernelGGL(copy_dropped_kernel, dim3(gx, samples), dim3(256), 0, stream, (const bf16*)x, (bf16*)y, rank, vps);
+  FIBER_CHECK_LAUNCH();
   return FIBER_OK;
 }
 
diff --git a/fiber_amd/csrc/gemm.hip b/fiber_amd/csrc/gemm.hip
--- a/fiber_amd/csrc/gemm.hip
+++ b/fiber_amd/csrc/gemm.hip
@@ -151,8 +151,8 @@
   }
 }
 
-template <int BM, int BN, int WM, int WN, int NS, int EPI, bool HAS_R, bool HAS_RS>
-__global__ __launch_bounds__(64 * WM * WN) void gemm_nt_glds_kernel(GemmArgs a) {
+template <int BM, int BN, int WM, int WN, int NS, int EPI, bool HAS_R, bool HAS_RS, bool MAP>
+__device__ __forceinline__ void gemm_nt_glds_body(const GemmArgs& a) {
   constexpr int NT = 64 * WM * WN;
   constexpr int WTM = BM / WM, WTN = BN / WN;
   constexpr int TM = WTM / 32, TN = WTN / 32;
@@ -279,9 +279,18 @@
   }
 
   if (tm0 + BM <= a.M && tn0 + BN <= a.N)
-    tile_epilogue<BM, BN, WM, WN, 1, EPI, HAS_R, HAS_RS, true>(a, acc, smem, bias_s, tm0, tn0);
+    tile_epilogue<BM, BN, WM, WN, 1, EPI, HAS_R, HAS_RS, true, false, MAP>(a, acc, smem, bias_s, tm0, tn0);
   else
-    tile_epilogue<BM, BN, WM, WN, 1, EPI, HAS_R, HAS_RS, false>(a, acc, smem, bias_s, tm0, tn0);
+    tile_epilogue<BM, BN, WM, WN, 1, EPI, HAS_R, HAS_RS, false, false, MAP>(a, acc, smem, bias_s, tm0, tn0);
+}
+
+template <int BM, int BN, int WM, int WN, int NS, int EPI, bool HAS_R, bool HAS_RS>
+__global__ __launch_bounds__(64 * WM * WN) void gemm_nt_glds_kernel(GemmArgs a) {
+  gemm_nt_glds_body<BM, BN, WM, WN, NS, EPI, HAS_R, HAS_RS, false>(a);
+}
+template <int BM, int BN, int WM, int WN, int NS>
+__global__ __launch_bounds__(64 * WM * WN) void gemm_nt_glds_scatter_kernel(GemmArgs a) {
+  gemm_nt_glds_body<BM, BN, WM, WN, NS, 0, true, true, true>(a);
 }
 
 template <int WM, int WN, int EPI, bool HAS_R, bool HAS_RS>
@@ -418,8 +427,8 @@
   }
 }
 
-template <int EPI, bool HAS_R, bool HAS_RS, bool TRACE = false>
-__global__ __launch_bounds__(512) void gemm_nt_q8_kernel(GemmArgs a) {
+template <int EPI, bool HAS_R, bool HAS_RS, bool TRACE, bool MAP>
+__device__ __forceinline__ void gemm_nt_q8_body(const GemmArgs& a) {
   constexpr int BM = 256, BN = 256, WN = 4;
   constexpr int WTM = 128, WTN = 64, TM = 4, TN = 2;
   constexpr int STAGE = (BM + BN) * BK;
@@ -649,9 +658,9 @@
     if constexpr (TRACE) t0 = __builtin_amdgcn_s_memtime();
     if (n0w >= a.N) {
     } else if (tm0 + BM <= a.M)
-      wave_epilogue<TM, EPI, HAS_R, HAS_RS, true>(a, acc, cw, tm0 + wm * WTM, tn0 + wn * WTN);
+      wave_epilogue<TM, EPI, HAS_R, HAS_RS, true, MAP>(a, acc, cw, tm0 + wm * WTM, tn0 + wn * WTN);
     else
-      wave_epilogue<TM, EPI, HAS_R, HAS_RS, false>(a, acc, cw, tm0 + wm * WTM, tn0 + wn * WTN);
+      wave_epilogue<TM, EPI, HAS_R, HAS_RS, false, MAP>(a, acc, cw, tm0 + wm * WTM, tn0 + wn * WTN);
     mark(16);
   }
   if (keep_stagger && wm == 0) { __builtin_amdgcn_s_barrier(); asm volatile("" ::: "memory"); }
@@ -665,6 +674,14 @@
       o[19] = (float)T;
     }
   }
+}
+
+template <int EPI, bool HAS_R, bool HAS_RS, bool TRACE = false>
+__global__ __launch_bounds__(512) void gemm_nt_q8_kernel(GemmArgs a) {
+  gemm_nt_q8_body<EPI, HAS_R, HAS_RS, TRACE, false>(a);
+}
+__global__ __launch_bounds__(512) void gemm_nt_q8_scatter_kernel(GemmArgs a) {
+  gemm_nt_q8_body<0, true, true, false, true>(a);
 }
 
 constexpr bool q8_ok(int epi, bool r, bool rs) { return (epi == 0 && (!r || rs)) || (epi == 1 && !r) || epi == 2 || (epi == 3 && rs); }
@@ -728,6 +745,16 @@
   } else if (p.family == kRing256x128) hipLaunchKernelGGL((gemm_nt_glds_kernel<256, 128, 4, 2, 3, EPI, R, RS>), grid, dim3(512), 0, stream, a);
   else if (p.family == kRing128) hipLaunchKernelGGL((gemm_nt_glds_kernel<128, 128, 2, 2, 2, EPI, R, RS>), grid, dim3(256), 0, stream, a);
   else hipLaunchKernelGGL((gemm_nt_glds_kernel<64, 64, 2, 2, 2, EPI, R, RS>), grid, dim3(256), 0, stream, a);
+  return FIBER_OK;
+}
+
+static int launch_nt_scatter(const GemmPlan& p, const GemmArgs& a, hipStream_t stream) {
+  const dim3 grid(p.grid);
+  if (p.family == kQ8) hipLaunchKernelGGL(gemm_nt_q8_scatter_kernel, grid, dim3(512), 0, stream, a);
+  else if (p.family == kRing256x128) hipLaunchKernelGGL((gemm_nt_glds_scatter_kernel<256, 128, 4, 2, 3>), grid, dim3(512), 0, stream, a);
+  else if (p.family == kRing128) hipLaunchKernelGGL((gemm_nt_glds_scatter_kernel<128, 128, 2, 2, 2>), grid, dim3(256), 0, stream, a);
+  else if (p.family == kRing64) hipLaunchKernelGGL((gemm_nt_glds_scatter_kernel<64, 64, 2, 2, 2>), grid, dim3(256), 0, stream, a);
+  else return FIBER_EINVAL;
   return FIBER_OK;
 }
 
@@ -782,4 +809,20 @@
   FIBER_CHECK_LAUNCH();
   return FIBER_OK;
 }
+
+extern "C" int fiber_gemm_nt_scatter_bf16(const void* X, const void* W, const float* bias, const void* residual, void* Y,
+                                          const float* rowscale, const int* kept, int rows_per_sample, int M, int N, int K, int ldx,
+                                          int ldw, int ldy, int ldr, hipStream_t stream) {
+  if (M <= 0 || N <= 0 || K <= 0) return FIBER_OK;
+  if (!residual || !rowscale || !kept || rows_per_sample <= 0 || (rows_per_sample & 7) || M % rows_per_sample) return FIBER_EINVAL;
+  if ((K & 63) || (N & 7) || (ldx & 7) || (ldw & 7) || (ldy & 7) || (ldr & 7)) return FIBER_EINVAL;
+  GemmArgs a{(const bf16*)X, (const bf16*)W, bias, (const bf16*)residual, (bf16*)Y, nullptr, rowscale,
+             nullptr, nullptr, M, N, K, ldx, ldw, ldy, ldr, 0, rows_per_sample, 0, kept};
+  if ((size_t)M * N * 2 > ((size_t)256 << 20)) a.act |= 0x2000;
+  const GemmPlan plan = gemm_plan(M, N, K, ldy, ldr, true, true, false, 0);
+  const int rc = launch_nt_scatter(plan, a, stream);
+  if (rc != FIBER_OK) return rc;
+  FIBER_CHECK_LAUNCH();
+  return FIBER_OK;
+}
 #endif
diff --git a/fiber_amd/csrc/gemm_epilogue.h b/fiber_amd/csrc/gemm_epilogue.h
--- a/fiber_amd/csrc/gemm_epilogue.h
+++ b/fiber_amd/csrc/gemm_epilogue.h
@@ -11,7 +11,13 @@
   const bf16* aux;
   float* colpart;
   int M, N, K, ldx, ldw, ldy, ldr, act, rows_per_sample, ldaux;
+  const int* kept;
 };
+
+__device__ __forceinline__ int map_row(const GemmArgs& a, int m) {
+  const int mc = min(m, a.M - 1), j = mc / a.rows_per_sample;
+  return a.kept[j] * a.rows_per_sample + (mc - j * a.rows_per_sample);
+}
 
 __device__ __forceinline__ int swz(int row, int chunk) { return (row * 8 + (chunk ^ ((row >> 1) & 7))) * 8; }
 
@@ -31,7 +37,7 @@
   }
 }
 
-template <int BM, int BN, int WM, int WN, int ROUNDS, int EPI, bool HAS_R, bool HAS_RS, bool FULL, bool RAWBAR = false>
+template <int BM, int BN, int WM, int WN, int ROUNDS, int EPI, bool HAS_R, bool HAS_RS, bool FULL, bool RAWBAR = false, bool MAP = false>
 __device__ __forceinline__ void tile_epilogue(const GemmArgs& a, f32x16 (&acc)[BM / WM / 32][BN / WN / 32], bf16* Cs,
                                               const float* bias_s, int tm0, int tn0) {
   constexpr int NT = 64 * WM * WN;
@@ -60,7 +66,15 @@
     const int mbase = tm0 + h * HM + erow;
     bf16x8 side[SIDE ? NPH : 1];
     float prs[((EPI == 1 || EPI == 2) && HAS_RS) ? NPH : 1];
-    if constexpr (SIDE) {
+    int prow[MAP ? NPH : 1];
+    if constexpr (MAP) {
+      static_assert(EPI == 0 && HAS_R && HAS_RS, "the scatter form exists for the DropPath residual epilogue only");
+#pragma unroll
+      for (int pp = 0; pp < NPH; ++pp) prow[pp] = map_row(a, mbase + pp * RPP);
+#pragma unroll
+      for (int pp = 0; pp < NPH; ++pp)
+        if (FULL || (mbase + pp * RPP < a.M && col_ok)) side[pp] = *reinterpret_cast<const bf16x8*>(sidep + (size_t)prow[pp] * sideld + n_out);
+    } else if constexpr (SIDE) {
       const bf16* sp = sidep + (size_t)mbase * sideld + n_out;
 #pragma unroll
       for (int pp = 0; pp < NPH; ++pp)
@@ -136,7 +150,8 @@
 #pragma unroll
             for (int e = 0; e < 8; ++e) v[e] = f2bf(bf2f(v[e]) + bf2f(side[pp][e]));
           }
-          st_out(reinterpret_cast<bf16x8*>(yp + pp * ystep), v, (a.act & 0x2000) != 0);
+          if constexpr (MAP) st_out(reinterpret_cast<bf16x8*>(a.Y + (size_t)prow[pp] * a.ldy + n_out), v, (a.act & 0x2000) != 0);
+          else st_out(reinterpret_cast<bf16x8*>(yp + pp * ystep), v, (a.act & 0x2000) != 0);
           if constexpr (EPI == 2) {
 #pragma unroll
             for (int e = 0; e < 8; ++e) csum[e] += bf2f(v[e]);
@@ -175,7 +190,7 @@
   }
 }
 
-template <int TM, int EPI, bool HAS_R, bool HAS_RS, bool FULL>
+template <int TM, int EPI, bool HAS_R, bool HAS_RS, bool FULL, bool MAP = false>
 __device__ __forceinline__ void wave_epilogue(const GemmArgs& a, f32x16 (&acc)[TM][2], bf16* cw, int m0w, int n0w) {
   int lane = __builtin_amdgcn_mbcnt_hi(~0u, __builtin_amdgcn_mbcnt_lo(~0u, 0u));
   asm volatile("" : "+v"(lane));
@@ -206,9 +221,15 @@
     const int row = pp * 8 + rr;
     return *reinterpret_cast<const bf16x8*>(rbase + pp * 8 * 64 + ((rc ^ ((row >> 1) & 7)) << 3));
   };
+  auto pass_row = [&](int i, int pp) { return map_row(a, m0w + i * 32 + pp * 8) + rr; };
   auto load_side = [&](int i, bf16x8 (&sd)[4], float (&prs)[4]) {
     const int mrow = m0w + i * 32 + rr;
-    if constexpr (SIDE) {
+    if constexpr (MAP) {
+      static_assert(EPI == 0 && HAS_R && HAS_RS, "the scatter form exists for the DropPath residual epilogue only");
+#pragma unroll
+      for (int pp = 0; pp < 4; ++pp)
+        if (FULL || mrow + pp * 8 < a.M) sd[pp] = *reinterpret_cast<const bf16x8*>(sidep + (size_t)pass_row(i, pp) * sideld + n_out);
+    } else if constexpr (SIDE) {
       const bf16* sp = sidep + (size_t)mrow * sideld + n_out;
 #pragma unroll
       for (int pp = 0; pp < 4; ++pp)
@@ -284,7 +305,8 @@
 #pragma unroll
             for (int e = 0; e < 8; ++e) v[e] = f2bf(bf2f(v[e]) + bf2f(sd[pp][e]));
           }
-          st_out(reinterpret_cast<bf16x8*>(yp + (size_t)pp * 8 * a.ldy), v, (a.act & 0x2000) != 0);
+          if constexpr (MAP) st_out(reinterpret_cast<bf16x8*>(a.Y + (size_t)pass_row(i, pp) * a.ldy + n_out), v, (a.act & 0x2000) != 0);
+          else st_out(reinterpret_cast<bf16x8*>(yp + (size_t)pp * 8 * a.ldy), v, (a.act & 0x2000) != 0);
         }
       }
       if constexpr (HAS_R || EPI == 2) __builtin_amdgcn_sched_barrier(0);
diff --git a/fiber_amd/csrc/norm.hip b/fiber_amd/csrc/norm.hip
--- a/fiber_amd/csrc/norm.hip
+++ b/fiber_amd/csrc/norm.hip
@@ -12,6 +12,14 @@
   }
 };
 
+struct SampleMap {
+  const int* idx; int rps;
+  __device__ __forceinline__ int row(int r) const { const int b = r / rps; return idx[b] * rps + (r - b * rps); }
+  __device__ __forceinline__ int slot_row(int r) const { const int b = r / rps, k = idx[b]; return k < 0 ? -1 : k * rps + (r - b * rps); }
+};
+
+constexpr int kSampleMap = 16;
+
 template <int LPR>
 __device__ __forceinline__ float group_sum(float v) {
 #pragma unroll
@@ -19,11 +27,14 @@
   return v;
 }
 
-template <int LPR, int NV, bool MERGE, bool X32, int U>
+template <int LPR, int NV, bool MERGE, bool X32, int UM>
 __global__ __launch_bounds__(256) void ln_fwd_kernel(const void* __restrict__ xv, const float* __restrict__ gamma,
                                                      const float* __restrict__ beta, bf16* __restrict__ y,
                                                      float* __restrict__ y32, float* __restrict__ mean,
-                                                     float* __restrict__ rstd, int rows, int C, float eps, MergeMap mm) {
+                                                     float* __restrict__ rstd, int rows, int C, float eps, MergeMap mm,
+                                                     SampleMap sm) {
+  constexpr int U = UM & 15;
+  constexpr bool SMAP = (UM & kSampleMap) != 0;
   const bf16* x = reinterpret_cast<const bf16*>(xv);
   const float* xf = reinterpret_cast<const float*>(xv);
   constexpr int RPW = 64 / LPR;
@@ -47,7 +58,9 @@
       for (int i = 0; i < NV; ++i) {
         const int vi = gl + i * LPR;
         if (row < rows && vi < nvec) {
-          const size_t off = MERGE ? mm.src(row, vi * 8) : (size_t)row * C + vi * 8;
+          size_t off;
+          if constexpr (SMAP) off = (size_t)sm.row(row) * C + vi * 8;
+          else off = MERGE ? mm.src(row, vi * 8) : (size_t)row * C + vi * 8;
           if constexpr (X32) {
             const float4 t0 = *reinterpret_cast<const float4*>(xf + off), t1 = *reinterpret_cast<const float4*>(xf + off + 4);
             v[u][i][0] = t0.x; v[u][i][1] = t0.y; v[u][i][2] = t0.z; v[u][i][3] = t0.w;
@@ -118,13 +131,15 @@
   }
 }
 
-template <int LPR, int NV, bool MERGE, bool X32, int U>
+template <int LPR, int NV, bool MERGE, bool X32, int UM>
 __global__ __launch_bounds__(256) void ln_bwd_kernel(const bf16* __restrict__ dy, const void* __restrict__ xv,
                                                      const float* __restrict__ gamma, const float* __restrict__ mean,
                                                      const float* __restrict__ rstd, const bf16* __restrict__ dres,
                                                      bf16* __restrict__ dx,
                                                      float* __restrict__ part , int rows, int C,
-                                                     MergeMap mm) {
+                                                     MergeMap mm, SampleMap sm) {
+  constexpr int U = UM & 15;
+  constexpr bool SMAP = (UM & kSampleMap) != 0;
   constexpr int RPW = 64 / LPR;
   const bf16* x = reinterpret_cast<const bf16*>(xv);
   const float* xf = reinterpret_cast<const float*>(xv);
@@ -146,12 +161,23 @@
     for (int u = 0; u < U; ++u) {
       const int row = base + u * RPW + sub;
       const bool rok = row < rows;
-      mu[u] = rok ? mean[row] : 0.f;
-      rs[u] = rok ? rstd[row] : 0.f;
+      int crow = row;
+      if constexpr (SMAP) crow = rok ? sm.slot_row(row) : -1;
+      const bool live = SMAP ? crow >= 0 : rok;
+      mu[u] = live ? mean[crow] : 0.f;
+      rs[u] = live ? rstd[crow] : 0.f;
 #pragma unroll
       for (int i = 0; i < NV; ++i) {
         const int vi = gl + i * LPR;
-        if (rok && vi < nvec) {
+        if constexpr (SMAP) {
+          if (rok && !live && vi < nvec) {
+#pragma unroll
+            for (int e = 0; e < 8; ++e) { rd[u][i][e] = (bf16)0.f; rx[u][i][e] = (bf16)0.f; }
+            rr[u][i] = *reinterpret_cast<const bf16x8*>(dres + (size_t)row * C + vi * 8);
+            continue;
+          }
+        }
+        if (live && vi < nvec) {
           const size_t off = MERGE ? mm.src(row, vi * 8) : (size_t)row * C + vi * 8;
           if constexpr (X32) {
             const float4 t0 = *reinterpret_cast<const float4*>(xf + off), t1 = *reinterpret_cast<const float4*>(xf + off + 4);
@@ -160,7 +186,7 @@
           } else {
             rx[u][i] = *reinterpret_cast<const bf16x8*>(x + off);
           }
-          rd[u][i] = *reinterpret_cast<const bf16x8*>(dy + (size_t)row * C + vi * 8);
+          rd[u][i] = *reinterpret_cast<const bf16x8*>(dy + (size_t)crow * C + vi * 8);
           if (dres) rr[u][i] = *reinterpret_cast<const bf16x8*>(dres + off);
         } else {
 #pragma unroll
@@ -285,25 +311,28 @@
   return u * (nvec <= 8 ? 8 : nvec <= 16 ? 4 : nvec <= 32 ? 2 : 1);
 }
 
-template <bool MERGE, bool X32>
+template <bool MERGE, bool X32, bool SMAP = false>
 int launch_fwd(const void* x, const float* g, const float* b, bf16* y, float* y32, float* mean, float* rstd, int rows, int C,
-               float eps, MergeMap mm, hipStream_t st) {
+               float eps, MergeMap mm, hipStream_t st, SampleMap sm = SampleMap{nullptr, 1}) {
   const int need = cdiv(rows, 4 * rows_per_wave(C));
   static const int div = getenv("FIBER_LN_FWD_DIV") ? atoi(getenv("FIBER_LN_FWD_DIV")) : 4;
   const int want = cdiv(need, div < 1 ? 1 : div);
   const int grid = want < 4096 ? want : 4096;
-#define FWD(LPR, NV, UU, ...) hipLaunchKernelGGL((ln_fwd_kernel<LPR, NV, MERGE, X32, UU>), dim3(grid), dim3(256), 0, st, __VA_ARGS__)
-  LN_DISPATCH(FWD, LN_UF, (LN_UF > 1 ? 2 : 1), x, g, b, y, y32, mean, rstd, rows, C, eps, mm);
+#define FWD(LPR, NV, UU, ...) \
+  hipLaunchKernelGGL((ln_fwd_kernel<LPR, NV, MERGE, X32, (UU) | (SMAP ? kSampleMap : 0)>), dim3(grid), dim3(256), 0, st, __VA_ARGS__)
+  LN_DISPATCH(FWD, LN_UF, (LN_UF > 1 ? 2 : 1), x, g, b, y, y32, mean, rstd, rows, C, eps, mm, sm);
 #undef FWD
   FIBER_CHECK_LAUNCH();
   return FIBER_OK;
 }
 
-template <bool MERGE, bool X32>
+template <bool MERGE, bool X32, bool SMAP = false>
 int launch_bwd(const bf16* dy, const void* x, const float* g, const float* mean, const float* rstd, const bf16* dres,
-               bf16* dx, float* dgamma, float* dbeta, float* ws, int grid, int rows, int C, MergeMap mm, hipStream_t st) {
-#define BWD(LPR, NV, UU, ...) hipLaunchKernelGGL((ln_bwd_kernel<LPR, NV, MERGE, X32, UU>), dim3(grid), dim3(256), 0, st, __VA_ARGS__)
-  LN_DISPATCH(BWD, LN_UB, 1, dy, x, g, mean, rstd, dres, dx, ws, rows, C, mm);
+               bf16* dx, float* dgamma, float* dbeta, float* ws, int grid, int rows, int C, MergeMap mm, hipStream_t st,
+               SampleMap sm = SampleMap{nullptr, 1}) {
+#define BWD(LPR, NV, UU, ...) \
+  hipLaunchKernelGGL((ln_bwd_kernel<LPR, NV, MERGE, X32, (UU) | (SMAP ? kSampleMap : 0)>), dim3(grid), dim3(256), 0, st, __VA_ARGS__)
+  LN_DISPATCH(BWD, LN_UB, 1, dy, x, g, mean, rstd, dres, dx, ws, rows, C, mm, sm);
 #undef BWD
   FIBER_CHECK_LAUNCH();
   hipLaunchKernelGGL(ln_bwd_reduce_kernel, dim3(cdiv(2 * C, 16)), dim3(1024), 0, st, ws, dgamma, dbeta, grid, C);
@@ -340,6 +369,26 @@
   if (C & 7) return FIBER_EINVAL;
   return launch_bwd<false, false>((const bf16*)dy, x, gamma, mean, rstd, (const bf16*)dres, (bf16*)dx, dgamma, dbeta, workspace,
                                   fiber_layernorm_bwd_grid(rows), rows, C, MergeMap{0, 0, 0}, stream);
+}
+
+extern "C" int fiber_layernorm_fwd_gather_bf16(const void* x, const float* gamma, const float* beta, void* y, float* mean,
+                                               float* rstd, int rows, int C, float eps, const int* kept, int rows_per_sample,
+                                               hipStream_t stream) {
+  if (rows <= 0) return FIBER_OK;
+  if ((C & 7) || !kept || rows_per_sample <= 0 || rows % rows_per_sample) return FIBER_EINVAL;
+  return launch_fwd<false, false, true>(x, gamma, beta, (bf16*)y, nullptr, mean, rstd, rows, C, eps, MergeMap{0, 0, 0}, stream,
+                                        SampleMap{kept, rows_per_sample});
+}
+
+extern "C" int fiber_layernorm_bwd_scatter_bf16(const void* dy, const void* x, const float* gamma, const float* mean,
+                                                const float* rstd, const void* dres, void* dx, float* dgamma, float* dbeta,
+                                                float* workspace, int rows, int C, const int* rank, int rows_per_sample,
+                                                hipStream_t stream) {
+  if (rows <= 0) return FIBER_OK;
+  if ((C & 7) || !rank || !dres || rows_per_sample <= 0 || rows % rows_per_sample) return FIBER_EINVAL;
+  return launch_bwd<false, false, true>((const bf16*)dy, x, gamma, mean, rstd, (const bf16*)dres, (bf16*)dx, dgamma, dbeta, workspace,
+                                        fiber_layernorm_bwd_grid(rows), rows, C, MergeMap{0, 0, 0}, stream,
+                                        SampleMap{rank, rows_per_sample});
 }
 
 extern "C" int fiber_layernorm_bwd_stream(const void* dy, const void* x, const float* gamma, const float* mean,
diff --git a/fiber_amd/lib.py b/fiber_amd/lib.py
--- a/fiber_amd/lib.py
+++ b/fiber_amd/lib.py
@@ -47,6 +47,12 @@
     "fiber_droppath_scale_f32": [P, I, F, U64, P],
     "fiber_rowscale_add_bf16": [P, P, P, P, L, L],
     "fiber_rowscale_colsum_bf16": [P, P, P, P, P, I, I, I],
+    "fiber_rowscale_colsum_gather_bf16": [P, P, P, P, P, P, I, I, I],
+    "fiber_droppath_map_i32": [P, P, P, P, I],
+    "fiber_layernorm_fwd_gather_bf16": [P, P, P, P, P, P, I, I, F, P, I],
+    "fiber_layernorm_bwd_scatter_bf16": [P, P, P, P, P, P, P, P, P, P, I, I, P, I],
+    "fiber_gemm_nt_scatter_bf16": [P, P, P, P, P, P, P, I, I, I, I, I, I, I, I],
+    "fiber_copy_dropped_bf16": [P, P, P, I, L],
     "fiber_ce_fwd_bf16": [P, P, P, P, P, I, I, L],
     "fiber_colsum_labelled_bf16": [P, P, P, P, I, I, L],
     "fiber_ce_bwd_bf16": [P, P, P, P, P, I, I, L],
diff --git a/fiber_amd/modules/swin_transformer.py b/fiber_amd/modules/swin_transformer.py
--- a/fiber_amd/modules/swin_transformer.py
+++ b/fiber_amd/modules/swin_transformer.py
@@ -118,11 +118,12 @@
         dp = self.drop_path_rate if self.training else 0.0
         s1 = ops.drop_path_scale(B, dp, x.device) if dp > 0.0 else None
         s2 = ops.drop_path_scale(B, dp, x.device) if dp > 0.0 else None
+        m2 = ops.drop_path_map(s2) if s2 is not None and ops.droppath_compactable(x) else None
         u, x = ops.layernorm_res(x, self.norm1.weight, self.norm1.bias, self.norm1.eps)
         rv = 1.0 / (1.0 - dp) if dp > 0.0 else None
         x = self.attn(u, (H, W), self.shift_size, shortcut=x, y=y, y_mask=y_mask, rowscale=s1, rowscale_value=rv)
         return ops.ln_mlp(x, self.norm2.weight, self.norm2.bias, self.norm2.eps, self.mlp.fc1.weight, self.mlp.fc1.bias,
-                          self.mlp.fc2.weight, self.mlp.fc2.bias, rowscale=s2, rowscale_value=rv)
+                          self.mlp.fc2.weight, self.mlp.fc2.bias, rowscale=s2, rowscale_value=rv, drop_map=m2)
 
 
 class PatchMerging(nn.Module):
diff --git a/fiber_amd/ops.py b/fiber_amd/ops.py
--- a/fiber_amd/ops.py
+++ b/fiber_amd/ops.py
@@ -654,11 +654,21 @@
 class _MLP(torch.autograd.Function):
 
     @staticmethod
-    def forward(ctx, x, w1, b1, w2, b2, residual, rowscale, rs_value=None, res32=None):
+    def forward(ctx, x, w1, b1, w2, b2, residual, rowscale, rs_value=None, res32=None, dmap=None):
         shp = x.shape
         x2 = _c(x).view(-1, shp[-1])
         need_bwd = any(ctx.needs_input_grad[:5])
         g, h = gemm_nt(x2, bf16_weight(w1), b1, None, 1, need_bwd)
+        ctx.dmap = dmap
+        if dmap is not None:
+            assert res32 is None and residual is not None and x2.shape[0] % dmap.n_kept == 0
+            rps = x2.shape[0] // dmap.n_kept
+            r2 = _c(residual).view(-1, w2.shape[0])
+            y = gemm_nt_scatter(g, bf16_weight(w2), b2, r2, dmap, rps)
+            if need_bwd:
+                ctx.save_for_backward(x2, w1, w2, h, g, rowscale)
+            ctx.has_res, ctx.shp, ctx.rs_value = True, shp, rs_value
+            return y.view(residual.shape), None
         rps = (x2.shape[0] // rowscale.numel()) if rowscale is not None else 0
         oshp = (*shp[:-1], w2.shape[0])
         if res32 is not None:
@@ -678,7 +688,7 @@
     def backward(ctx, dy, _dy32=None):
         dres = dy if ctx.has_res else None
         if not ctx.saved_tensors:
-            return (None,) * 5 + (dres, None, None, None)
+            return (None,) * 5 + (dres, None, None, None, None)
         x2, w1, w2, h, g, rowscale = ctx.saved_tensors
         dy2 = _c(dy).view(-1, w2.shape[0])
         db2 = None
@@ -686,7 +696,9 @@
         fused = C % 64 == 0 and C4 % 8 == 0 and _FUSED_MLP_BWD != "0"
         fold = fused and dy2.shape[1] % 8 == 0 and droppath_foldable(dy2.shape[0], rowscale, ctx.rs_value)
         rs_arg, rps, mask, scale = None, 0, None, 1.0
-        if fold:
+        if ctx.dmap is not None:
+            dy2, db2 = rowscale_colsum_gather(dy2, ctx.dmap, x2.shape[0] // ctx.dmap.n_kept)
+        elif fold:
             rs_arg, rps, mask, scale = rowscale, dy2.shape[0] // rowscale.numel(), rowscale, ctx.rs_value
         elif rowscale is not None:
             if dy2.shape[1] % 8 == 0:
@@ -710,11 +722,11 @@
             dw1, db1 = wgrad(dh, x2, want_bias=True)
         else:
             dw1 = wgrad(dh, x2)
-        return dx, dw1, db1, dw2, db2, dres, None, None, None
-
-
-def mlp(x, w1, b1, w2, b2, residual=None, rowscale=None, rowscale_value=None):
-    y, y32 = _MLP.apply(x, w1, b1, w2, b2, residual, rowscale, rowscale_value, f32_of(residual))
+        return dx, dw1, db1, dw2, db2, dres, None, None, None, None
+
+
+def mlp(x, w1, b1, w2, b2, residual=None, rowscale=None, rowscale_value=None, drop_map=None):
+    y, y32 = _MLP.apply(x, w1, b1, w2, b2, residual, rowscale, rowscale_value, f32_of(residual), drop_map)
     return with_f32(y, y32)
 
 
@@ -806,9 +818,14 @@
         return dx.view(ctx.shp), dgamma, dbeta, None, dw1, db1, dw2, db2, None, None
 
 
-def ln_mlp(x, gamma, beta, eps, w1, b1, w2, b2, rowscale=None, rowscale_value=None):
+def ln_mlp(x, gamma, beta, eps, w1, b1, w2, b2, rowscale=None, rowscale_value=None, drop_map=None):
     if ln_mlp_eligible(x, x.shape[-1]) and w1.shape[0] == 4 * x.shape[-1]:
         return _LnMlp.apply(x, gamma, beta, eps, w1, b1, w2, b2, rowscale, rowscale_value)
+    if drop_map is not None and droppath_compactable(x):
+        if drop_map.n_kept == 0:
+            return x
+        v, r = layernorm_res(x, gamma, beta, eps, drop_map=drop_map)
+        return mlp(v, w1, b1, w2, b2, residual=r, rowscale=rowscale, rowscale_value=rowscale_value, drop_map=drop_map)
     v, r = layernorm_res(x, gamma, beta, eps)
     return mlp(v, w1, b1, w2, b2, residual=r, rowscale=rowscale, rowscale_value=rowscale_value)
 
@@ -874,10 +891,23 @@
 class _LayerNormRes(torch.autograd.Function):
 
     @staticmethod
-    def forward(ctx, x, gamma, beta, eps, x32=None):
+    def forward(ctx, x, gamma, beta, eps, x32=None, dmap=None):
         C = x.shape[-1]
         x2 = _c(x).view(-1, C)
         xs = _c(x32).view(-1, C) if x32 is not None else None
+        ctx.dmap, ctx.xshape = dmap, x.shape
+        if dmap is not None:
+            assert xs is None and x.shape[0] == dmap.n
+            rps = x2.shape[0] // dmap.n
+            rows = dmap.n_kept * rps
+            y = torch.empty((rows, C), dtype=BF16, device=x2.device)
+            mean = torch.empty(rows, dtype=torch.float32, device=x2.device)
+            rstd = torch.empty_like(mean)
+            lib.call("fiber_layernorm_fwd_gather_bf16", lib.ptr(x2), lib.ptr(gamma), lib.ptr(beta), lib.ptr(y), lib.ptr(mean), lib.ptr(rstd),
+                     rows, C, eps, lib.ptr(dmap.kept), rps)
+            ctx.save_for_backward(x2, gamma, mean, rstd)
+            ctx.is32 = False
+            return y.view(dmap.n_kept, *x.shape[1:]), x2.view(x.shape)
         y, _, mean, rstd = _ln_fwd(x2, xs, gamma, beta, eps, False)
         ctx.save_for_backward(xs if xs is not None else x2, gamma, mean, rstd)
         ctx.is32 = xs is not None
@@ -888,15 +918,25 @@
         xs, gamma, mean, rstd = ctx.saved_tensors
         rows, C = xs.shape
         if dy is None:
-            return dres, None, None, None, None
+            return dres, None, None, None, None, None
+        if ctx.dmap is not None:
+            dmap = ctx.dmap
+            dr2 = _c(dres).view(rows, C) if dres is not None else torch.zeros((rows, C), dtype=BF16, device=xs.device)
+            dx = torch.empty((rows, C), dtype=BF16, device=xs.device)
+            dg = torch.empty(C, dtype=torch.float32, device=xs.device)
+            db = torch.empty_like(dg)
+            ws = torch.empty(lib.plain("fiber_layernorm_bwd_grid", rows) * 8 * C, dtype=torch.float32, device=xs.device)
+            lib.call("fiber_layernorm_bwd_scatter_bf16", lib.ptr(_c(dy).view(-1, C)), lib.ptr(xs), lib.ptr(gamma), lib.ptr(mean), lib.ptr(rstd),
+                     lib.ptr(dr2), lib.ptr(dx), lib.ptr(dg), lib.ptr(db), lib.ptr(ws), rows, C, lib.ptr(dmap.rank), rows // dmap.n)
+            return dx.view(ctx.xshape), dg, db, None, None, None
         dr2 = _c(dres).view(rows, C) if dres is not None else None
         dx, dg, db = _ln_bwd(_c(dy).view(rows, C), xs, ctx.is32, gamma, mean, rstd, dr2)
-        return dx.view(dy.shape), dg, db, None, None
-
-
-def layernorm_res(x, gamma, beta, eps=1e-5):
+        return dx.view(dy.shape), dg, db, None, None, None
+
+
+def layernorm_res(x, gamma, beta, eps=1e-5, drop_map=None):
     x32 = f32_of(x)
-    y, r = _LayerNormRes.apply(x, gamma, beta, eps, x32)
+    y, r = _LayerNormRes.apply(x, gamma, beta, eps, x32, drop_map)
     return y, with_f32(r, x32)
 
 
@@ -1489,8 +1529,79 @@
 
 def drop_path_scale(batch, p, device):
     out = torch.empty(batch, dtype=torch.float32, device=device)
-    lib.call("fiber_droppath_scale_f32", lib.ptr(out), batch, 1.0 - p, next_seed(), seed_base_ptr())
+    key = next_seed()
+    lib.call("fiber_droppath_scale_f32", lib.ptr(out), batch, 1.0 - p, key, seed_base_ptr())
+    if seed_base_ptr() is None:
+        out._dp_draw = (key, 1.0 - p)
     return out
+
+
+_DROPPATH_COMPACT = os.environ.get("FIBER_DROPPATH_COMPACT", "1") != "0"
+
+
+def droppath_host_keep(n, keep, key):
+    import numpy as np
+    u64 = np.uint64
+    with np.errstate(over="ignore"):
+        z = u64(key & _M64) + np.arange(n, dtype=u64) * u64(0x9E3779B97F4A7C15)
+        z = (z ^ (z >> u64(30))) * u64(0xBF58476D1CE4E5B9)
+        z = (z ^ (z >> u64(27))) * u64(0x94D049BB133111EB)
+        z = z ^ (z >> u64(31))
+    u = (z >> u64(41)).astype(np.float32) * np.float32(1.0 / 8388608.0)
+    return np.floor(np.float32(keep) + u) >= np.float32(1.0)
+
+
+class DropMap:
+    __slots__ = ("n", "n_kept", "kept", "rank", "cscale", "host_keep")
+
+
+def droppath_compactable(x):
+    return (x.dim() == 3 and x.is_cuda and x.dtype == BF16 and x.shape[-1] >= 512 and x.shape[-1] % 64 == 0 and x.shape[1] % 8 == 0
+            and f32_of(x) is None)
+
+
+def drop_path_map(scale):
+    draw = getattr(scale, "_dp_draw", None) if scale is not None else None
+    if (draw is None or not _DROPPATH_COMPACT or _RESIDUAL_FP32[0] or seed_base_ptr() is not None
+            or torch.cuda.is_current_stream_capturing()):
+        return None
+    n = scale.numel()
+    keep = droppath_host_keep(n, draw[1], draw[0])
+    n_kept = int(keep.sum())
+    if n_kept == n:
+        return None
+    m = DropMap()
+    m.n, m.n_kept, m.host_keep = n, n_kept, keep
+    idx = torch.empty((2, n), dtype=torch.int32, device=scale.device)
+    m.kept, m.rank = idx[0], idx[1]
+    m.cscale = torch.empty(n, dtype=torch.float32, device=scale.device)
+    lib.call("fiber_droppath_map_i32", lib.ptr(scale), lib.ptr(m.kept), lib.ptr(m.rank), lib.ptr(m.cscale), n)
+    return m
+
+
+def gemm_nt_scatter(x2, wb, bias, residual2, dmap, rows_per_sample):
+    M, K = x2.shape
+    N = wb.shape[0]
+    assert x2.dtype == BF16 and wb.dtype == BF16 and x2.stride(1) == 1 and wb.stride(1) == 1 and residual2.stride(1) == 1
+    assert M == dmap.n_kept * rows_per_sample and residual2.shape == (dmap.n * rows_per_sample, N) and residual2.stride(0) == N
+    y = torch.empty((residual2.shape[0], N), dtype=BF16, device=x2.device)
+    lib.call("fiber_gemm_nt_scatter_bf16", lib.ptr(x2), lib.ptr(wb), lib.ptr(bias), lib.ptr(residual2), lib.ptr(y), lib.ptr(dmap.cscale),
+             lib.ptr(dmap.kept), rows_per_sample, M, N, K, x2.stride(0), wb.stride(0), N, residual2.stride(0))
+    lib.call("fiber_copy_dropped_bf16", lib.ptr(residual2), lib.ptr(y), lib.ptr(dmap.rank), dmap.n, rows_per_sample * N)
+    return y
+
+
+def rowscale_colsum_gather(dy2, dmap, rows_per_sample):
+    N = dy2.shape[1]
+    M = dmap.n_kept * rows_per_sample
+    assert dy2.shape[0] == dmap.n * rows_per_sample and dy2.stride(0) == N
+    ds = torch.empty((M, N), dtype=BF16, device=dy2.device)
+    db = torch.empty(N, dtype=torch.float32, device=dy2.device)
+    slabs = lib.plain("fiber_colsum_slabs", M, N)
+    ws = torch.empty(slabs * N, dtype=torch.float32, device=dy2.device) if slabs > 1 else None
+    lib.call("fiber_rowscale_colsum_gather_bf16", lib.ptr(dy2), lib.ptr(dmap.cscale), lib.ptr(dmap.kept), lib.ptr(ds), lib.ptr(db), lib.ptr(ws),
+             M, N, rows_per_sample)
+    return ds, db
 
 
 def rowscale_add(resid, x, scale):
diff --git a/include/fiber_hip.h b/include/fiber_hip.h
--- a/include/fiber_hip.h
+++ b/include/fiber_hip.h
@@ -111,6 +111,19 @@
 int fiber_rowscale_colsum_bf16(const void* x, const float* scale, void* y, float* db, float* workspace, int M, int N,
                                int rows_per_sample, fiber_stream_t stream);
 
+int fiber_droppath_map_i32(const float* scale, int* kept, int* rank, float* cscale, int n, fiber_stream_t stream);
+int fiber_layernorm_fwd_gather_bf16(const void* x, const float* gamma, const float* beta, void* y, float* mean, float* rstd, int rows, int C,
+                                    float eps, const int* kept, int rows_per_sample, fiber_stream_t stream);
+int fiber_layernorm_bwd_scatter_bf16(const void* dy, const void* x, const float* gamma, const float* mean, const float* rstd, const void* dres,
+                                     void* dx, float* dgamma, float* dbeta, float* workspace, int rows, int C, const int* rank,
+                                     int rows_per_sample, fiber_stream_t stream);
+int fiber_gemm_nt_scatter_bf16(const void* X, const void* W, const float* bias, const void* residual, void* Y, const float* rowscale,
+                               const int* kept, int rows_per_sample, int M, int N, int K, int ldx, int ldw, int ldy, int ldr,
+                               fiber_stream_t stream);
+int fiber_copy_dropped_bf16(const void* x, void* y, const int* rank, int samples, long per_sample, fiber_stream_t stream);
+int fiber_rowscale_colsum_gather_bf16(const void* x, const float* scale, const int* kept, void* y, float* db, float* workspace, int M, int N,
+                                      int rows_per_sample, fiber_stream_t stream);
+
 int fiber_ce_fwd_bf16(const void* logits, const long long* labels, float* loss, float* lse, int* pred, int rows, int V,
                       long long ignore_index, fiber_stream_t stream);
 int fiber_ce_bwd_bf16(const void* logits, const long long* labels, const float* lse, const float* scale, void* dlogits, int rows,
```

New measurement: 998.9 images/s. About the same (-0.2%).
